# reclaimprotocol/gnark-symmetric-crypto

Measured on AMD Instinct MI355X. Metric: Groth16 proofs/sec (ChaCha20-V3 1-block), higher is better.
Workload: dtype u32 limbs (BN254 Fr/Fp, 254-bit modular integers); 1 GPU; ChaCha20-V3 single 64-byte block, reference pk.chacha20/r1cs.chacha20; 1xMI355X per rank: batch of 8192 independent proofs per GPU per step, fixed (r,s) (--dump-outputs); statements from xoshiro256** seeded 0x9E3779B97F4A7C15 + index; batch_per_gpu=8192, callers=2, parallelism=proofs sharded over 1 GPU(s), one process per GPU, gather to rank 0, tables=single algorithm per device

## Files before the change

gnark-symmetric-crypto_amd/__init__.py:

```python
import ctypes as C
import json
import os
import subprocess

_HERE = os.path.dirname(os.path.abspath(__file__))
LIB_PATH = os.path.join(_HERE, "libprove.so")
VERIFY_LIB_PATH = os.path.join(_HERE, "libverify.so")
CSRC = os.path.join(_HERE, "csrc")

CHACHA20, AES_128, AES_256 = 0, 1, 2
ALGORITHM_NAMES = {0: "chacha20", 1: "aes-128-ctr", 2: "aes-256-ctr"}

EXPORTS = ["enforce_binding", "InitAlgorithm", "Free", "Prove", "ProveBatch", "gsc_prove_raw", "gsc_setup",
           "gsc_set_deterministic_randomness", "gsc_debug_prove", "gsc_debug_vector", "gsc_describe", "gsc_last_stage_ms", "gsc_last_dominant_kernel", "gsc_last_kernel_clock", "gsc_debug_field_ops", "gsc_debug_limb_ops", "gsc_debug_curve_ops", "gsc_debug_decode_points", "gsc_debug_tower_ops", "gsc_debug_compute_h", "gsc_debug_compute_d", "gsc_debug_z_sum", "gsc_debug_quot_fold_dft", "gsc_debug_secret_residue", "gsc_debug_secret_scan", "gsc_debug_wipe", "gsc_debug_clock_trace", "gsc_debug_glv_split",
           "gsc_verify_init", "gsc_verify_raw", "VerifyBatch", "gsc_debug_pairing",
           "gsc_verify_raw_batched", "gsc_verify_all", "VerifyAll", "gsc_debug_verify_randomizers",
           "gsc_verify_json", "gsc_verify_last_path", "gsc_debug_verify_path", "gsc_debug_pairing_few",
           "gsc_verify_claims", "VerifyClaims",
           "gsc_prove_check_init", "gsc_prove_check_stats", "gsc_debug_prove_corrupt",
           "gsc_release_algorithm", "gsc_replace_algorithm", "gsc_memory_info", "gsc_key_generation",
           "gsc_setup_contribute", "gsc_setup_verify_contribution", "gsc_debug_scale_points",
           "gsc_srs_verify", "gsc_debug_srs_generate", "gsc_debug_group_idft", "gsc_debug_column_sums", "gsc_setup_from_srs", "gsc_debug_msm", "gsc_debug_solve", "gsc_debug_assemble",
           "gsc_srs_initial", "gsc_srs_contribute", "gsc_srs_verify_contribution", "gsc_debug_scale_powers"]


class GoSlice(C.Structure):
    _fields_ = [("data", C.c_void_p), ("len", C.c_longlong), ("cap", C.c_longlong)]


class DebugMsmArgs(C.Structure):
    _fields_ = [("group", C.c_int32), ("nbases", C.c_uint32),
                ("points", C.c_char_p), ("kind", C.c_char_p), ("rowlen", C.c_void_p), ("rows", C.c_void_p),
                ("n_rows", C.c_uint32), ("zero_row", C.c_uint32),
                ("c", C.c_int32), ("cv", C.c_int32), ("mont", C.c_int32),
                ("batch", C.c_uint32), ("nproofs", C.c_uint32), ("per_flat", C.c_uint32), ("per_win", C.c_uint32), ("digit_bases", C.c_uint32),
                ("digit_rows", C.c_void_p), ("scalars_be", C.c_char_p),
                ("plane", C.c_char_p), ("plane_rows", C.c_uint32), ("plane_stride", C.c_uint32),
                ("out", C.c_void_p), ("out_inf", C.c_void_p),
                ("flat_digits", C.c_void_p), ("flat_digits_cap", C.c_size_t), ("win_digits", C.c_void_p), ("win_digits_cap", C.c_size_t),
                ("gok", C.c_void_p), ("gok_cap", C.c_size_t), ("group_ok", C.c_void_p), ("group_ok_cap", C.c_size_t),
                ("info", C.c_void_p)]


class DebugSolveArgs(C.Structure):
    _fields_ = [("n_public", C.c_uint32), ("n_secret", C.c_uint32), ("n_internal", C.c_uint32), ("n_constraints", C.c_uint32),
                ("calldata", C.c_void_p), ("n_calldata", C.c_uint32),
                ("blueprint", C.c_void_p), ("constraint_off", C.c_void_p), ("wire_off", C.c_void_p), ("n_instr", C.c_uint32),
# ... 660 lines not shown
    if n <= 0:
        raise RuntimeError("algorithm not initialised")
    assert len(ab_be) == 2 * m * 64 * 32
    out = C.create_string_buffer(n * 64 * 32)
    if L.gsc_debug_compute_d(algorithm_id, ab_be, m, out, len(out)) != n:
        raise RuntimeError("gsc_debug_compute_d failed")
    return out.raw


def debug_z_sum(algorithm_id: int, abc_be: bytes, m: int):
    L = lib()
    L.gsc_debug_z_sum.restype = C.c_int
    L.gsc_debug_z_sum.argtypes = [C.c_ubyte, C.c_char_p, C.c_size_t, C.c_void_p, C.c_void_p]
    assert len(abc_be) == 3 * m * 64 * 32
    out, flags = C.create_string_buffer(64 * 64), C.create_string_buffer(64)
    if L.gsc_debug_z_sum(algorithm_id, abc_be, m, out, flags) != 0:
        raise RuntimeError("gsc_debug_z_sum failed")
    return out.raw, flags.raw


def debug_quot_fold_dft(L: int, m: int, perm, u_be: bytes, u_inf: bytes, v_be: bytes, v_inf: bytes):
    lb = lib()
    n = 1 << L
    lb.gsc_debug_quot_fold_dft.restype = C.c_int
    lb.gsc_debug_quot_fold_dft.argtypes = [C.c_int, C.c_uint32, C.c_void_p] + [C.c_char_p] * 4 + [C.c_void_p] * 4
    assert len(u_be) == 64 * m and len(u_inf) == m and len(v_be) == 64 * n and len(v_inf) == n and (perm is None or len(perm) == n)
    pm = (C.c_uint32 * n)(*perm) if perm is not None else None
    u2, f2, v2, g2 = C.create_string_buffer(64 * m), C.create_string_buffer(m), C.create_string_buffer(64 * max(m - 1, 1)), C.create_string_buffer(max(m - 1, 1))
    if lb.gsc_debug_quot_fold_dft(L, m, pm, u_be, u_inf, v_be, v_inf, u2, f2, v2, g2) != 0:
        raise RuntimeError("gsc_debug_quot_fold_dft failed")
    return u2.raw, f2.raw, v2.raw[:64 * (m - 1)], g2.raw[:m - 1]


def verify_init(algorithm_id: int, verifying_key: bytes) -> bool:
    s, keep = _slice(verifying_key)
    return bool(lib().gsc_verify_init(algorithm_id, s))


def verify_raw(algorithm_id: int, proofs: bytes, lens, signals: bytes, n: int = None):
    n = len(lens) if n is None else n
    assert len(proofs) >= 196 * n and len(signals) >= 144 * n
    lens_arr = (C.c_uint32 * max(n, 1))(*lens[:n])
    out = C.create_string_buffer(max(n, 1))
    rc = lib().gsc_verify_raw(algorithm_id, bytes(proofs), lens_arr, bytes(signals), n, out)
    if rc < 0:
        raise RuntimeError("gsc_verify_raw failed (%d): %s" % (rc, "no key loaded" if rc == -1 else "device error"))
    return list(out.raw[:n])


def verify_batch(items) -> list:
    enc = [{k: (list(v) if isinstance(v, (bytes, bytearray)) else v) for k, v in it.items()} if isinstance(it, dict) else it for it in items]
    s, keep = _slice(json.dumps(enc).encode())
    return json.loads(_take(lib().VerifyBatch(s)))


def verify_batch_bytes(params_json: bytes) -> bytes:
    s, keep = _slice(params_json)
    return _take(lib().VerifyBatch(s))


def verify_raw_batched(algorithm_id: int, proofs: bytes, lens, signals: bytes, n: int = None):
    n = len(lens) if n is None else n
    assert len(proofs) >= 196 * n and len(signals) >= 144 * n
    lens_arr = (C.c_uint32 * max(n, 1))(*lens[:n])
    out = C.create_string_buffer(max(n, 1))
    rc = lib().gsc_verify_raw_batched(algorithm_id, bytes(proofs), lens_arr, bytes(signals), n, out)
# ... 125 lines not shown
```

gnark-symmetric-crypto_amd/csrc/capi.cpp:

```cpp
#include "../../include/libprove.h"
#include "engine.hpp"
#include "dispatch.hpp"
#include "formats.hpp"
#include "registry.hpp"
#include "glv.hpp"
#include "host_ciphers.hpp"
#include "json.hpp"
#include "setup.hpp"
#include "phase2_gpu.hpp"
#include "srs_gpu.hpp"
#include "srs_contrib.hpp"
#include "srs_contrib_gpu.hpp"
#include "msm_debug.hpp"
#include "solver_debug.hpp"
#include "assemble_debug.hpp"
#include <sys/random.h>
#include <cerrno>
#include <condition_variable>
#include <deque>
#include <thread>
#include <cstdio>
#include <cstdlib>
#include <chrono>
#include <cstring>
// ... 634 lines not shown
        std::string report;
        const long long total = (long long)a->debug_secret_scan(report);
        if (out && cap) { const size_t n = report.size() < cap - 1 ? report.size() : cap - 1; memcpy(out, report.data(), n); out[n] = 0; }
        return total;
    } catch (const std::exception& e) { fprintf(stderr, "gsc_debug_secret_scan: %s\n", e.what()); return -1; }
}
int gsc_debug_wipe(uint64_t bytes, int fill, const uint64_t* desc, size_t ndesc, const uint8_t* cls, size_t ncls, uint8_t* buf_out, const uint64_t* win, size_t nwin, uint64_t* counts, float* ms) {
    if (hooks_refused("gsc_debug_wipe") || (ndesc && !desc) || (nwin && (!win || !counts)) || (ncls && !cls) || ndesc > 4096 || nwin > 4096) return -1;
    try { const float t = debug_wipe(config_from_env().device, bytes, fill, desc, ndesc, cls, ncls, buf_out, win, nwin, counts); if (ms) *ms = t; return 0; }
    catch (const std::exception& e) { fprintf(stderr, "gsc_debug_wipe: %s\n", e.what()); return -1; }
}
long long gsc_debug_compute_d(GoUint8 algorithmID, const uint8_t* ab_be, size_t m, uint8_t* d_out, size_t cap) {
    if (hooks_refused("gsc_debug_compute_d") || algorithmID > 2) return -1;
    const Snapshot snap = snapshot(algorithmID); Algorithm* a = algo_of(snap); if (!a) return -1;
    if (!d_out) return (long long)a->domain_size();
    if (cap < a->domain_size() * 64 * 32) return -1;
    try { a->debug_compute_d(ab_be, m, d_out); return (long long)a->domain_size(); }
    catch (const std::exception& e) { printf("%s\n", e.what()); return -1; }
}
int gsc_debug_z_sum(GoUint8 algorithmID, const uint8_t* abc_be, size_t m, uint8_t* out, uint8_t* flags) {
    if (hooks_refused("gsc_debug_z_sum") || algorithmID > 2 || !abc_be || !out || !flags) return -1;
    const Snapshot snap = snapshot(algorithmID); Algorithm* a = algo_of(snap); if (!a) return -1;
    try { a->debug_z_sum(abc_be, m, out, flags); return 0; }
    catch (const std::exception& e) { printf("%s\n", e.what()); return -1; }
}

int gsc_debug_quot_fold_dft(int L, uint32_t m, const uint32_t* perm, const uint8_t* u_be, const uint8_t* u_inf, const uint8_t* v_be, const uint8_t* v_inf,
                            uint8_t* u2_be, uint8_t* u2_inf, uint8_t* v2_be, uint8_t* v2_inf) {
    if (hooks_refused("gsc_debug_quot_fold_dft") || L < 2 || L > 17 || m < 2 || m > (1u << L) || !u_be || !u_inf || !v_be || !v_inf || !u2_be || !u2_inf || !v2_be || !v2_inf) return -1;
    try { debug_quot_fold_dft(config_from_env().device, L, m, perm, u_be, u_inf, v_be, v_inf, u2_be, u2_inf, v2_be, v2_inf); return 0; }
    catch (const std::exception& e) { printf("%s\n", e.what()); return -1; }
}

size_t gsc_describe(GoUint8 algorithmID, char* out, size_t cap) {
    if (algorithmID > 2 || !cap) return 0;
    const Snapshot snap = snapshot(algorithmID); Algorithm* a = algo_of(snap);
    std::string s = a ? a->describe() + " key=" + snap->key_id + " gen=" + std::to_string(snap.generation()) : std::string("not initialised");
    size_t n = s.size() < cap - 1 ? s.size() : cap - 1; memcpy(out, s.data(), n); out[n] = 0; return n;
}
int gsc_last_dominant_kernel(GoUint8 algorithmID, char* name, size_t cap, float* ms, size_t* statements, size_t* columns, size_t* nbases) {
    if (algorithmID > 2) return -1;
    const Snapshot snap = snapshot(algorithmID); Algorithm* a = algo_of(snap); if (!a) return -1;
    const KernelStat st = a->last_kernel_stat();
    if (name && cap) { const size_t n = strlen(st.name) < cap - 1 ? strlen(st.name) : cap - 1; memcpy(name, st.name, n); name[n] = 0; }
    if (ms) *ms = st.ms;
    if (statements) *statements = st.statements;
    if (columns) *columns = st.columns;
    if (nbases) *nbases = st.nbases;
    return 0;
}
int gsc_last_kernel_clock(GoUint8 algorithmID, float* clock_mhz, int* windows) {
    if (algorithmID > 2) return -1;
    const Snapshot snap = snapshot(algorithmID); Algorithm* a = algo_of(snap); if (!a) return -1;
    const KernelStat st = a->last_kernel_stat();
    if (clock_mhz) *clock_mhz = st.clock_mhz;
    if (windows) *windows = st.nwin;
    return 0;
}
int gsc_last_stage_ms(GoUint8 algorithmID, float out[4]) {
    if (algorithmID > 2) return -1;
    const Snapshot snap = snapshot(algorithmID); Algorithm* a = algo_of(snap); if (!a) return -1;
    const KernelStat st = a->last_kernel_stat();
    for (int i = 0; i < 4; i++) out[i] = st.stage_ms[i];
    return 0;
}

// ... 2 lines not shown
```

gnark-symmetric-crypto_amd/csrc/chunk_route.hpp:

```cpp
#pragma once
#include "engine.hpp"

namespace gsc {

struct RouteFacts {
    bool small_ok = false;
    bool has_commitment = false;
    bool quotient_eval = false, fuse_z_digits = false;
    bool zfew_flat = false;
    bool a_flat = false, b1_flat = false, b2_flat = false;
};
struct RouteCall {
    bool dbg = false;
    bool allow_few_solver = true;
    bool allow_small = true;
    bool skip_resident = false;
};

struct ChunkRoute {
    bool latency = false;
    bool resident_wanted = false;
    bool small = false;
    bool resident = false;
    bool early_ab = false, early_b2 = false;
    bool use_zfew = false;
    bool eval = false;
    bool z_digits_ready = false;
    bool overlap_q = false;
    const char* kernel_name = "";
};

constexpr size_t OVERLAP_QUOTIENT_BELOW = 4096;

inline ChunkRoute chunk_route(size_t n, const EngineConfig& cfg, const RouteFacts& f, const RouteCall& call) {
    const size_t B = (n + 63) / 64 * 64;
    ChunkRoute r;
    r.latency = cfg.few_path && n <= (size_t)cfg.few_max;
    r.resident_wanted = n <= (size_t)cfg.few_max && B == 64 && cfg.few_solver;
    r.small = f.small_ok && call.allow_small && !cfg.solver_trace && (!r.latency || cfg.small_witness_few);
    r.resident = r.resident_wanted && call.allow_few_solver && !r.small && !call.skip_resident;
    r.early_ab = r.latency && f.a_flat && f.b1_flat;
    r.early_b2 = r.early_ab && f.b2_flat;
    r.use_zfew = r.latency && f.zfew_flat;
    r.eval = f.quotient_eval && !r.use_zfew;
    r.z_digits_ready = r.eval && f.fuse_z_digits && !r.latency;
    r.overlap_q = r.z_digits_ready && !call.dbg && (cfg.overlap_quotient == 2 || (cfg.overlap_quotient && B < OVERLAP_QUOTIENT_BELOW));
    r.kernel_name = !r.latency ? "k_msm_win<Fp29f>"
                  : r.small ? "k_wit_chain + k_wit_rows"
                  : !r.resident ? "k_solver (one launch per level)"
                  : f.has_commitment ? "k_solver_few + commitment MSM" : "k_solver_few";
    return r;
}

}
```

gnark-symmetric-crypto_amd/csrc/engine.hip:

```cpp
#include "engine_impl.hpp"
#include "dispatch.hpp"
#include <cstdio>
#include <cstdlib>
#include <cstring>
#include <thread>

namespace gsc {

namespace {
int env_int(const char* name, int dflt) { const char* v = getenv(name); return v && *v ? atoi(v) : dflt; }
}

bool test_hooks_enabled() {
    static const bool on = [] { const char* e = getenv("GSC_ENABLE_TEST_HOOKS"); return e && e[0] == '1' && e[1] == 0; }();
    return on;
}
namespace { const bool g_hooks_read_at_load = test_hooks_enabled(); }

EngineConfig config_from_env() {
    EngineConfig c;
    c.device = env_int("GSC_DEVICE", 0);
    if (const char* dv = getenv("GSC_DEVICES")) {
        for (const char* q = dv; *q;) { while (*q == ',' || *q == ' ') q++; if (!*q) break; char* end = nullptr; const long v = strtol(q, &end, 10); if (end == q) throw std::runtime_error("GSC_DEVICES: expected a comma-separated list of device ordinals"); c.devices.push_back((int)v); q = end; }
    }
    c.max_batch = (size_t)env_int("GSC_MAX_BATCH", 1024);
    c.lanes = env_int("GSC_LANES", 0);
    c.small_lanes = env_int("GSC_SMALL_LANES", -1);
    if (c.small_lanes > 8) throw std::runtime_error("GSC_SMALL_LANES must be at most 8");
    c.small_lane_cap = env_int("GSC_SMALL_LANE_CAP", 0);
    if (c.small_lane_cap < 0 || c.small_lane_cap % 64) throw std::runtime_error("GSC_SMALL_LANE_CAP must be a multiple of 64");
    const bool hooks = test_hooks_enabled();
    c.min_split = (size_t)(hooks ? env_int("GSC_MIN_SPLIT", 0) : 0);
    c.bit_groups = env_int("GSC_BIT_GROUPS", 1);
    c.window_z = env_int("GSC_WINDOW_Z", 0);
    c.window_w = env_int("GSC_WINDOW_W", 0);
    c.z_table_gb = env_int("GSC_Z_TABLE_GB", 48);
    c.w_table_gb = env_int("GSC_W_TABLE_GB", 16);
    c.row_margin_bits = hooks ? env_int("GSC_ROW_MARGIN_BITS", 1) : 1;
    c.few_path = env_int("GSC_FEW_PATH", 1);
    c.few_solver = env_int("GSC_FEW_SOLVER", 1);
    c.few_max = env_int("GSC_FEW_MAX", 0);
    if (c.few_max < 0 || c.few_max > (int)MSM_FEW_PROOFS) throw std::runtime_error("GSC_FEW_MAX must be in [0, 32]");
    c.few_workgroups = hooks ? env_int("GSC_FEW_WGS", 0) : 0;
    c.few_z_gb = env_int("GSC_FEW_Z_GB", 12);
    c.few_wide = env_int("GSC_FEW_WIDE", 1);
    c.quotient_eval = env_int("GSC_QUOTIENT_EVAL", 1);
    c.fuse_z_digits = env_int("GSC_FUSE_Z_DIGITS", 1);
    c.quotient_fold = env_int("GSC_QUOTIENT_FOLD", 1);
    if (c.quotient_fold < 0 || c.quotient_fold > 2) throw std::runtime_error("GSC_QUOTIENT_FOLD must be 0, 1 or 2");
    c.quotient_live_tiles = env_int("GSC_QUOTIENT_LIVE_TILES", 1) ? 1 : 0;
    c.small_witness = env_int("GSC_SMALL_WITNESS", 1);
    c.small_witness_few = env_int("GSC_SMALL_WITNESS_FEW", 1);
    c.ntt_plain = env_int("GSC_NTT_PLAIN", 1) ? 1 : 0;
    c.overlap_quotient = env_int("GSC_OVERLAP_QUOTIENT", 1);
    if (c.overlap_quotient < 0 || c.overlap_quotient > 2) throw std::runtime_error("GSC_OVERLAP_QUOTIENT must be 0, 1 or 2");
    c.stream_priorities = env_int("GSC_STREAM_PRIORITIES", 1);
    if (c.stream_priorities != 0 && c.stream_priorities != 1 && !(hooks && c.stream_priorities >= 111 && c.stream_priorities <= 333)) throw std::runtime_error("GSC_STREAM_PRIORITIES must be 0 or 1");
    if (test_hooks_enabled()) { c.win_slice = env_int("GSC_WIN_SLICE", 256); if (c.win_slice < 64 || c.win_slice > 4096 || c.win_slice % 8) throw std::runtime_error("GSC_WIN_SLICE must be a multiple of 8 in [64, 4096]"); }
    if (c.small_witness < 0 || c.small_witness > 2 || (c.small_witness == 2 && !test_hooks_enabled())) throw std::runtime_error("GSC_SMALL_WITNESS must be 0 or 1");
    if (c.few_workgroups < 0 || c.few_workgroups > 256) throw std::runtime_error("GSC_FEW_WGS must be in [0, 256]");
    c.trace_host = getenv("GSC_TRACE_HOST") != nullptr;
    c.prove_check = env_int("GSC_PROVE_CHECK", 0) != 0;
    if (const char* d = getenv("GSC_VK_DIR")) c.vk_dir = d;
    if (test_hooks_enabled()) { c.solver_trace = getenv("GSC_SOLVER_TRACE") != nullptr; c.few_test_abort = getenv("GSC_FEW_TEST_ABORT") != nullptr; c.keep_secrets = getenv("GSC_KEEP_SECRETS") != nullptr; c.wipe_full = env_int("GSC_WIPE", 1) != 0; c.fail_after_stage = env_int("GSC_FAIL_AFTER_STAGE", 0); c.wipe_grid = env_int("GSC_WIPE_GRID", 0); if (c.wipe_grid < 0 || c.wipe_grid > 65536) throw std::runtime_error("GSC_WIPE_GRID must be in [0, 65536]"); c.z_exp_entry_bits = env_int("GSC_Z_EXP_ENTRY_BITS", 0); }
    if (c.max_batch < 64) c.max_batch = 64;
    c.max_batch = (c.max_batch + 63) / 64 * 64;
    if ((c.window_z && (c.window_z < 4 || c.window_z > MSM_MAX_WINDOW)) || (c.window_w && (c.window_w < 4 || c.window_w > 16))) throw std::runtime_error("GSC_WINDOW_Z must be in [4,17], GSC_WINDOW_W in [4,16]");
    return c;
}

void debug_field_ops(int device, int field, int op, const uint8_t* a, const uint8_t* b, uint8_t* out, size_t n, int chain) {
    use_device(device);
    DevBuf<fe> da(n), db(n), dout(n);
    HIP_CHECK(hipMemcpy(da.p, a, 32 * n, hipMemcpyHostToDevice)); HIP_CHECK(hipMemcpy(db.p, b, 32 * n, hipMemcpyHostToDevice));
    if (!launch_field_ops(field, op, da.p, db.p, dout.p, n, chain, nullptr)) throw std::runtime_error("gsc_debug_field_ops: field " + std::to_string(field) + " has no op " + std::to_string(op));
    HIP_CHECK(hipGetLastError());
    HIP_CHECK(hipDeviceSynchronize());
    HIP_CHECK(hipMemcpy(out, dout.p, 32 * n, hipMemcpyDeviceToHost));
}

void debug_limb_ops(int device, int field, int op, const int32_t* a, const int32_t* b, const int32_t* c, const int32_t* d, int32_t* out, size_t n) {
    const int operands = op == 0 ? 2 : op == 2 ? 4 : 1;
    const int32_t* src[4] = {a, b, c, d};
// ... 68 lines not shown
    HIP_CHECK(hipMemset(dflags.p, 0, n));
    if (!launch_tower_ops(path, op, din.p, dout.p, dflags.p, n, nullptr)) return false;
    HIP_CHECK(hipGetLastError());
    HIP_CHECK(hipDeviceSynchronize());
    if (ow) HIP_CHECK(hipMemcpy(out, dout.p, 4 * (size_t)ow * n, hipMemcpyDeviceToHost));
    HIP_CHECK(hipMemcpy(flags, dflags.p, n, hipMemcpyDeviceToHost));
    return true;
}

void debug_quot_fold_dft(int device, int L, uint32_t m, const uint32_t* perm, const uint8_t* u_be, const uint8_t* u_inf, const uint8_t* v_be, const uint8_t* v_inf,
                         uint8_t* u2_be, uint8_t* u2_inf, uint8_t* v2_be, uint8_t* v2_inf) {
    const size_t n = (size_t)1 << L;
    std::vector<uint32_t> pm(n);
    {
        std::vector<uint8_t> seen(n, 0);
        for (size_t i = 0; i < n; i++) { pm[i] = perm ? perm[i] : (uint32_t)i; if (pm[i] >= n || seen[pm[i]]++) throw std::runtime_error("gsc_debug_quot_fold_dft: perm is not a permutation of 0 .. n - 1"); }
    }
    use_device(device);
    DevBuf<uint32_t> d_perm(n);
    DevBuf<uint8_t> d_be((m + n) * 64), d_inf(m + n), d_stU(m), d_stV(n), d_stU2(m), d_stV2(m - 1), d_out((2 * (size_t)m - 1) * 64), d_flags(2 * (size_t)m - 1), scratch(quot_fold_dft_scratch_bytes(L, m));
    DevBuf<G1Aff> d_U(m), d_V(n), d_U2(m), d_V2(m - 1);
    HIP_CHECK(hipMemcpy(d_perm.p, pm.data(), 4 * n, hipMemcpyHostToDevice));
    HIP_CHECK(hipMemcpy(d_be.p, u_be, 64 * (size_t)m, hipMemcpyHostToDevice)); HIP_CHECK(hipMemcpy(d_be.p + 64 * (size_t)m, v_be, 64 * n, hipMemcpyHostToDevice));
    HIP_CHECK(hipMemcpy(d_inf.p, u_inf, m, hipMemcpyHostToDevice)); HIP_CHECK(hipMemcpy(d_inf.p + m, v_inf, n, hipMemcpyHostToDevice));
    launch_g1_aff_from_be(d_be.p, d_inf.p, m, d_U.p, d_stU.p, nullptr);
    launch_g1_aff_from_be(d_be.p + 64 * (size_t)m, d_inf.p + m, n, d_V.p, d_stV.p, nullptr);
    launch_quot_fold_dft(L, m, d_perm.p, d_U.p, d_stU.p, d_V.p, d_stV.p, d_U2.p, d_stU2.p, d_V2.p, d_stV2.p, scratch.p, nullptr);
    launch_g1_aff_to_be(d_U2.p, d_stU2.p, m, d_out.p, d_flags.p, nullptr);
    launch_g1_aff_to_be(d_V2.p, d_stV2.p, m - 1, d_out.p + 64 * (size_t)m, d_flags.p + m, nullptr);
    HIP_CHECK(hipGetLastError());
    HIP_CHECK(hipDeviceSynchronize());
    HIP_CHECK(hipMemcpy(u2_be, d_out.p, 64 * (size_t)m, hipMemcpyDeviceToHost)); HIP_CHECK(hipMemcpy(u2_inf, d_flags.p, m, hipMemcpyDeviceToHost));
    if (m > 1) { HIP_CHECK(hipMemcpy(v2_be, d_out.p + 64 * (size_t)m, 64 * (size_t)(m - 1), hipMemcpyDeviceToHost)); HIP_CHECK(hipMemcpy(v2_inf, d_flags.p + m, m - 1, hipMemcpyDeviceToHost)); }
}

float debug_wipe(int device, uint64_t bytes, int fill, const uint64_t* desc, size_t ndesc, const uint8_t* cls, size_t ncls, uint8_t* out, const uint64_t* win, size_t nwin, uint64_t* counts) {
    use_device(device);
    if (!bytes || bytes > ((uint64_t)1 << 36)) throw std::runtime_error("gsc_debug_wipe: buffer size out of range");
    auto checked = [&](const uint64_t* d, uint8_t* base, const uint8_t* d_cls) {
        const uint64_t off = d[0], rows = d[1], pitch = d[2], width = d[3];
        if (off > bytes || rows > bytes || pitch > bytes || width > bytes) throw std::runtime_error("gsc_debug_wipe: descriptor outside the buffer");
        if (rows && width) {
            if (rows > 1 && pitch < width) throw std::runtime_error("gsc_debug_wipe: rows overlap");
            const unsigned __int128 end = (unsigned __int128)off + (unsigned __int128)(rows - 1) * pitch + width;
            if (end > bytes) throw std::runtime_error("gsc_debug_wipe: descriptor outside the buffer");
        }
        if (d[4] && (!d_cls || !ncls)) throw std::runtime_error("gsc_debug_wipe: plane image without row classes");
        return WipeDesc{base + off, rows, pitch, width, d[4] ? d_cls : nullptr, d[4] ? (uint64_t)ncls : 0};
    };
    DevBuf<uint8_t> buf(bytes), d_cls(ncls ? ncls : 1); DevBuf<unsigned long long> d_cnt(nwin ? nwin : 1);
    if (ncls) HIP_CHECK(hipMemcpy(d_cls.p, cls, ncls, hipMemcpyHostToDevice));
    std::vector<WipeDesc> ds, ws;
    for (size_t i = 0; i < ndesc; i++) ds.push_back(checked(desc + 5 * i, buf.p, d_cls.p));
    for (size_t i = 0; i < nwin; i++) ws.push_back(checked(win + 5 * i, buf.p, d_cls.p));
    HIP_CHECK(hipMemset(buf.p, fill, bytes));
    HIP_CHECK(hipMemset(d_cnt.p, 0, d_cnt.bytes()));
    HIP_CHECK(hipDeviceSynchronize());
    hipEvent_t e0, e1; HIP_CHECK(hipEventCreate(&e0)); HIP_CHECK(hipEventCreate(&e1));
    struct Ev { hipEvent_t a, b; ~Ev() { (void)hipEventDestroy(a); (void)hipEventDestroy(b); } } ev{e0, e1};
    HIP_CHECK(hipEventRecord(e0, nullptr));
    launch_wipe(ds.data(), ds.size(), 0, nullptr);
    HIP_CHECK(hipEventRecord(e1, nullptr));
    for (size_t i = 0; i < nwin; i++) launch_scan_idle(ws[i], d_cnt.p + i, nullptr);
    HIP_CHECK(hipGetLastError());
    HIP_CHECK(hipDeviceSynchronize());
    float ms = 0; HIP_CHECK(hipEventElapsedTime(&ms, e0, e1));
// ... 41 lines not shown
    for (size_t k = 0; k < impls_.size(); k++) { std::lock_guard<std::mutex> l(impls_[k]->check_mu); impls_[k]->check = ctx[k]; }
    return true;
}
void Algorithm::prove_check_off() { for (auto& i : impls_) { std::lock_guard<std::mutex> l(i->check_mu); i->check.reset(); } }
void Algorithm::prove_check_stats(uint64_t out[4]) const {
    for (int k = 0; k < 4; k++) out[k] = 0;
    for (auto& i : impls_) if (auto c = i->check_now()) prove_check_add_stats(*c, out);
}
bool Algorithm::debug_prove_corrupt(uint32_t index, int which, int mode) {
    if (which < 0 || which > 4 || mode < 0 || mode > 1 || (which > 2 && !impls_[0]->has_commitment)) return false;
    corrupt_.store((uint64_t)1 << 63 | (uint64_t)mode << 40 | (uint64_t)which << 32 | index);
    return true;
}
Algorithm::~Algorithm() = default;
Cipher Algorithm::cipher() const { return impls_[0]->cipher; }
size_t Algorithm::max_batch() const { size_t c = 0; for (auto& i : impls_) c += i->cap; return c; }
size_t Algorithm::devices() const { return impls_.size(); }
size_t Algorithm::lanes() const { return impls_[0]->lanes.size(); }
namespace { thread_local KernelStat t_call_stat; thread_local const Algorithm* t_call_owner = nullptr; }
KernelStat Algorithm::last_kernel_stat() const {
    if (t_call_owner == this) return t_call_stat;
    AlgorithmImpl* a = impls_[last_replica_.load() < impls_.size() ? last_replica_.load() : 0].get();
    std::lock_guard<std::mutex> lk(a->stat_mu);
    return a->last_stat;
}
std::string Algorithm::describe() const {
    const AlgorithmImpl* impl_ = impls_[0].get();
    char buf[640];
    snprintf(buf, sizeof buf, "wires=%zu constraints=%zu domain=2^%d max_batch=%zu lanes=%zu small=%zux%zu devices=%zu window_z=%d window_w=%d tables=%.2f GiB bases A=%zu B=%zu K=%zu Z=%zu grouped A=%zu B=%zu K=%zu wide(windowed+expanded) A=%zu+%zu B=%zu+%zu K=%zu+%zu",
             impl_->n_wires, impl_->n_constraints, impl_->L, max_batch(), impl_->full_lanes, impl_->lanes.size() - impl_->full_lanes, impl_->lanes.size() > impl_->full_lanes ? impl_->lanes.back()->cap : (size_t)0, impls_.size(), impl_->cfg.window_z, impl_->cfg.window_w, impl_->table_bytes / 1073741824.0,
             impl_->mA.nbases, impl_->mB1.nbases, impl_->mK.nbases, impl_->mZ.digit_bases ? impl_->mZ.digit_bases : impl_->mZ.nbases, impl_->mA.nbit, impl_->mB1.nbit, impl_->mK.nbit,
             impl_->mA.nwide, impl_->mA.nexpanded, impl_->mB1.nwide, impl_->mB1.nexpanded, impl_->mK.nwide, impl_->mK.nexpanded);
    std::string out = buf;
    if (impl_->quotient_eval) out += std::string(" quotient=evaluation-form") + (impl_->fuse_z_digits ? "+digits" : "") + (!impl_->fuse_z_digits || !impl_->cfg.overlap_quotient ? "" : impl_->cfg.overlap_quotient == 2 ? "+beside-wire-sets" : "+beside-wire-sets(<4096)") + "(c: " + std::to_string(impl_->mC.nbit) + " grouped + " + std::to_string(impl_->mC.nflat - impl_->mC.nbit) + " flat + " + std::to_string(impl_->mC.nwide) + " windowed)";
    else out += " quotient=coefficient-form";
    if (impl_->quotient_eval) out += impl_->mZ.digit_bases ? " Zlive=" + std::to_string(impl_->mZ.nwide) + " Zfold=dft" :" Zfold=off(" + impl_->fold_why + ")";
    if (impl_->quotient_eval) out += " Qtiles=" + std::to_string(quot_live_tiles(impl_->L, impl_->quot_live)) + "/" + std::to_string(1u << (impl_->L - (impl_->L + 1) / 2));
    out += impl_->small.ok ? " witness=small-integer(" + std::to_string(impl_->small.n_levels) + " chained levels, fallbacks " + std::to_string(impl_->small_fallbacks.load()) + ")" : " witness=generic" + (impl_->small.why.empty() ? std::string() : "(" + impl_->small.why + ")");
    out += impl_->cfg.keep_secrets ? " wipe=off" : impl_->cfg.wipe_full ? " wipe=full" : " wipe=inputs";
    {
        size_t bytes = 0; bool on = false;
        for (auto& i : impls_) if (auto c = i->check_now()) { on = true; bytes += prove_check_device_bytes(*c); }
        out += on ? " check=on(" + std::to_string(bytes) + ")" : " check=off";
    }
    out += " served(calls/statements)=";
    const auto sv = picker_->served();
    for (size_t i = 0; i < sv.size(); i++) out += (i ? "," : "") + std::to_string(sv[i].calls) + "/" + std::to_string(sv[i].statements);
    return out;
}
size_t Algorithm::domain_size() const { return impls_[0]->domain_n; }
template <class Quot>
static void debug_quotient(AlgorithmImpl& a, const char* who, const uint8_t* mats_be, size_t mats, size_t m, uint8_t* out, Quot quot) {
    if (m > a.n_constraints) throw std::runtime_error(std::string(who) + ": more rows than constraints");
    HIP_CHECK(hipSetDevice(a.cfg.device));
    struct Hold { AlgorithmImpl& a; size_t i; ~Hold() { a.release_lane(i); } } hold{a, a.acquire_lane(0)};
    AlgorithmImpl::Lane& ln = *a.lanes[0];
    const size_t B = 64, cnt = m * B;
    DevBuf<uint8_t> d_be(mats * cnt * 32 + 32, true);
    d_be.upload(mats_be, mats * cnt * 32, ln.stream);
    fe* const dst[3] = {ln.d_A.p, ln.d_B.p, ln.d_C.p};
    for (size_t k = 0; k < mats; k++) launch_fr_from_be(d_be.p + k * cnt * 32, dst[k], cnt, ln.stream);
    NttPlan plan{a.L, a.tw_fwd.p, a.tw_inv.p, a.scale_mid.p, a.scale_out.p, a.dom.p + 5, a.qr.p};
    HIP_CHECK(quot(plan, ln, B));
    if (out) HIP_CHECK(hipMemcpyAsync(out, ln.d_A.p, a.domain_n * B * 32, hipMemcpyDeviceToHost, ln.stream));
    if (!a.cfg.keep_secrets && a.cfg.wipe_full) a.wipe_whole(ln, ln.stream);
    HIP_CHECK(hipStreamSynchronize(ln.stream));
}
// ... 119 lines not shown
```

gnark-symmetric-crypto_amd/csrc/engine.hpp:

```cpp
#pragma once
#include <cstdint>
#include <cstring>
#include <atomic>
#include <cstddef>
#include <memory>
#include <string>
#include <utility>
#include <vector>

namespace gsc {

enum Cipher : int { CHACHA20 = 0, AES_128 = 1, AES_256 = 2 };

struct ProofRequest {
    uint8_t key[32]; uint32_t keylen;
    uint8_t nonce[12]; uint32_t counter;
    uint8_t plaintext[64];
    uint8_t ciphertext[64];
    uint8_t r[32], s[32], mask[32];
    ~ProofRequest() { explicit_bzero(this, sizeof *this); }
};
struct ProofResult {
    int status = 0;
    uint8_t proof[196]; size_t proof_len = 0;
};

struct EngineConfig {
    int device = 0;
    std::vector<int> devices;
    size_t max_batch = 1024;
    int lanes = 0;
    int small_lanes = -1;
    int small_lane_cap = 0;
    size_t min_split = 0;
    int window_z = 0;
    int window_w = 0;
    int z_table_gb = 48, w_table_gb = 16;
    int bit_groups = 1;
    int row_margin_bits = 1;
    int few_path = 1;
    int few_max = 0;
    int few_solver = 1;
    int few_workgroups = 0;
    int few_z_gb = 12;
    int few_wide = 1;
    int quotient_eval = 1;
    int fuse_z_digits = 1;
    int quotient_fold = 1;
    int quotient_live_tiles = 1;
    int small_witness = 1;
    int ntt_plain = 1;
    int overlap_quotient = 1;
    int stream_priorities = 1;
    int small_witness_few = 1;
    int win_slice = 256;
    bool prove_check = false;
    std::string vk_dir;
    bool trace_host = false;
    bool solver_trace = false;
    int z_exp_entry_bits = 0;
    bool keep_secrets = false;
    bool wipe_full = true;
    int wipe_grid = 0;
    int fail_after_stage = 0;
    bool few_test_abort = false;
    std::vector<size_t> outgoing_bytes; size_t reclaim_bytes = 0;
};
EngineConfig config_from_env();
bool test_hooks_enabled();

struct KernelStat { const char* name = ""; float ms = 0; size_t statements = 0, columns = 0, nbases = 0; float stage_ms[4] = {0, 0, 0, 0}; float clock_mhz = 0; int nwin = 0; };

struct DebugVectors { std::vector<uint8_t> W, A, B, C, H; size_t n_wires = 0, n_constraints = 0, n = 0; };

class AlgorithmImpl;
class Algorithm {
  public:
    Algorithm(Cipher cipher, const uint8_t* pk, size_t pk_len, const uint8_t* r1cs, size_t r1cs_len, const EngineConfig& cfg);
    ~Algorithm();
    Cipher cipher() const;
    void prove_batch(const ProofRequest* reqs, size_t n, ProofResult* results, DebugVectors* debug_first = nullptr, bool whole = false);
    void forget_thread_stat() const;
    size_t max_batch() const;
    size_t devices() const;
    size_t lanes() const;
    std::string describe() const;
    KernelStat last_kernel_stat() const;
    void debug_compute_h(const uint8_t* abc_be, size_t m, uint8_t* h_out);
    void debug_compute_d(const uint8_t* ab_be, size_t m, uint8_t* d_out);
    size_t domain_size() const;
    void debug_z_sum(const uint8_t* abc_be, size_t m, uint8_t* out, uint8_t* flags);
    size_t debug_secret_residue();
    size_t debug_secret_scan(std::string& report);
    size_t scrub_before_free();
    std::vector<std::pair<int, size_t>> replica_bytes() const;
    bool prove_check_init(const uint8_t* vk, size_t len);
    void prove_check_off();
    void prove_check_stats(uint64_t out[4]) const;
    bool debug_prove_corrupt(uint32_t index, int which, int mode);
  private:
    std::atomic<uint64_t> corrupt_{0};
    std::vector<std::unique_ptr<AlgorithmImpl>> impls_;
    std::unique_ptr<class ReplicaPicker> picker_;
    mutable std::atomic<size_t> last_replica_{0};
};

bool device_memory_info(int device, uint64_t out[4]);
size_t verifier_device_bytes(int device);

void debug_quot_fold_dft(int device, int L, uint32_t m, const uint32_t* perm, const uint8_t* u_be, const uint8_t* u_inf, const uint8_t* v_be, const uint8_t* v_inf,
                         uint8_t* u2_be, uint8_t* u2_inf, uint8_t* v2_be, uint8_t* v2_inf);
float debug_wipe(int device, uint64_t bytes, int fill, const uint64_t* desc, size_t ndesc, const uint8_t* cls, size_t ncls, uint8_t* out, const uint64_t* win, size_t nwin, uint64_t* counts);
void debug_clock_trace(int device, uint32_t n, uint32_t interval_us, unsigned long long* out);
void debug_field_ops(int device, int field, int op, const uint8_t* a, const uint8_t* b, uint8_t* out, size_t n, int chain);
void debug_limb_ops(int device, int field, int op, const int32_t* a, const int32_t* b, const int32_t* c, const int32_t* d, int32_t* out, size_t n);
void debug_curve_ops(int device, int group, int op, const uint8_t* pts, const uint8_t* inf, const uint8_t* lam, size_t n, size_t k, uint8_t* out, uint8_t* flags);
void debug_decode_points(int device, int group, const uint8_t* bytes, size_t len, size_t n, uint8_t* out_xy, uint8_t* status);
bool debug_tower_ops(int device, int path, int op, const int32_t* in, size_t n, int32_t* out, uint8_t* flags);

}
```

gnark-symmetric-crypto_amd/csrc/engine_impl.hpp:

```cpp
#pragma once
#include "engine.hpp"
#include "chunk_route.hpp"
#include "formats.hpp"
#include "kernels.hpp"
#include "wit_small.hpp"
#include "solver_tables.hpp"
#include "msm_set.hpp"
#include "wipe_plan.hpp"
#include "prove_check.hpp"
#include <atomic>
#include <chrono>
#include <cstring>
#include <condition_variable>
#include <memory>
#include <mutex>
#include <stdexcept>
#include <string>
#include <vector>

namespace gsc {

template <class T>
struct PinnedBuf {
    T* p = nullptr; size_t n = 0;
    PinnedBuf() = default;
    PinnedBuf(const PinnedBuf&) = delete; PinnedBuf& operator=(const PinnedBuf&) = delete;
    ~PinnedBuf() { if (p) (void)hipHostFree(p); }
    void alloc(size_t count) { if (p) { (void)hipHostFree(p); p = nullptr; } n = count; if (count) { HIP_CHECK(hipHostMalloc((void**)&p, count * sizeof(T), hipHostMallocDefault)); memset(p, 0, count * sizeof(T)); } }
    size_t bytes() const { return n * sizeof(T); }
};

struct KeyPoints {
    std::vector<uint8_t> x, y;
    KeyPoints() = default;
    KeyPoints(const std::vector<uint8_t>& x_, const std::vector<uint8_t>& y_ = {}) : x(x_), y(y_) {}
};
std::vector<uint8_t> decode_g1_points(const KeyPoints& pts, G1Aff* out, hipStream_t stream);
std::vector<uint8_t> decode_g2_points(const KeyPoints& pts, G2Aff* out, hipStream_t stream);


constexpr int STREAM_PLAIN = 1 << 30, STREAM_ROLE_INIT = -1;
hipStream_t stream_take(int device, int kind, int role);
void stream_give(int device, int kind, int role, hipStream_t s);

std::atomic<size_t>& prover_bytes_on(int device);

class AlgorithmImpl : public SolverTables {
  public:
    Cipher cipher; EngineConfig cfg;
    size_t domain_n = 0; int L = 0;
    std::mutex pool_mu; std::condition_variable pool_cv; std::vector<uint8_t> lane_busy;
    size_t acquire_lane(int want = -1, size_t n = 0) {
        std::unique_lock<std::mutex> l(pool_mu);
        size_t got = 0;
        pool_cv.wait(l, [&] {
            bool found = false;
            for (size_t i = 0; i < lane_busy.size(); i++) {
                if (lane_busy[i] || (want >= 0 && (size_t)want != i) || lanes[i]->cap < n) continue;
                if (!found || lanes[i]->cap < lanes[got]->cap) { got = i; found = true; }
            }
            return found;
        });
        lane_busy[got] = 1;
        return got;
    }
    std::atomic<int> calls_in_flight{0};
    int cu_count = 256;
    std::atomic<uint32_t> few_skip{0}; std::atomic<uint32_t> few_penalty{16};
    std::mutex stat_mu; KernelStat last_stat;
    std::mutex check_mu; std::shared_ptr<ProveCheckCtx> check;
    std::shared_ptr<ProveCheckCtx> check_now() { std::lock_guard<std::mutex> l(check_mu); return check; }
    std::atomic<uint64_t>* corrupt = nullptr;
    void release_lane(size_t i) { { std::lock_guard<std::mutex> l(pool_mu); lane_busy[i] = 0; } pool_cv.notify_all(); }
    hipStream_t stream = nullptr;
    size_t table_bytes = 0;
    std::vector<uint8_t> row_class;

    std::vector<uint8_t> row_class_a, row_class_b;
    void init_small(const SolverProgram& sp);
    std::atomic<uint64_t> small_fallbacks{0};
    DevBuf<int32_t> tw_fwd, tw_inv, tw_inv_plain, qr; DevBuf<fe> scale_mid, scale_mid_plain, scale_out, dom;
    MsmSet<G1Aff> mA, mB1, mK, mZ, mZfew, mPed, mPedSigma; MsmSet<G2Aff> mB2;
    bool quotient_eval = false; MsmSet<G1Aff> mC; std::vector<uint8_t> row_class_c;
    bool fuse_z_digits = false;
    std::string fold_why = "GSC_QUOTIENT_FOLD=0";
    size_t quot_live = 0;
    bool fold_quotient_bases(const DevBuf<G1Aff>& d_U, const std::vector<uint8_t>& stU, const DevBuf<G1Aff>& d_V, const std::vector<uint8_t>& stV, const std::vector<uint32_t>& rowsZ,
                             DevBuf<G1Aff>& d_U2, std::vector<uint8_t>& stU2, DevBuf<G1Aff>& d_V2, std::vector<uint8_t>& stV2);
    struct Lane {
        hipStream_t stream = nullptr, side = nullptr, side2 = nullptr;
        hipEvent_t ev_ab = nullptr, ev_fs = nullptr, ev_b2 = nullptr, ev_s2 = nullptr;
        hipEvent_t ev_ws = nullptr;
        hipEvent_t ev_wa = nullptr, ev_wa_done = nullptr;
        hipEvent_t ev_few = nullptr;
        hipEvent_t ev[7] = {};
        float stage_ms[4] = {0, 0, 0, 0}; float msm_z_kernel_ms = 0; size_t last_batch = 0;
        PinnedBuf<uint8_t> h_in, h_rs, h_mask, h_out, h_flags, h_cpts; PinnedBuf<uint32_t> h_status; PinnedBuf<GlvSplit> h_glv; PinnedBuf<unsigned long long> h_words;
        uint32_t* h_fsync() const { return reinterpret_cast<uint32_t*>(h_words.p); }
        uint32_t& h_wsflag() const { return *reinterpret_cast<uint32_t*>(h_words.p + 1); }
        unsigned long long* h_clk() const { return h_words.p + 2; }
        KernelStat stat;
        DevBuf<unsigned long long> d_clk;
        size_t n_real = 0;
        size_t cap = 0;
        DevBuf<uint8_t> d_inputs, d_rs, d_out, d_flags, d_mask_in, d_cpts; DevBuf<uint32_t> d_status, d_fsync; DevBuf<GlvSplit> d_glv;
        DevBuf<fe> d_mask, d_commit; DevBuf<G1Xyzz> d_sumD, d_sumPok;
        DevBuf<fe> d_W, d_A, d_B, d_C;
        bool small_active = false;
        DevBuf<int8_t> d_W8, d_A8, d_B8, d_C8; DevBuf<uint32_t> d_wsflag;
        DevBuf<G1Xyzz> d_part1a, d_part1b, d_sumA, d_sumB1, d_sumK, d_sumZ, d_sumC, d_tmp; DevBuf<G2Xyzz> d_part2a, d_part2b, d_sumB2;
        DevBuf<uint4> d_digits_s2; DevBuf<uint8_t> d_gok_s2;
        DevBuf<uint4> d_digits_s; DevBuf<uint8_t> d_gok_s; DevBuf<G1Xyzz> d_part1c, d_part1d;
        DevBuf<uint4> d_digits;
        DevBuf<uint4> d_digits_w;
        static constexpr int NSETS = 8;
        DevBuf<G1Xyzz> d_sj1[NSETS], d_flat1[NSETS]; DevBuf<G2Xyzz> d_sj2, d_flat2;
        MsmHornerJobs pending1{}, pending2{};
        DevBuf<uint8_t> d_gok;
        struct Region { int region; uint8_t* p; size_t bytes; };
        std::vector<Region> regions; size_t allocated = 0;
        template <class T> void reg(int region, DevBuf<T>& b) { if (b.p) regions.push_back(Region{region, reinterpret_cast<uint8_t*>(b.p), b.bytes()}); }
        struct ScratchNeed { size_t part1a = 0, part1b = 0, part2a = 0, part2b = 0, digits = 0, digits_w = 0, gok = 0, sj1[8] = {0, 0, 0, 0, 0, 0, 0, 0}, sj2 = 0; };
        std::vector<ScratchNeed> need_at;
        bool wipe_a_pending = false;
        ~Lane() { if (ev_few) { for (int d = 0; d < 64; d++) { FewSolverChain& c = few_solver_chain(d); std::lock_guard<std::mutex> lk(c.m); if (c.last == ev_few) c.last = nullptr; } (void)hipEventDestroy(ev_few); }
                  for (auto& e : ev) if (e) (void)hipEventDestroy(e); if (ev_ws) (void)hipEventDestroy(ev_ws); if (ev_wa) (void)hipEventDestroy(ev_wa); if (ev_wa_done) (void)hipEventDestroy(ev_wa_done); if (ev_ab) (void)hipEventDestroy(ev_ab); if (ev_fs) (void)hipEventDestroy(ev_fs); if (ev_b2) (void)hipEventDestroy(ev_b2); if (ev_s2) (void)hipEventDestroy(ev_s2); if (side2) stream_give(device, kind[2], 3 * index + 2, side2); if (side) stream_give(device, kind[1], 3 * index + 1, side); if (stream) stream_give(device, kind[0], 3 * index, stream); }
        int device = 0, index = 0, kind[3] = {STREAM_PLAIN, STREAM_PLAIN, STREAM_PLAIN};
    };
    std::vector<std::unique_ptr<Lane>> lanes;
    size_t cap = 0;
    size_t full_lanes = 0;
    static constexpr size_t SMALL_LANE_CAP = 1024;

    AlgorithmImpl(Cipher c, const uint8_t* pk, size_t pk_len, const uint8_t* r1cs, size_t r1cs_len, const EngineConfig& cf);
    ~AlgorithmImpl() { prover_bytes_on(cfg.device) -= accounted; lanes.clear(); if (stream) stream_give(cfg.device, STREAM_PLAIN, STREAM_ROLE_INIT, stream); }
    size_t held_bytes() const { size_t b = table_bytes; for (auto& ln : lanes) b += ln->allocated; return b; }
    size_t accounted = 0;

    std::unique_ptr<SolverProgram> init_program(const R1csFile& cs);

    static void pack_inputs(const ProofRequest* reqs, size_t n, size_t B, uint8_t* h_in, uint8_t* h_rs);

    void calibrate();

    std::vector<uint8_t> decompress_g1(const KeyPoints& pts, G1Aff* out) { return decode_g1_points(pts, out, stream); }
    std::vector<uint8_t> decompress_g2(const KeyPoints& pts, G2Aff* out) { return decode_g2_points(pts, out, stream); }

    static constexpr size_t EXPAND_MAX = 64;
    static constexpr int EXPAND_C = 15, NARROW_MAX_BITS = 14;

    template <class AffT, class XyzzT, class Decomp>
    void build_set(MsmSet<AffT>& set, const KeyPoints& raw, size_t point_bytes, const std::vector<uint32_t>& rows, int c, const char* what, Decomp decomp, bool uniform, int expand_cv = 0,
                   const std::vector<uint8_t>* classes = nullptr, uint32_t zero_row = 0xFFFFFFFFu, bool latency_layout = true);
    void init_key(const R1csFile& cs, const PkFile& key);

    void alloc_lane(Lane& ln, size_t B);

    RouteFacts route_facts() const { return RouteFacts{small.ok, has_commitment, quotient_eval, fuse_z_digits, mZfew.nflat != 0, mA.latency_flat(), mB1.latency_flat(), mB2.latency_flat()}; }
    struct Chunk {
        const ProofRequest* reqs; size_t n, B; DebugVectors* dbg; ChunkRoute rt;
        std::chrono::steady_clock::time_point t_start, t_enqueued, t_done;
        std::shared_ptr<ProveCheckCtx> check = nullptr;
        uint64_t corrupt = 0;
        std::vector<uint8_t> verdict = {};
        bool check_fell_back = false;
    };
    MsmLaunchOpts msm_opts;
    MsmCtx with_plane(MsmCtx c, const Lane& ln, const fe* scalars) const {
        if (!ln.small_active) return c;
        if (scalars == ln.d_W.p) { c.plane = ln.d_W8.p; c.plane_rows = n_wires; c.plane_stride = small.rows_per_group; }
        else if (scalars == ln.d_C.p) { c.plane = ln.d_C8.p; c.plane_rows = n_constraints; c.plane_stride = n_constraints; }
        return c;
    }
    int set_index(const MsmSet<G1Aff>& set) const { const MsmSet<G1Aff>* all[Lane::NSETS] = {&mA, &mB1, &mK, &mZ, &mPed, &mPedSigma, &mZfew, &mC}; for (int k = 0; k < Lane::NSETS; k++) if (all[k] == &set) return k; return 0; }
    void run_msm_g1(Lane& ln, const Chunk& ck, const MsmSet<G1Aff>& set, const fe* scalars, int mont, G1Xyzz* sum, bool timed = false, bool side = false, bool digits_ready = false);
    void run_msm_g2(Lane& ln, const Chunk& ck, const MsmSet<G2Aff>& set, const fe* scalars, int mont, G2Xyzz* sum, bool side = false);
    template <class AffT> void flush_horner(MsmHornerJobs& pending, size_t B, hipStream_t s) { launch_msm_horner<AffT>(pending, B, s); pending.n = 0; }

    void fetch_column(Lane& ln, const fe* mat, size_t rows, size_t B, size_t col, std::vector<uint8_t>& out);
    void wipe_secrets(Lane& ln, size_t B, bool small_call);
    WipePlan plan_wipe(const Lane& ln, const Chunk& ck) const;
    void run_wipe(Lane& ln, const std::vector<WipeItem>& items, hipStream_t s, unsigned max_blocks);
    void wipe_phase_a(Lane& ln, const Chunk& ck);
    void wipe_phase_b(Lane& ln, const Chunk& ck);
    void wipe_whole(Lane& ln, hipStream_t s);
    void fail_after(int stage) const { if (cfg.fail_after_stage == stage) throw std::runtime_error("GSC_FAIL_AFTER_STAGE=" + std::to_string(stage) + ": test failure injected"); }
    size_t secret_residue();
    size_t secret_scan(size_t lane_base, std::string& report, size_t& registered, size_t& allocated);

    void prove_chunk(Lane& ln, const ProofRequest* reqs, size_t n, ProofResult* results, DebugVectors* dbg, bool allow_few_solver = true, bool allow_small = true);
    std::unique_ptr<ProveCheckPass> check_enqueue(Lane& ln, const Chunk& ck);
    void stage_upload(Lane& ln, const Chunk& ck);
    void stage_witness(Lane& ln, const Chunk& ck);
    void stage_early_sums(Lane& ln, const Chunk& ck);
    void stage_quotient(Lane& ln, const Chunk& ck);
    void stage_msms(Lane& ln, const Chunk& ck);
    void stage_assembly(Lane& ln, Chunk& ck);
    void stage_stat(Lane& ln, const Chunk& ck);
    void run_levels(Lane& ln, const Chunk& ck, SolverArgs& sa, uint32_t from, uint32_t to);
    void solve_small(Lane& ln, const Chunk& ck);
    void dump_solver_trace(Lane& ln, const unsigned long long* d_trace);
    void trace_chunk(Lane& ln, const Chunk& ck);

    void serialize(const uint8_t* o, uint8_t flags, uint32_t status, const uint8_t* commitment_xy, const uint8_t* pok_xy, ProofResult& res, bool released = true) const;
};

}
// ... 1 lines not shown
```

gnark-symmetric-crypto_amd/csrc/engine_prove.hip:

```cpp
#include "engine_impl.hpp"
#include "glv.hpp"
#include "prove_check_kernels.hpp"
#include <chrono>
#include <cstdio>
#include <cstring>

namespace gsc {

FewSolverChain& few_solver_chain(int device) { static FewSolverChain* chains = new FewSolverChain[64]; return chains[device & 63]; }

namespace {
const uint8_t kHalfP[32] = {0x18, 0x32, 0x27, 0x39, 0x70, 0x98, 0xd0, 0x14, 0xdc, 0x28, 0x22, 0xdb, 0x40, 0xc0, 0xac, 0x2e,
                            0xcb, 0xc0, 0xb5, 0x48, 0xb4, 0x38, 0xe5, 0x46, 0x9e, 0x10, 0x46, 0x0b, 0x6c, 0x3e, 0x7e, 0xa3};

void le_limbs_to_be(const uint8_t* le, uint8_t* be) { for (int i = 0; i < 32; i++) be[i] = le[31 - i]; }
bool be_greater(const uint8_t* a, const uint8_t* b) { int c = memcmp(a, b, 32); return c > 0; }
bool be_is_zero(const uint8_t* a) { for (int i = 0; i < 32; i++) if (a[i]) return false; return true; }
}

void AlgorithmImpl::run_msm_g1(Lane& ln, const Chunk& ck, const MsmSet<G1Aff>& set, const fe* scalars, int mont, G1Xyzz* sum, bool timed, bool side, bool digits_ready) {
    const int k = set_index(set);
    MsmRun<G1Xyzz> r{MsmCtx{ln.stream, ln.d_digits_w.p && &set != &mZ ? ln.d_digits_w.p : ln.d_digits.p, ln.d_gok.p}, scalars, mont != 0, ck.B, ck.n, ck.rt.latency,
                     ln.d_part1a.p, ln.d_part1b.p, ln.d_sj1[k].p, ln.d_flat1[k].p, sum};
    if (side) {
// ... 252 lines not shown
        if (dbg) {
            DevBuf<fe> ta(domain_n * B, true), tb(domain_n * B, true), tc(domain_n * B, true);
            HIP_CHECK(hipMemcpyAsync(ta.p, ln.d_A.p, n_constraints * B * sizeof(fe), hipMemcpyDeviceToDevice, ln.stream));
            HIP_CHECK(hipMemcpyAsync(tb.p, ln.d_B.p, n_constraints * B * sizeof(fe), hipMemcpyDeviceToDevice, ln.stream));
            HIP_CHECK(hipMemcpyAsync(tc.p, ln.d_C.p, n_constraints * B * sizeof(fe), hipMemcpyDeviceToDevice, ln.stream));
            HIP_CHECK(launch_compute_h(plan, ta.p, tb.p, tc.p, n_constraints, B, ln.stream, 0));
            fetch_column(ln, ta.p, domain_n, B, 0, dbg->H);
        }
        if (rt.overlap_q) HIP_CHECK(hipStreamWaitEvent(qs, ln.ev[1], 0));
        if (rt.z_digits_ready) HIP_CHECK(launch_compute_d_digits(plan, ln.d_A.p, ln.d_B.p, n_constraints, B, QuotDigits{ln.d_digits.p, mZ.c, mZ.nwin}, qs, narrow, quot_live));
        else HIP_CHECK(launch_compute_d(plan, ln.d_A.p, ln.d_B.p, n_constraints, B, ln.stream, few_cols, narrow, quot_live));
    } else HIP_CHECK(launch_compute_h(plan, ln.d_A.p, ln.d_B.p, ln.d_C.p, n_constraints, B, ln.stream, few_cols, narrow));
    HIP_CHECK(hipEventRecord(ln.ev[2], qs));
    if (dbg && !rt.eval) fetch_column(ln, ln.d_A.p, domain_n, B, 0, dbg->H);
}

void AlgorithmImpl::stage_msms(Lane& ln, const Chunk& ck) {
    const size_t B = ck.B; const ChunkRoute& rt = ck.rt;
    if (!rt.early_ab) {
        run_msm_g1(ln, ck, mA, ln.d_W.p, 1, ln.d_sumA.p);
        run_msm_g1(ln, ck, mB1, ln.d_W.p, 1, ln.d_sumB1.p);
        flush_horner<G1Aff>(ln.pending1, B, ln.stream);
        HIP_CHECK(hipEventRecord(ln.ev_ab, ln.stream));
        HIP_CHECK(hipStreamWaitEvent(ln.side, ln.ev_ab, 0));
        launch_fin_scalarmul(ln.d_sumA.p, ln.d_sumB1.p, ln.d_rs.p, B, ln.d_out.p, ln.d_flags.p, ln.d_tmp.p, ln.side);
    }
    if (!rt.early_b2) run_msm_g2(ln, ck, mB2, ln.d_W.p, 1, ln.d_sumB2.p);
    if (ln.pending2.n) {
        HIP_CHECK(hipEventRecord(ln.ev_b2, ln.stream));
        HIP_CHECK(hipStreamWaitEvent(ln.side, ln.ev_b2, 0));
        flush_horner<G2Aff>(ln.pending2, B, ln.side);
    }
    HIP_CHECK(hipEventRecord(ln.ev_fs, ln.side));
    run_msm_g1(ln, ck, mK, ln.d_W.p, 1, ln.d_sumK.p);
    if (rt.eval) {
        HIP_CHECK(hipMemsetAsync(ln.d_C.p + domain_n * B, 0, B * sizeof(fe), ln.stream));
        run_msm_g1(ln, ck, mC, ln.d_C.p, 1, ln.d_sumC.p);
    }
    if (rt.overlap_q) { HIP_CHECK(hipEventRecord(ln.ev_ws, ln.stream)); HIP_CHECK(hipStreamWaitEvent(ln.stream, ln.ev[2], 0)); }
    wipe_phase_a(ln, ck);
    run_msm_g1(ln, ck, rt.use_zfew ? mZfew : mZ, ln.d_A.p, 0, ln.d_sumZ.p, !rt.latency, false, rt.z_digits_ready);
    if (has_commitment) run_msm_g1(ln, ck, mPedSigma, ln.d_W.p, 1, ln.d_sumPok.p);
    flush_horner<G1Aff>(ln.pending1, B, ln.stream);
    if (has_commitment) launch_points_to_affine_be(ln.d_sumPok.p, B, ln.d_cpts.p + 64 * B, ln.d_flags.p, 16, ln.stream);
    HIP_CHECK(hipGetLastError());
    HIP_CHECK(hipEventRecord(ln.ev[3], ln.stream));
}

void AlgorithmImpl::stage_assembly(Lane& ln, Chunk& ck) {
    const size_t B = ck.B; const ChunkRoute& rt = ck.rt;
    HIP_CHECK(hipStreamWaitEvent(ln.stream, ln.ev_fs, 0));
    if (rt.early_b2) HIP_CHECK(hipStreamWaitEvent(ln.stream, ln.ev_s2, 0));
    launch_fin_combine(ln.d_sumB2.p, ln.d_sumK.p, ln.d_sumZ.p, rt.eval ? ln.d_sumC.p : nullptr, ln.d_tmp.p, B, ln.d_out.p, ln.d_flags.p, ln.stream);
    HIP_CHECK(hipGetLastError());
    HIP_CHECK(hipEventRecord(ln.ev[4], ln.stream));
    if (ck.corrupt) {
        launch_prove_corrupt(ln.d_out.p, ln.d_cpts.p, B, ck.n, (uint32_t)ck.corrupt, (int)((ck.corrupt >> 32) & 0xFF), (int)((ck.corrupt >> 40) & 0xFF), ln.stream);
        HIP_CHECK(hipGetLastError());
    }
    const std::unique_ptr<ProveCheckPass> pass = ck.check ? check_enqueue(ln, ck) : nullptr;
    HIP_CHECK(hipMemcpyAsync(ln.h_out.p, ln.d_out.p, 256 * B, hipMemcpyDeviceToHost, ln.stream));
    HIP_CHECK(hipMemcpyAsync(ln.h_flags.p, ln.d_flags.p, (B + 3) / 4 * 4, hipMemcpyDeviceToHost, ln.stream));
    HIP_CHECK(hipMemcpyAsync(ln.h_status.p, ln.d_status.p, B * 4, hipMemcpyDeviceToHost, ln.stream));
    if (has_commitment) HIP_CHECK(hipMemcpyAsync(ln.h_cpts.p, ln.d_cpts.p, 128 * B, hipMemcpyDeviceToHost, ln.stream));
    memset(ln.h_words.p, 0, ln.h_words.bytes());
    if (rt.resident) HIP_CHECK(hipMemcpyAsync(ln.h_fsync(), ln.d_fsync.p, 8, hipMemcpyDeviceToHost, ln.stream));
    if (rt.small) HIP_CHECK(hipMemcpyAsync(&ln.h_wsflag(), ln.d_wsflag.p, 4, hipMemcpyDeviceToHost, ln.stream));
    wipe_phase_b(ln, ck);
    if (!rt.latency) { HIP_CHECK(hipMemcpyAsync(ln.h_clk(), ln.d_clk.p, (cfg.trace_host ? 44 : 32) * 8, hipMemcpyDeviceToHost, ln.stream)); HIP_CHECK(hipMemsetAsync(ln.d_clk.p, 0, 32 * 8, ln.stream)); }
    ck.t_enqueued = std::chrono::steady_clock::now();
    HIP_CHECK(hipStreamSynchronize(ln.stream));
    if (pass) {
        ck.verdict = pass->finish(ln.h_status.p, ln.h_flags.p); ck.check_fell_back = pass->fell_back();
        if (!ln.h_fsync()[1] && !ln.h_wsflag()) {
            size_t checked = 0, refused = 0;
            for (size_t i = 0; i < ck.n; i++) if (ln.h_status.p[i] == 0xFFFFFFFFu && !ln.h_flags.p[i]) { checked++; refused += !ck.verdict[i]; }
            pass->count(checked, refused);
        }
    }
    ck.t_done = std::chrono::steady_clock::now();
}

std::unique_ptr<ProveCheckPass> AlgorithmImpl::check_enqueue(Lane& ln, const Chunk& ck) {
    std::vector<uint8_t> sig(144 * ck.n);
    for (size_t i = 0; i < ck.n; i++) {
        const ProofRequest& q = ck.reqs[i]; uint8_t* o = sig.data() + 144 * i;
// ... 121 lines not shown
```

gnark-symmetric-crypto_amd/csrc/engine_tables.hip:

```cpp
#include "engine_impl.hpp"
#include "host_ciphers.hpp"
#include <algorithm>
#include <chrono>
#include <cstdio>
#include <cstring>
#include <map>
#include <tuple>

namespace gsc {

AlgorithmImpl::AlgorithmImpl(Cipher c, const uint8_t* pk, size_t pk_len, const uint8_t* r1cs, size_t r1cs_len, const EngineConfig& cf) : cipher(c), cfg(cf) {
    if (!cfg.few_max) cfg.few_max = cipher == CHACHA20 ? 32 : 20;
    if (cfg.few_max < 0 || cfg.few_max > (int)MSM_FEW_PROOFS) throw std::runtime_error("EngineConfig::few_max must be in [0, " + std::to_string(MSM_FEW_PROOFS) + "]");
    msm_opts.win_slice = (size_t)cfg.win_slice;
    int ndev = 0;
    if (hipGetDeviceCount(&ndev) != hipSuccess || ndev == 0) throw std::runtime_error("no HIP device available: the GPU prover has no CPU fallback");
    HIP_CHECK(hipSetDevice(cfg.device));
    stream = stream_take(cfg.device, STREAM_PLAIN, STREAM_ROLE_INIT);
    struct StreamGuard { hipStream_t& s; int device; bool armed = true; ~StreamGuard() { if (armed && s) { stream_give(device, STREAM_PLAIN, STREAM_ROLE_INIT, s); s = nullptr; } } } stream_guard{stream, cfg.device};
    { int cus = 0; if (hipDeviceGetAttribute(&cus, hipDeviceAttributeMultiprocessorCount, cfg.device) == hipSuccess && cus > 0) cu_count = cus; }
    const bool trace = cfg.trace_host;
    auto now = [] { return std::chrono::steady_clock::now(); };
    auto ms = [](std::chrono::steady_clock::time_point a, std::chrono::steady_clock::time_point b) { return std::chrono::duration<double, std::milli>(b - a).count(); };
    const auto t0 = now();
// ... 129 lines not shown
    HIP_CHECK(hipStreamSynchronize(stream));
}

namespace {
template <class AffT, size_t STRIDE, class Compressed, class Raw, class After>
std::vector<uint8_t> decode_points(const KeyPoints& pts, AffT* out, hipStream_t stream, Compressed compressed, Raw raw, After after) {
    const size_t n = pts.x.size() / STRIDE; std::vector<uint8_t> st(n);
    if (!n) return st;
    if (!pts.y.empty() && pts.y.size() != pts.x.size()) throw std::runtime_error("key points: the y bytes do not match the x bytes");
    DevBuf<uint8_t> d_x(pts.x.size()), d_y(pts.y.size()), d_st(n);
    d_x.upload(pts.x.data(), pts.x.size(), stream);
    compressed(d_x.p, out, d_st.p, n, stream);
    if (!pts.y.empty()) {
        d_y.upload(pts.y.data(), pts.y.size(), stream);
        raw(d_x.p, d_y.p, out, d_st.p, n, stream);
    }
    after(out, d_st.p, n, stream);
    HIP_CHECK(hipGetLastError());
    HIP_CHECK(hipMemcpyAsync(st.data(), d_st.p, n, hipMemcpyDeviceToHost, stream));
    HIP_CHECK(hipStreamSynchronize(stream));
    return st;
}
}

std::vector<uint8_t> decode_g1_points(const KeyPoints& pts, G1Aff* out, hipStream_t stream) {
    return decode_points<G1Aff, 32>(pts, out, stream, launch_decompress_g1, launch_decode_raw_g1, [](G1Aff*, uint8_t*, size_t, hipStream_t) {});
}
std::vector<uint8_t> decode_g2_points(const KeyPoints& pts, G2Aff* out, hipStream_t stream) {
    return decode_points<G2Aff, 64>(pts, out, stream, launch_decompress_g2, launch_decode_raw_g2, launch_g2_subgroup);
}

template <class AffT, class XyzzT, class Decomp>
void AlgorithmImpl::build_set(MsmSet<AffT>& set, const KeyPoints& raw, size_t point_bytes, const std::vector<uint32_t>& rows, int c, const char* what, Decomp decomp, bool uniform, int expand_cv,
                              const std::vector<uint8_t>* classes, uint32_t zero_row, bool latency_layout) {
    const std::vector<uint8_t>& cls = classes ? *classes : row_class;
    const size_t n = raw.x.size() / point_bytes;
    if (rows.size() != n) throw std::runtime_error(std::string("pk: row map size mismatch for ") + what);
    set.nbases = n;
    DevBuf<AffT> bases(n ? n : 1);
    const std::vector<uint8_t> st = decomp(raw, bases.p);
    for (size_t i = 0; i < n; i++) if (st[i] == 1) throw std::runtime_error(std::string("pk: invalid point in ") + what);
    const uint32_t ROW_ZERO = zero_row != 0xFFFFFFFFu ? zero_row : (uint32_t)(n_wires + 3);
    const MsmFlatPlan plan = msm_plan_flat(msm_sort_bases(st, rows, cls, uniform, cfg.bit_groups, cfg.row_margin_bits, NARROW_MAX_BITS), rows, ROW_ZERO, uniform, expand_cv, EXPAND_MAX, EXPAND_C, msm_windows);
    msm_build_tables<AffT, XyzzT>(set, bases.p, plan, rows, c, stream, &table_bytes);
    if (set.nwide && !uniform && cfg.few_path && cfg.few_wide && latency_layout) {
        const std::vector<uint32_t>& wide = plan.wide;
        KeyPoints raw_w; raw_w.x.resize(set.nwide * point_bytes); if (!raw.y.empty()) raw_w.y.resize(set.nwide * point_bytes);
        std::vector<uint32_t> rows_w(set.nwide);
        for (size_t i = 0; i < set.nwide; i++) {
            memcpy(raw_w.x.data() + i * point_bytes, raw.x.data() + (size_t)wide[i] * point_bytes, point_bytes); rows_w[i] = rows[wide[i]];
            if (!raw.y.empty()) memcpy(raw_w.y.data() + i * point_bytes, raw.y.data() + (size_t)wide[i] * point_bytes, point_bytes);
        }
        set.few_wide.reset(new MsmSet<AffT>());
        build_set<AffT, XyzzT>(*set.few_wide, raw_w, point_bytes, rows_w, c, what, decomp, true, 8, classes, zero_row);
    }
}

bool AlgorithmImpl::fold_quotient_bases(const DevBuf<G1Aff>& d_U, const std::vector<uint8_t>& stU, const DevBuf<G1Aff>& d_V, const std::vector<uint8_t>& stV, const std::vector<uint32_t>& rowsZ,
                                        DevBuf<G1Aff>& d_U2, std::vector<uint8_t>& stU2, DevBuf<G1Aff>& d_V2, std::vector<uint8_t>& stV2) {
    const size_t m = n_constraints;
    DevBuf<uint32_t> d_perm(domain_n); d_perm.upload(rowsZ.data(), domain_n, stream);
    DevBuf<uint8_t> d_stU(m), d_stV(domain_n), d_stU2(m), d_stV2(m - 1), scratch(quot_fold_dft_scratch_bytes(L, (uint32_t)m));
    d_stU.upload(stU.data(), m, stream); d_stV.upload(stV.data(), domain_n, stream);
    d_U2.alloc(m); d_V2.alloc(m - 1); stU2.resize(m); stV2.resize(m - 1);
    hipEvent_t ev[3]; for (auto& e : ev) HIP_CHECK(hipEventCreate(&e));
    struct Free { hipEvent_t* e; ~Free() { for (int i = 0; i < 3; i++) (void)hipEventDestroy(e[i]); } } free_ev{ev};
    HIP_CHECK(hipEventRecord(ev[0], stream));
    launch_quot_fold_dft(L, (uint32_t)m, d_perm.p, d_U.p, d_stU.p, d_V.p, d_stV.p, d_U2.p, d_stU2.p, d_V2.p, d_stV2.p, scratch.p, stream, ev[1]);
    HIP_CHECK(hipGetLastError());
    HIP_CHECK(hipEventRecord(ev[2], stream));
    HIP_CHECK(hipMemcpyAsync(stU2.data(), d_stU2.p, m, hipMemcpyDeviceToHost, stream));
    HIP_CHECK(hipMemcpyAsync(stV2.data(), d_stV2.p, m - 1, hipMemcpyDeviceToHost, stream));
    HIP_CHECK(hipStreamSynchronize(stream));
    if (cfg.trace_host) {
        float w = 0, t = 0; HIP_CHECK(hipEventElapsedTime(&w, ev[0], ev[1])); HIP_CHECK(hipEventElapsedTime(&t, ev[1], ev[2]));
        fprintf(stderr, "  tables G1.Z fold (dft): weights %.0f ms, transforms %.0f ms\n", w, t);
    }
    if (std::count(stV2.begin(), stV2.end(), (uint8_t)0) != (ptrdiff_t)(m - 1)) { fold_why = "a folded V base is the point at infinity"; return false; }
    fold_why.clear();
    return true;
}

void AlgorithmImpl::init_key(const R1csFile& cs, const PkFile& key) {
    if (key.n_wires != n_wires) throw std::runtime_error("pk: wire count does not match the r1cs");
    domain_n = key.domain_n; L = 0; while (((size_t)1 << L) < domain_n) L++;
    if (domain_n < n_constraints || domain_n != (size_t)1 << L) throw std::runtime_error("pk: domain too small for the constraint system");
    if (L < NTT_MIN_LOG2 || L > NTT_MAX_LOG2) throw std::runtime_error("pk: unsupported domain size 2^" + std::to_string(L) + " (the quotient kernels cover 2^15 .. 2^17: ChaCha20-V3 and AES-V2)");
    if (cs.has_commitment != key.has_commitment_key) throw std::runtime_error("pk: commitment keys do not match the r1cs");
    {
        uint8_t be[5 * 32];
        memcpy(be, key.omega, 32); memcpy(be + 32, key.omega_inv, 32); memcpy(be + 64, key.coset_g, 32); memcpy(be + 96, key.coset_g_inv, 32); memcpy(be + 128, key.n_inv, 32);
        DevBuf<uint8_t> d_be(sizeof be); d_be.upload(be, sizeof be, stream);
        dom.alloc(6);
        launch_fr_from_be(d_be.p, dom.p, 5, stream);
        tw_fwd.alloc(domain_n / 2 * 12); tw_inv.alloc(domain_n / 2 * 12); scale_mid.alloc(domain_n); scale_mid_plain.alloc(domain_n); tw_inv_plain.alloc(domain_n / 2 * 12); scale_out.alloc(domain_n); qr.alloc((2 * NTT_QMAX + 1) * 12);
        DevBuf<uint32_t> d_flag(1); uint32_t flag = 0;
        HIP_CHECK(hipMemsetAsync(d_flag.p, 0, 4, stream));
        launch_ntt_constants(dom.p, dom.p + 1, dom.p + 4, L, tw_fwd.p, tw_inv.p, scale_mid.p, scale_out.p, dom.p + 5, qr.p, d_flag.p, tw_inv_plain.p, scale_mid_plain.p, stream);
        HIP_CHECK(hipGetLastError());
        HIP_CHECK(hipMemcpyAsync(&flag, d_flag.p, 4, hipMemcpyDeviceToHost, stream));
        HIP_CHECK(hipStreamSynchronize(stream));
        if (flag) throw std::runtime_error("pk: the domain generator is not gnark-crypto's root of unity for this size");
    }
    auto cat = [](KeyPoints a, std::initializer_list<KeyPoints> more) {
        bool any_y = !a.y.empty();
        for (auto& m : more) any_y = any_y || !m.y.empty();
        if (any_y) a.y.resize(a.x.size(), 0);
        for (auto& m : more) {
            a.x.insert(a.x.end(), m.x.begin(), m.x.end());
            if (any_y) { a.y.insert(a.y.end(), m.y.begin(), m.y.end()); a.y.resize(a.x.size(), 0); }
        }
        return a;
    };
    const uint32_t ROW_ONE = 0, ROW_R = (uint32_t)n_wires, ROW_S = ROW_R + 1, ROW_NRS = ROW_R + 2;
    std::vector<uint32_t> rowsA, rowsB, rowsK;
    for (size_t i = 0; i < n_wires; i++) { if (!key.inf_A[i]) rowsA.push_back((uint32_t)i); if (!key.inf_B[i]) rowsB.push_back((uint32_t)i); }
    {
        std::vector<uint8_t> skip(n_wires, 0);
        if (cs.has_commitment) { for (uint32_t w : cs.commit_private) skip[w] = 1; skip[cs.commit_wire] = 1; }
        for (size_t i = cs.n_public; i < n_wires; i++) if (!skip[i]) rowsK.push_back((uint32_t)i);
        if (rowsK.size() * 32 != key.g1_K.size()) throw std::runtime_error("pk: G1.K size does not match the private wires");
    }
    rowsA.push_back(ROW_ONE); rowsA.push_back(ROW_R);
    std::vector<uint32_t> rowsB2 = rowsB;
    rowsB.push_back(ROW_ONE); rowsB.push_back(ROW_S); rowsB2.push_back(ROW_ONE); rowsB2.push_back(ROW_S);
    rowsK.push_back(ROW_NRS);
    quotient_eval = cfg.quotient_eval != 0;
    std::vector<uint32_t> rowsZ(quotient_eval ? domain_n : domain_n - 1); for (size_t i = 0; i < rowsZ.size(); i++) rowsZ[i] = quotient_eval ? quot_digit_index(L, (uint32_t)i) : (uint32_t)i;
    std::vector<uint32_t> rowsZkey(domain_n - 1); for (size_t i = 0; i < rowsZkey.size(); i++) rowsZkey[i] = (uint32_t)i;
    std::vector<uint32_t> rowsC; if (quotient_eval) { rowsC.resize(n_constraints); for (size_t i = 0; i < n_constraints; i++) rowsC[i] = (uint32_t)i; }
    if (!cfg.window_z) {
        double budget = cfg.z_table_gb * 1e9;
        size_t free_b = 0, total_b = 0;
        if (hipMemGetInfo(&free_b, &total_b) == hipSuccess) {
            const double nlanes = cfg.lanes > 0 ? cfg.lanes : (cs.has_commitment ? 2 : 1);
            const double lane = nlanes * (double)cfg.max_batch * ((double)n_wires * 32 + 3.0 * (double)domain_n * 32 + (double)domain_n * 2 * 20 + 1e5) * 1.15;
            const double others = (cfg.w_table_gb + (cfg.few_path ? cfg.few_z_gb + (cs.has_commitment ? 8 : 0) : 0)) * 1e9 + 8.0 * 1073741824.0;
            const double room = (double)free_b + (double)cfg.reclaim_bytes - lane - others;
            if (room < budget) budget = room > 0 ? room : 0;
        }
        cfg.window_z = 4;
        for (int c = MSM_MAX_WINDOW; c >= 4; c--) if ((double)rowsZ.size() * (double)((size_t)1 << (c - 1)) * 64.0 <= budget) { cfg.window_z = c; break; }
    }
    if (!cfg.window_w) {
        auto wide_in = [&](const std::vector<uint32_t>& rows, const std::vector<uint8_t>& cls) {
            size_t k = 0;
            for (uint32_t r : rows) { const int cl = r < cls.size() ? cls[r] : 255; if (cfg.bit_groups <= 0 || cl == 255 || cl + cfg.row_margin_bits > NARROW_MAX_BITS) k++; }
            return k > EXPAND_MAX ? (double)k : 0.0;
        };
        auto wide_of = [&](const std::vector<uint32_t>& rows) { return wide_in(rows, row_class); };
        const double g1 = wide_of(rowsA) + wide_of(rowsB) + wide_of(rowsK) + 2 * wide_of(cs.commit_private) + wide_in(rowsC, row_class_c), g2 = wide_of(rowsB2);
        cfg.window_w = 4;
        for (int c = 16; c >= 4; c--) if ((g1 * 64.0 + g2 * 128.0) * (double)((size_t)1 << (c - 1)) <= cfg.w_table_gb * 1e9) { cfg.window_w = c; break; }
    }
    auto dec1 = [this](const KeyPoints& raw, G1Aff* out) { return decompress_g1(raw, out); };
    auto dec2 = [this](const KeyPoints& raw, G2Aff* out) { return decompress_g2(raw, out); };
    const bool trace = cfg.trace_host;
    auto timed = [&](const char* what, auto&& fn) {
        const auto a0 = std::chrono::steady_clock::now(); const size_t b0 = table_bytes; fn();
        if (trace) fprintf(stderr, "  tables %-8s %7.0f ms %8.2f GiB\n", what, std::chrono::duration<double, std::milli>(std::chrono::steady_clock::now() - a0).count(), (table_bytes - b0) / 1073741824.0);
    };
    timed("G1.A", [&] { build_set<G1Aff, G1Xyzz>(mA, cat({key.g1_A, key.g1_A_y}, {{key.g1_alpha, key.g1_alpha_y}, {key.g1_delta, key.g1_delta_y}}), 32, rowsA, cfg.window_w, "G1.A", dec1, false); });
    timed("G1.B", [&] { build_set<G1Aff, G1Xyzz>(mB1, cat({key.g1_B, key.g1_B_y}, {{key.g1_beta, key.g1_beta_y}, {key.g1_delta, key.g1_delta_y}}), 32, rowsB, cfg.window_w, "G1.B", dec1, false); });
    timed("G1.K", [&] { build_set<G1Aff, G1Xyzz>(mK, cat({key.g1_K, key.g1_K_y}, {{key.g1_delta, key.g1_delta_y}}), 32, rowsK, cfg.window_w, "G1.K", dec1, false); });
    if (!quotient_eval) timed("G1.Z", [&] { build_set<G1Aff, G1Xyzz>(mZ, KeyPoints(key.g1_Z, key.g1_Z_y), 32, rowsZ, cfg.window_z, "G1.Z", dec1, true); });
    else {
        const size_t nz = key.g1_Z.size() / 32;
        if (nz + 1 != domain_n) throw std::runtime_error("pk: G1.Z does not hold n - 1 points");
        DevBuf<G1Aff> d_U(domain_n), d_V(domain_n); std::vector<uint8_t> stU(domain_n), stV(domain_n);
        timed("G1.Z -> U, V", [&] {
            DevBuf<G1Aff> zb(nz); const std::vector<uint8_t> st = decompress_g1(KeyPoints(key.g1_Z, key.g1_Z_y), zb.p);
            for (size_t i = 0; i < nz; i++) if (st[i] == 1) throw std::runtime_error("pk: invalid point in G1.Z");
            DevBuf<uint8_t> d_st(nz), d_stU(domain_n), d_stV(domain_n); d_st.upload(st.data(), nz, stream);
            DevBuf<fe> tw(domain_n / 2); DevBuf<G1Xyzz> scratch(domain_n); DevBuf<uint32_t> d_perm(domain_n);
            d_perm.upload(rowsZ.data(), domain_n, stream);
            launch_quot_bases(zb.p, d_st.p, L, 0, dom.p + 1, dom.p + 4, tw.p, scratch.p, nullptr, d_U.p, d_stU.p, stream);
            launch_quot_bases(zb.p, d_st.p, L, 1, dom.p + 1, dom.p + 4, tw.p, scratch.p, d_perm.p, d_V.p, d_stV.p, stream);
            HIP_CHECK(hipGetLastError());
            HIP_CHECK(hipMemcpyAsync(stU.data(), d_stU.p, domain_n, hipMemcpyDeviceToHost, stream));
            HIP_CHECK(hipMemcpyAsync(stV.data(), d_stV.p, domain_n, hipMemcpyDeviceToHost, stream));
            HIP_CHECK(hipStreamSynchronize(stream));
        });
        auto from_dev = [this](const DevBuf<G1Aff>& src, const std::vector<uint8_t>& st) {
            return [this, &src, &st](const KeyPoints& raw, G1Aff* out) {
                const size_t n = raw.x.size() / 32;
                HIP_CHECK(hipMemcpyAsync(out, src.p, n * sizeof(G1Aff), hipMemcpyDeviceToDevice, stream));
                HIP_CHECK(hipStreamSynchronize(stream));
                return std::vector<uint8_t>(st.begin(), st.begin() + n);
            };
        };
        DevBuf<G1Aff> d_U2, d_V2; std::vector<uint8_t> stU2, stV2;
        size_t live = domain_n;
        if (cfg.quotient_fold) {
            if (n_constraints < 2 || domain_n - n_constraints + 1 < domain_n / 64) fold_why = "nothing to drop";
            else if (std::count(stV.begin(), stV.end(), (uint8_t)0) != (ptrdiff_t)domain_n) fold_why = "a V base is the point at infinity";
            else timed("G1.Z fold", [&] { if (fold_quotient_bases(d_U, stU, d_V, stV, rowsZ, d_U2, stU2, d_V2, stV2)) live = n_constraints - 1; });
        }
        const bool folded = live != domain_n;
        const std::vector<uint8_t> rawV(live * 32, 0), rawU(n_constraints * 32, 0);
        const std::vector<uint32_t> rowsV(rowsZ.begin(), rowsZ.begin() + live);
        timed("G1.Z (V)", [&] { build_set<G1Aff, G1Xyzz>(mZ, rawV, 32, rowsV, cfg.window_z, "G1.Z (evaluation form)", folded ? from_dev(d_V2, stV2) : from_dev(d_V, stV), true); });
        fuse_z_digits = mZ.nwide == live && cfg.fuse_z_digits != 0;
        if (folded) mZ.digit_bases = domain_n;
        quot_live = folded && cfg.quotient_live_tiles ? live : 0;
        timed("G1.Z (U)", [&] { build_set<G1Aff, G1Xyzz>(mC, rawU, 32, rowsC, cfg.window_w, "G1.Z (evaluation form, c)", folded ? from_dev(d_U2, stU2) : from_dev(d_U, stU), false, 0, &row_class_c, (uint32_t)domain_n, false); });
    }
    if (cfg.few_path && cfg.few_z_gb > 0) {
        const size_t nz = key.g1_Z.size() / 32;
        int cv = 0;
        for (int t : {8, 6, 4}) if ((double)nz * msm_windows(t) * (double)((size_t)1 << (t - 1)) * sizeof(G1Aff) <= (double)cfg.few_z_gb * 1e9) { cv = t; break; }
        if (cv) timed("G1.Z (latency layout)", [&] { build_set<G1Aff, G1Xyzz>(mZfew, KeyPoints(key.g1_Z, key.g1_Z_y), 32, rowsZkey, cfg.window_z, "G1.Z", dec1, true, cv); });
    }
    timed("G2.B", [&] { build_set<G2Aff, G2Xyzz>(mB2, cat({key.g2_B, key.g2_B_y}, {{key.g2_beta, key.g2_beta_y}, {key.g2_delta, key.g2_delta_y}}), 64, rowsB2, cfg.window_w, "G2.B", dec2, false); });
    if (cs.has_commitment) {
        if (cs.n_public_committed) throw std::runtime_error("r1cs: public committed wires are not supported");
        if (key.ped_basis.size() != cs.commit_private.size() * 32) throw std::runtime_error("pk: commitment basis size does not match the r1cs");
        build_set<G1Aff, G1Xyzz>(mPed, KeyPoints(key.ped_basis, key.ped_basis_y), 32, cs.commit_private, cfg.window_w, "commitment basis", dec1, false);
        build_set<G1Aff, G1Xyzz>(mPedSigma, KeyPoints(key.ped_basis_sigma, key.ped_basis_sigma_y), 32, cs.commit_private, cfg.window_w, "commitment basis (sigma)", dec1, false);
    }
}

void AlgorithmImpl::alloc_lane(Lane& ln, size_t B) {
    ln.cap = B;
    struct Tally { Tally(size_t* t) { devbuf_tally = t; } ~Tally() { devbuf_tally = nullptr; } } tally{&ln.allocated};
    int least = 0, greatest = 0;
    HIP_CHECK(hipDeviceGetStreamPriorityRange(&least, &greatest));
    if (cfg.stream_priorities && least != greatest) {
        const int code = cfg.stream_priorities == 1 ? 213 : cfg.stream_priorities;
        auto level = [&](int d) { return d == 1 ? greatest : d == 3 ? least : (least + greatest) / 2; };
        ln.kind[0] = level(code / 100); ln.kind[1] = level(code / 10 % 10); ln.kind[2] = level(code % 10);
    }
    ln.device = cfg.device; ln.index = (int)lanes.size() - 1;
    ln.stream = stream_take(ln.device, ln.kind[0], 3 * ln.index); ln.side = stream_take(ln.device, ln.kind[1], 3 * ln.index + 1); ln.side2 = stream_take(ln.device, ln.kind[2], 3 * ln.index + 2);
    for (auto& e : ln.ev) HIP_CHECK(hipEventCreate(&e));
    HIP_CHECK(hipEventCreate(&ln.ev_ws));
    HIP_CHECK(hipEventCreateWithFlags(&ln.ev_wa, hipEventDisableTiming)); HIP_CHECK(hipEventCreateWithFlags(&ln.ev_wa_done, hipEventDisableTiming));
    HIP_CHECK(hipEventCreateWithFlags(&ln.ev_few, hipEventDisableTiming));
    HIP_CHECK(hipEventCreateWithFlags(&ln.ev_ab, hipEventDisableTiming)); HIP_CHECK(hipEventCreateWithFlags(&ln.ev_fs, hipEventDisableTiming)); HIP_CHECK(hipEventCreateWithFlags(&ln.ev_b2, hipEventDisableTiming)); HIP_CHECK(hipEventCreateWithFlags(&ln.ev_s2, hipEventDisableTiming));
    ln.h_in.alloc(176 * B); ln.h_rs.alloc(64 * B); ln.h_glv.alloc(2 * MSM_FEW_PROOFS); ln.h_out.alloc(256 * B); ln.h_flags.alloc((B + 3) / 4 * 4); ln.h_status.alloc(B); ln.h_words.alloc(56);
    ln.d_clk.alloc(48); HIP_CHECK(hipMemsetAsync(ln.d_clk.p, 0, 48 * 8, ln.stream));
    ln.d_inputs.alloc(176 * B); ln.d_rs.alloc(64 * B); ln.d_out.alloc(256 * B); ln.d_flags.alloc((B + 3) / 4 * 4); ln.d_status.alloc(B); ln.d_fsync.alloc(2); ln.d_glv.alloc(2 * MSM_FEW_PROOFS);
    HIP_CHECK(hipMemsetAsync(ln.d_out.p, 0, ln.d_out.bytes(), ln.stream)); HIP_CHECK(hipMemsetAsync(ln.d_flags.p, 0, ln.d_flags.bytes(), ln.stream));
    HIP_CHECK(hipMemsetAsync(ln.d_status.p, 0, ln.d_status.bytes(), ln.stream)); HIP_CHECK(hipMemsetAsync(ln.d_fsync.p, 0, ln.d_fsync.bytes(), ln.stream));
    ln.d_W.alloc((n_wires + 4) * B); ln.d_A.alloc(domain_n * B); ln.d_B.alloc(domain_n * B); ln.d_C.alloc((domain_n + 1) * B);
    if (small.ok) {
        ln.d_W8.alloc((size_t)small.rows_per_group * B); ln.d_A8.alloc(n_constraints * B); ln.d_B8.alloc(n_constraints * B); ln.d_C8.alloc(n_constraints * B); ln.d_wsflag.alloc(1);
        HIP_CHECK(hipMemsetAsync(ln.d_wsflag.p, 0, 4, ln.stream));
        launch_wit_mark_wide(ln.d_A8.p, n_constraints, n_constraints, ws_cls_a.p, B, ln.stream); launch_wit_mark_wide(ln.d_B8.p, n_constraints, n_constraints, ws_cls_b.p, B, ln.stream);
        launch_wit_mark_wide(ln.d_C8.p, n_constraints, n_constraints, ws_cls_c.p, B, ln.stream);
        HIP_CHECK(hipGetLastError());
    }
    size_t p1 = 0, p1b = 0, p2 = 0, p2b = 0, dg = 0, dgz = 0, sj2 = 0, gk = 0; size_t sj1[Lane::NSETS] = {0, 0, 0, 0, 0, 0, 0, 0};
    auto need = [&](auto& m, size_t b, size_t& pa, size_t& pb, size_t& sj) {
        for (int latency = 0; latency <= (b == 64 ? 1 : 0); latency++) {
            const MsmGeometry g = msm_geometry(m.shape(), b, latency != 0, msm_opts);
            pa = std::max(pa, g.pa); pb = std::max(pb, g.pb); sj = std::max(sj, g.sj); dg = std::max(dg, g.digit_words); gk = std::max(gk, g.gok_bytes);
        }
    };
    MsmSet<G1Aff>* g1sets[Lane::NSETS] = {&mA, &mB1, &mK, &mZ, &mPed, &mPedSigma, &mZfew, &mC};
    ln.need_at.clear();
    for (size_t b = 64; b <= B; b += 64) {
        for (int k = 0; k < Lane::NSETS; k++) if (g1sets[k] != &mZfew || b == 64) {
            if (fuse_z_digits && g1sets[k] == &mZ) { const size_t keep = dg; dg = 0; need(mZ, b, p1, p1b, sj1[k]); if (dg > dgz) dgz = dg; dg = keep; }
            else need(*g1sets[k], b, p1, p1b, sj1[k]);
        }
        need(mB2, b, p2, p2b, sj2);
        Lane::ScratchNeed nd;
        nd.part1a = p1 * sizeof(G1Xyzz); nd.part1b = p1b * sizeof(G1Xyzz); nd.part2a = p2 * sizeof(G2Xyzz); nd.part2b = p2b * sizeof(G2Xyzz);
        nd.digits = (fuse_z_digits ? dgz : dg) * sizeof(uint4); nd.digits_w = fuse_z_digits ? (dg ? dg : 1) * sizeof(uint4) : 0; nd.gok = gk ? gk : 1; nd.sj2 = (sj2 ? sj2 : 1) * sizeof(G2Xyzz);
        for (int k = 0; k < Lane::NSETS; k++) nd.sj1[k] = (sj1[k] ? sj1[k] : 1) * sizeof(G1Xyzz);
        ln.need_at.push_back(nd);
    }
    if (fuse_z_digits) { ln.d_digits_w.alloc(dg ? dg : 1); dg = dgz; }
    ln.d_part1a.alloc(p1); ln.d_part1b.alloc(p1b); ln.d_part2a.alloc(p2); ln.d_part2b.alloc(p2b);
    ln.d_digits.alloc(dg); ln.d_gok.alloc(gk ? gk : 1);
    {
        size_t dgs = 1, gks = 1, ps = 1;
        for (const MsmSet<G1Aff>* m : {&mA, &mB1}) {
            const size_t noct = (m->nflat + 7) / 8, nsl = (noct + 63) / 64, noctw = m->few_wide ? (m->few_wide->nflat + 7) / 8 : 0, nslw = (noctw + 63) / 64;
            if (noct * 64 > dgs) dgs = noct * 64;
            if (noctw * 64 > dgs) dgs = noctw * 64;
            if (m->nbit / 8 * MSM_FEW_PROOFS > gks) gks = m->nbit / 8 * MSM_FEW_PROOFS;
            if ((nsl + nslw) * 64 > ps) ps = (nsl + nslw) * 64;
        }
        { const size_t o1 = (mB2.nflat + 7) / 8, o2 = mB2.few_wide ? (mB2.few_wide->nflat + 7) / 8 : 0; ln.d_digits_s2.alloc((o1 > o2 ? o1 : o2) * 64 + 1); }
        ln.d_gok_s2.alloc(mB2.nbit / 8 * MSM_FEW_PROOFS + 1);
        ln.d_digits_s.alloc(dgs); ln.d_gok_s.alloc(gks); ln.d_part1c.alloc(ps); ln.d_part1d.alloc((ps / 64 + MSM_REDUCE_FANIN - 1) / MSM_REDUCE_FANIN * 64 + 64);
    }
    for (int k = 0; k < Lane::NSETS; k++) { ln.d_sj1[k].alloc(sj1[k] ? sj1[k] : 1); ln.d_flat1[k].alloc(g1sets[k]->nflat && g1sets[k]->nwide ? B : 1); }
    ln.d_sj2.alloc(sj2 ? sj2 : 1); ln.d_flat2.alloc(B);
    ln.d_sumA.alloc(B); ln.d_sumB1.alloc(B); ln.d_sumK.alloc(B); ln.d_sumZ.alloc(B); ln.d_sumC.alloc(B); ln.d_sumB2.alloc(B); ln.d_tmp.alloc(2 * B);
    if (has_commitment) {
        ln.d_mask_in.alloc(32 * B); ln.d_mask.alloc(B); ln.d_commit.alloc(B); ln.d_cpts.alloc(128 * B); ln.d_sumD.alloc(B); ln.d_sumPok.alloc(B);
        ln.h_mask.alloc(32 * B); ln.h_cpts.alloc(128 * B);
        HIP_CHECK(hipMemsetAsync(ln.d_cpts.p, 0, ln.d_cpts.bytes(), ln.stream));
    }
    ln.regions.clear();
    ln.reg(WR_INPUTS, ln.d_inputs); ln.reg(WR_RS, ln.d_rs); ln.reg(WR_GLV, ln.d_glv); ln.reg(WR_MASK_IN, ln.d_mask_in); ln.reg(WR_MASK, ln.d_mask); ln.reg(WR_COMMIT, ln.d_commit);
    ln.reg(WR_SUM_D, ln.d_sumD); ln.reg(WR_SUM_POK, ln.d_sumPok);
    ln.reg(WR_W, ln.d_W); ln.reg(WR_A, ln.d_A); ln.reg(WR_B, ln.d_B); ln.reg(WR_C, ln.d_C); ln.reg(WR_W8, ln.d_W8); ln.reg(WR_A8, ln.d_A8); ln.reg(WR_B8, ln.d_B8); ln.reg(WR_C8, ln.d_C8);
    ln.reg(WR_PART1A, ln.d_part1a); ln.reg(WR_PART1B, ln.d_part1b); ln.reg(WR_PART2A, ln.d_part2a); ln.reg(WR_PART2B, ln.d_part2b); ln.reg(WR_PART1C, ln.d_part1c); ln.reg(WR_PART1D, ln.d_part1d);
    ln.reg(WR_DIGITS, ln.d_digits); ln.reg(WR_DIGITS_W, ln.d_digits_w); ln.reg(WR_DIGITS_S, ln.d_digits_s); ln.reg(WR_DIGITS_S2, ln.d_digits_s2);
    ln.reg(WR_GOK, ln.d_gok); ln.reg(WR_GOK_S, ln.d_gok_s); ln.reg(WR_GOK_S2, ln.d_gok_s2);
    for (int k = 0; k < Lane::NSETS; k++) { ln.reg(WR_SJ1 + k, ln.d_sj1[k]); ln.reg(WR_FLAT1 + k, ln.d_flat1[k]); }
    ln.reg(WR_SJ2, ln.d_sj2); ln.reg(WR_FLAT2, ln.d_flat2);
    ln.reg(WR_SUM_A, ln.d_sumA); ln.reg(WR_SUM_B1, ln.d_sumB1); ln.reg(WR_SUM_K, ln.d_sumK); ln.reg(WR_SUM_Z, ln.d_sumZ); ln.reg(WR_SUM_C, ln.d_sumC); ln.reg(WR_SUM_B2, ln.d_sumB2); ln.reg(WR_TMP, ln.d_tmp);
    ln.reg(WR_OUT, ln.d_out); ln.reg(WR_FLAGS, ln.d_flags); ln.reg(WR_STATUS, ln.d_status); ln.reg(WR_CPTS, ln.d_cpts); ln.reg(WR_CLK, ln.d_clk); ln.reg(WR_FSYNC, ln.d_fsync); ln.reg(WR_WSFLAG, ln.d_wsflag);
    wipe_whole(ln, ln.stream);
    HIP_CHECK(hipStreamSynchronize(ln.stream));
}
}
```

gnark-symmetric-crypto_amd/csrc/k_quot_bases.hip:

```cpp
#include "kernels.hpp"
#include "bn254_fp29.hpp"
#include "verify_dev.hpp"
#include "group_idft.hpp"

namespace gsc {
using namespace bn254;

namespace {

__device__ __forceinline__ fe9 qb_to_fp29(const fe& old_mont) { return Fp29::to_mont(Fp29::unpack(Fp::from_mont(old_mont))); }
__device__ __forceinline__ fe qb_from_fp29(const fe9& m) { return Fp::to_mont(Fp29::pack(Fp29::from_mont(m))); }

__device__ __forceinline__ fe qb_fr_pow(const fe& a, uint32_t e) {
    fe acc = Fr::one(); bool started = false;
    for (int i = 31; i >= 0; i--) {
        if (started) acc = Fr::sqr(acc);
        if ((e >> i) & 1) { acc = started ? Fr::mul(acc, a) : a; started = true; }
    }
    return acc;
}

__device__ __forceinline__ fe qb_zeta(int L) {
    fe c; const uint32_t w[8] = {0x725b19f0u, 0x9bd61b6eu, 0x41112ed4u, 0x402d111eu, 0x8ef62abcu, 0x00e0a7ebu, 0xa58a7e85u, 0x2a3c09f0u};
    for (int i = 0; i < 8; i++) c.l[i] = w[i];
    fe z = Fr::to_mont(c);
    for (int t = 0; t < 27 - L; t++) z = Fr::sqr(z);
    return z;
}

template <class F>
__device__ __noinline__ Xyzz9<F> qb_scalar_mul(const Xyzz9<F>& P, const fe& k) {
    using C = Curve9<F>;
    Xyzz9<F> acc = C::infinity();
    int top = 255;
    while (top >= 0 && !((k.l[top >> 5] >> (top & 31)) & 1u)) top--;
    for (int i = top; i >= 0; i--) {
// ... 127 lines not shown
    G1x::store_xyzz(dst, qb_scalar_mul(G1x::from_aff(P), Fr::from_mont(lam[pos - (m - 1)])));
}

__global__ __launch_bounds__(64) void k_qfd_pointwise(const fe* What, uint32_t n, int L, int mode, fe* Y) {
    const uint32_t k = blockIdx.x * blockDim.x + threadIdx.x;
    if (k >= n) return;
    fe s; uint32_t src = k;
    if (mode == 0) { s = qb_fr_pow(qb_zeta(L), n - 1 - k); src = (k + 1) & (n - 1); }
    else {
        const fe half = Fr::inv(Fr::from_u32(2));
        s = k ? Fr::sub(Fr::mul(Fr::from_u32(n + 1), half), Fr::from_u32(k)) : Fr::neg(Fr::mul(Fr::from_u32(n - 1), half));
    }
    const Xyzz9<Fp29f> p = G1x::load_xyzz(What + 4 * (size_t)src);
    G1x::store_xyzz(Y + 4 * (size_t)(__brev(k) >> (32 - L)), qb_scalar_mul(p, Fr::from_mont(s)));
}

__global__ __launch_bounds__(64) void k_qfd_finish(const fe* Ax, const fe* Gy, const uint32_t* perm, uint32_t n, uint32_t m, const fe* node, const fe* weight,
                                                   const Aff<Fp>* U, const uint8_t* stU, const Aff<Fp>* V, const uint8_t* stV, Aff<Fp>* U2, uint8_t* stU2, Aff<Fp>* V2, uint8_t* stV2) {
    const uint32_t p = blockIdx.x * blockDim.x + threadIdx.x;
    if (p >= 2 * m - 1) return;
    const bool on_coset = p >= m;
    const uint32_t o = on_coset ? p - m : p, i = on_coset ? perm[o] : p, at = (n - i) & (n - 1);
    const fe s = on_coset ? Fr::mul(weight[p], Fr::inv(Fr::mul(Fr::from_u32(n), node[p]))) : Fr::neg(Fr::mul(weight[p], Fr::inv(Fr::from_u32(2))));
    Xyzz9<Fp29f> q = qb_scalar_mul(G1x::load_xyzz((on_coset ? Gy : Ax) + 4 * (size_t)at), Fr::from_mont(s));
    const Aff<Fp>& b = on_coset ? V[o] : U[o];
    if ((on_coset ? stV[o] : stU[o]) != 2) q = G1x::add(q, G1x::from_aff(Aff9<Fp29f>{qb_to_fp29(b.x), qb_to_fp29(b.y)}));
    Aff<Fp>* out = on_coset ? V2 + o : U2 + o; uint8_t* st = on_coset ? stV2 + o : stU2 + o;
    if (q.inf) { *st = 2; *out = Aff<Fp>{Fp::zero(), Fp::zero()}; return; }
    const Aff9<Fp29f> a = G1x::to_aff(q);
    *out = Aff<Fp>{qb_from_fp29(a.x), qb_from_fp29(a.y)};
    *st = 0;
}

__global__ __launch_bounds__(64) void k_qfd_from_be(const uint8_t* be, const uint8_t* flags, uint32_t n, Aff<Fp>* out, uint8_t* status) {
    const uint32_t i = blockIdx.x * blockDim.x + threadIdx.x;
    if (i >= n) return;
    fe xy[2] = {fe{}, fe{}};
    for (int c = 0; c < 2; c++) for (int k = 0; k < 32; k++) xy[c].l[7 - k / 4] |= (uint32_t)be[64 * (size_t)i + 32 * c + k] << (8 * (3 - k % 4));
    const bool inf = flags[i] != 0;
    out[i] = inf ? Aff<Fp>{Fp::zero(), Fp::zero()} : Aff<Fp>{Fp::to_mont(xy[0]), Fp::to_mont(xy[1])};
    status[i] = inf ? 2 : 0;
}
__global__ __launch_bounds__(64) void k_qfd_to_be(const Aff<Fp>* in, const uint8_t* status, uint32_t n, uint8_t* be, uint8_t* flags) {
    const uint32_t i = blockIdx.x * blockDim.x + threadIdx.x;
    if (i >= n) return;
    const bool inf = status[i] == 2;
    fe xy[2] = {fe{}, fe{}};
    if (!inf) { xy[0] = Fp::from_mont(in[i].x); xy[1] = Fp::from_mont(in[i].y); }
    flags[i] = inf ? 1 : 0;
    for (int c = 0; c < 2; c++) for (int k = 0; k < 32; k++) be[64 * (size_t)i + 32 * c + k] = (uint8_t)(xy[c].l[7 - k / 4] >> (8 * (3 - k % 4)));
}

}

size_t quot_fold_dft_scratch_bytes(int L, uint32_t m) {
    const size_t n = (size_t)1 << L, nj = n - m + 1;
    return (2 + n + n / 2 + 2 * (2 * (size_t)m - 1) + 2 * nj) * sizeof(fe) + 3 * n * sizeof(G1Xyzz);
}
static void launch_quot_fold_weights(const fe* omega, const uint32_t* perm, int L, uint32_t m, fe* pw, fe* node, fe* weight, fe* yj, fe* lam, hipStream_t s) {
    const uint32_t n = 1u << L;
    hipLaunchKernelGGL(k_qf_powers, dim3((n + 63) / 64), dim3(64), 0, s, omega, perm, n, L, m, pw, yj);
    hipLaunchKernelGGL(k_qf_weights, dim3((m + n + 63) / 64), dim3(64), 0, s, pw, perm, n, L, m, node, weight, yj, lam);
}
void launch_quot_fold_dft(int L, uint32_t m, const uint32_t* perm, const G1Aff* U, const uint8_t* stU, const G1Aff* V, const uint8_t* stV,
                          G1Aff* U2, uint8_t* stU2, G1Aff* V2, uint8_t* stV2, void* scratch, hipStream_t s, hipEvent_t weights_done) {
    const uint32_t n = 1u << L, hn = n / 2, nj = n - m + 1, ncols = 2 * m - 1, blocks = (n + 63) / 64;
    fe* cst = static_cast<fe*>(scratch); fe* pw = cst + 2; fe* tw = pw + n; fe* node = tw + hn; fe* weight = node + ncols; fe* yj = weight + ncols; fe* lam = yj + nj;
    fe* What = lam + nj; fe* Ax = What + 4 * (size_t)n; fe* Gy = Ax + 4 * (size_t)n;
    hipLaunchKernelGGL(k_qfd_consts, dim3(1), dim3(64), 0, s, L, cst);
    launch_quot_fold_weights(cst, perm, L, m, pw, node, weight, yj, lam, s);
    if (weights_done) (void)hipEventRecord(weights_done, s);
    hipLaunchKernelGGL(k_qb_twiddles, dim3((hn + 63) / 64), dim3(64), 0, s, cst + 1, hn, tw);
    auto transform = [&](fe* Y) { for (int st = 0; st < L; st++) hipLaunchKernelGGL(k_qb_stage<Fp29f>, dim3((hn + 63) / 64), dim3(64), 0, s, Y, hn, L, st, tw); };
    hipLaunchKernelGGL(k_qfd_load, dim3(blocks), dim3(64), 0, s, reinterpret_cast<const Aff<Fp>*>(V), stV, perm, n, L, m, lam, What);
    transform(What);
    hipLaunchKernelGGL(k_qfd_pointwise, dim3(blocks), dim3(64), 0, s, What, n, L, 0, Ax);
    hipLaunchKernelGGL(k_qfd_pointwise, dim3(blocks), dim3(64), 0, s, What, n, L, 1, Gy);
    transform(Ax);
    transform(Gy);
    hipLaunchKernelGGL(k_qfd_finish, dim3((ncols + 63) / 64), dim3(64), 0, s, Ax, Gy, perm, n, m, node, weight, reinterpret_cast<const Aff<Fp>*>(U), stU,
                       reinterpret_cast<const Aff<Fp>*>(V), stV, reinterpret_cast<Aff<Fp>*>(U2), stU2, reinterpret_cast<Aff<Fp>*>(V2), stV2);
}
void launch_g1_aff_from_be(const uint8_t* be, const uint8_t* flags, size_t n, G1Aff* out, uint8_t* status, hipStream_t s) {
    if (n) hipLaunchKernelGGL(k_qfd_from_be, dim3((unsigned)((n + 63) / 64)), dim3(64), 0, s, be, flags, (uint32_t)n, reinterpret_cast<Aff<Fp>*>(out), status);
}
void launch_g1_aff_to_be(const G1Aff* in, const uint8_t* status, size_t n, uint8_t* be, uint8_t* flags, hipStream_t s) {
    if (n) hipLaunchKernelGGL(k_qfd_to_be, dim3((unsigned)((n + 63) / 64)), dim3(64), 0, s, reinterpret_cast<const Aff<Fp>*>(in), status, (uint32_t)n, be, flags);
}

void launch_g1_sum_be(const G1Xyzz* a, const G1Xyzz* b, size_t n, uint8_t* out, uint8_t* flags, hipStream_t s) {
    if (n) hipLaunchKernelGGL(k_qf_sum_be, dim3((unsigned)((n + 63) / 64)), dim3(64), 0, s, reinterpret_cast<const fe*>(a), reinterpret_cast<const fe*>(b), (uint32_t)n, out, flags);
}

size_t group_idft_scratch_bytes(int L, bool g2) { const size_t n = (size_t)1 << L; return (2 + n / 2) * sizeof(fe) + n * (g2 ? sizeof(G2Xyzz) : sizeof(G1Xyzz)); }
template <class P, class F> static void group_idft(const P* in, int L, void* scratch, P* out, hipStream_t s) {
    const uint32_t n = 1u << L, hn = n / 2;
    fe* cst = static_cast<fe*>(scratch); fe* tw = cst + 2; fe* Y = tw + hn;
    hipLaunchKernelGGL(k_qfd_consts, dim3(1), dim3(64), 0, s, L, cst);
    hipLaunchKernelGGL(k_qb_twiddles, dim3((hn + 63) / 64), dim3(64), 0, s, cst + 1, hn, tw);
    hipLaunchKernelGGL((k_gt_load<P, F>), dim3((n + 63) / 64), dim3(64), 0, s, in, n, L, Y);
    for (int st = 0; st < L; st++) hipLaunchKernelGGL(k_qb_stage<F>, dim3((hn + 63) / 64), dim3(64), 0, s, Y, hn, L, st, tw);
    hipLaunchKernelGGL((k_gt_finish<P, F>), dim3((n + 63) / 64), dim3(64), 0, s, (const fe*)Y, n, out);
}
void launch_group_idft(const vfy::VP1* in, int L, void* scratch, vfy::VP1* out, hipStream_t s) { group_idft<vfy::VP1, Fp29f>(in, L, scratch, out, s); }
void launch_group_idft(const vfy::VP2* in, int L, void* scratch, vfy::VP2* out, hipStream_t s) { group_idft<vfy::VP2, Fp2x>(in, L, scratch, out, s); }

void launch_quot_bases(const G1Aff* zfile, const uint8_t* zstatus, int L, int mode, const fe* omega_inv, const fe* n_inv,
                       fe* tw, G1Xyzz* scratch, const uint32_t* perm, G1Aff* out, uint8_t* status, hipStream_t s) {
    const uint32_t n = 1u << L, hn = n / 2;
    fe* Y = reinterpret_cast<fe*>(scratch);
    hipLaunchKernelGGL(k_qb_twiddles, dim3((hn + 63) / 64), dim3(64), 0, s, omega_inv, hn, tw);
    hipLaunchKernelGGL(k_qb_load, dim3((n + 63) / 64), dim3(64), 0, s, reinterpret_cast<const Aff<Fp>*>(zfile), zstatus, n, L, mode, omega_inv, n_inv, Y);
    for (int st = 0; st < L; st++) hipLaunchKernelGGL(k_qb_stage<Fp29f>, dim3((hn + 63) / 64), dim3(64), 0, s, Y, hn, L, st, tw);
    hipLaunchKernelGGL(k_qb_finish, dim3((n + 63) / 64), dim3(64), 0, s, Y, n, perm, reinterpret_cast<Aff<Fp>*>(out), status);
}
// ... 3 lines not shown
```

gnark-symmetric-crypto_amd/csrc/kernels.hpp:

```cpp
#pragma once
#include "glv.hpp"
#include "msm_layout.hpp"
#include <hip/hip_runtime.h>
#include <cstdint>
#include <cstddef>
#include "bn254_dev.hpp"

namespace gsc {
using bn254::fe;
using bn254::fe2;

struct G1Aff { fe x, y; };
struct G2Aff { fe2 x, y; };
struct G1Xyzz { fe x, y, zz, zzz; };
struct G2Xyzz { fe2 x, y, zz, zzz; };

void launch_decompress_g1(const uint8_t* in, G1Aff* out, uint8_t* status, size_t n, hipStream_t s);
void launch_decompress_g2(const uint8_t* in, G2Aff* out, uint8_t* status, size_t n, hipStream_t s);
void launch_decode_raw_g1(const uint8_t* in_x, const uint8_t* in_y, G1Aff* out, uint8_t* status, size_t n, hipStream_t s);
void launch_decode_raw_g2(const uint8_t* in_x, const uint8_t* in_y, G2Aff* out, uint8_t* status, size_t n, hipStream_t s);
void launch_g2_subgroup(const G2Aff* pts, uint8_t* status, size_t n, hipStream_t s);
void launch_fp_from_mont(const fe* in, fe* out, size_t n, hipStream_t s);
void launch_fr_from_be(const uint8_t* in, fe* out, size_t n, hipStream_t s);
void launch_fr_inverse(const fe* in, fe* out, size_t n, hipStream_t s);
// ... 67 lines not shown

struct WipeDesc { uint8_t* base; uint64_t rows, pitch, width; const uint8_t* cls; uint64_t cls_period; };
constexpr uint32_t WIPE_MAX_DESCS = 64;
constexpr uint64_t WIPE_UNIT_BYTES = 4096;
constexpr unsigned WIPE_GRID_DEFAULT = 2048, WIPE_GRID_SCAN = 4096;
constexpr unsigned WIPE_GRID_BESIDE = 512;
struct WipeList { WipeDesc d[WIPE_MAX_DESCS]; uint64_t first[WIPE_MAX_DESCS + 1]; uint32_t n; };
void launch_wipe(const WipeDesc* descs, size_t n, unsigned max_blocks, hipStream_t s);
void launch_scan_idle(const WipeDesc& desc, unsigned long long* counter, hipStream_t s);
struct NttPlan { int L; const int32_t* tw_fwd; const int32_t* tw_inv; const fe* scale_mid; const fe* scale_out; const fe* half_c; const int32_t* qr;
                 unsigned long long* clk = nullptr;
                 const int32_t* tw_inv_plain = nullptr; const fe* scale_mid_plain = nullptr; };
constexpr int NTT_QMAX = 512;
constexpr int NTT_MIN_LOG2 = 15, NTT_MAX_LOG2 = 17;
hipError_t launch_compute_h(const NttPlan& p, fe* a, fe* b, fe* c, size_t m, size_t batch, hipStream_t s, size_t ncols = 0, const NttNarrow* narrow = nullptr);
hipError_t launch_compute_d(const NttPlan& p, fe* a, fe* b, size_t m, size_t batch, hipStream_t s, size_t ncols = 0, const NttNarrow* narrow = nullptr, size_t live = 0);
struct QuotDigits { uint4* digits; int c, nwin; };
hipError_t launch_compute_d_digits(const NttPlan& p, fe* a, fe* b, size_t m, size_t batch, const QuotDigits& qd, hipStream_t s, const NttNarrow* narrow = nullptr, size_t live = 0);
inline uint32_t quot_digit_index(int L, uint32_t t) {
    const int Lhi = (L + 1) / 2, Llo = L - Lhi; const uint32_t quarter = (1u << Lhi) / 4;
    const uint32_t kq = t & 3, m = t >> 2, u4 = m % quarter, g = m / quarter;
    return ((u4 + kq * quarter) << Llo) + g;
}
inline uint32_t quot_live_tiles(int L, size_t live) {
    const int Lhi = (L + 1) / 2, Llo = L - Lhi; const size_t G = (size_t)1 << Lhi, all = (size_t)1 << Llo;
    const size_t tiles = live ? (live + G - 1) / G : all;
    return (uint32_t)(tiles < 1 ? 1 : tiles > all ? all : tiles);
}
void launch_quot_bases(const G1Aff* zfile, const uint8_t* zstatus, int L, int mode, const fe* omega_inv, const fe* n_inv,
                       fe* tw, G1Xyzz* scratch, const uint32_t* perm, G1Aff* out, uint8_t* status, hipStream_t s);
size_t quot_fold_dft_scratch_bytes(int L, uint32_t m);
void launch_quot_fold_dft(int L, uint32_t m, const uint32_t* perm, const G1Aff* U, const uint8_t* stU, const G1Aff* V, const uint8_t* stV,
                          G1Aff* U2, uint8_t* stU2, G1Aff* V2, uint8_t* stV2, void* scratch, hipStream_t s, hipEvent_t weights_done = nullptr);
void launch_g1_aff_from_be(const uint8_t* be, const uint8_t* flags, size_t n, G1Aff* out, uint8_t* status, hipStream_t s);
void launch_g1_aff_to_be(const G1Aff* in, const uint8_t* status, size_t n, uint8_t* be, uint8_t* flags, hipStream_t s);
void launch_g1_sum_be(const G1Xyzz* a, const G1Xyzz* b, size_t n, uint8_t* out, uint8_t* flags, hipStream_t s);

void launch_build_rows(const G1Aff* bases, const MsmRowSeg* segs, size_t nsegs, uint32_t cap, G1Aff* table, G1Xyzz* scratch, hipStream_t s);
void launch_build_rows(const G2Aff* bases, const MsmRowSeg* segs, size_t nsegs, uint32_t cap, G2Aff* table, G2Xyzz* scratch, hipStream_t s);
void launch_shift_bases(const G1Aff* in, const uint32_t* src, const uint32_t* shift, size_t n, G1Aff* out, hipStream_t s);
void launch_shift_bases(const G2Aff* in, const uint32_t* src, const uint32_t* shift, size_t n, G2Aff* out, hipStream_t s);

constexpr int MSM_MAX_WINDOW = 17;
struct MsmRecodeArgs {
    const fe* scalars; const uint32_t* rows;
    int mont;
    size_t nbases, batch; int c, nwin;
    uint4* digits;
};
void launch_msm_recode(const MsmRecodeArgs& a, hipStream_t s);
inline int msm_windows(int c) {
    int nwin = (254 + c - 1) / c;
    const int top_bits = 254 - c * (nwin - 1);
    const unsigned long long lead = 0xc19139cb84c680a6ull;
    const unsigned long long top = lead >> (64 - top_bits);
    if (top + 1 > (1ull << (c - 1)) - 1) nwin++;
    return nwin;
}
struct MsmWinArgs {
    const void* table; int c, nwin; size_t nbases;
    const uint4* digits; size_t batch;
    size_t nslices, per;
    void* partial;
    unsigned long long* clk = nullptr;
    uint32_t exp_entry_mask = 0;
    size_t digit_bases = 0;
// ... 52 lines not shown
```

gnark-symmetric-crypto_amd/csrc/msm_set.hip:

```cpp
#include "msm_set.hpp"

namespace gsc {

namespace {

template <class AffT, class XyzzT>
void build_rows(const AffT* bases, const std::vector<uint64_t>& off, const std::vector<uint32_t>& len, AffT* table, hipStream_t stream) {
    const uint32_t cap = 256;
    const std::vector<MsmRowSeg> segs = msm_row_segments(off, len, cap);
    if (segs.empty()) return;
    size_t chunk = ((size_t)4 << 30) / (cap * sizeof(XyzzT)); if (chunk > segs.size()) chunk = segs.size();
    DevBuf<XyzzT> scratch(chunk * cap); DevBuf<MsmRowSeg> d_segs(segs.size());
    d_segs.upload(segs.data(), segs.size(), stream);
    for (size_t t0 = 0; t0 < segs.size(); t0 += chunk) launch_build_rows(bases, d_segs.p + t0, segs.size() - t0 < chunk ? segs.size() - t0 : chunk, cap, table, scratch.p, stream);
    HIP_CHECK(hipGetLastError());
    HIP_CHECK(hipStreamSynchronize(stream));
}

template <class AffT, class XyzzT>
void build_subset(const AffT* b, size_t ng, AffT* t, uint8_t* ok, hipStream_t stream) {
    size_t chunk = ((size_t)2 << 30) / (MSM_GROUP_ENTRIES * sizeof(XyzzT)); if (chunk > ng) chunk = ng;
    DevBuf<XyzzT> sc(chunk * MSM_GROUP_ENTRIES);
    for (size_t g0 = 0; g0 < ng; g0 += chunk) launch_build_subset(b + 8 * g0, ng - g0 < chunk ? ng - g0 : chunk, t + g0 * MSM_GROUP_ENTRIES, sc.p, ok + g0, stream);
    HIP_CHECK(hipStreamSynchronize(stream));
}

template <class XyzzT>
void reduce_slices(const MsmRun<XyzzT>& r, size_t nslices, size_t cols, XyzzT* out, std::vector<std::pair<size_t, bool>>* levels) {
    XyzzT* src = r.pa; XyzzT* alt = r.pb; size_t ns = nslices;
    for (;;) {
        const size_t groups = r.latency ? (ns + 63) / 64 : msm_reduce_groups(ns, cols);
        XyzzT* dst = groups == 1 ? out : alt;
        if (levels) levels->emplace_back(ns, !r.latency && msm_reduce_by_proof(ns, cols));
        if (r.latency) launch_msm_reduce_few(src, ns, cols, r.B, r.n_real, dst, r.ctx.stream);
        else launch_msm_reduce(src, ns, cols, dst, r.ctx.stream);
        if (groups == 1) break;
        XyzzT* t = src; src = dst; alt = t; ns = groups;
    }
}

}

template <class AffT, class XyzzT>
void msm_build_tables(MsmSet<AffT>& set, const AffT* bases, const MsmFlatPlan& plan, const std::vector<uint32_t>& rows, int c, hipStream_t stream, size_t* table_bytes) {
    const std::vector<uint32_t>&src = plan.src, &shift = plan.shift, &frows = plan.frows, &len = plan.len, &wide = plan.wide; const std::vector<int32_t>& octwin = plan.octwin;
    const size_t D = (size_t)1 << (c - 1);
    set.c = c; set.nwin = msm_windows(c);
    if (plan.nexpanded) { set.cv = plan.cv; set.nexpanded = plan.nexpanded; }
    set.nflat = src.size(); set.nbit = plan.nbit;
    if (set.nflat) {
        DevBuf<AffT> fb(set.nflat); DevBuf<uint32_t> d_src(set.nflat), d_shift(set.nflat);
        d_src.upload(src.data(), src.size(), stream); d_shift.upload(shift.data(), shift.size(), stream);
        launch_shift_bases(bases, d_src.p, d_shift.p, set.nflat, fb.p, stream);
        std::vector<uint64_t> off; const size_t entries = msm_row_offsets(len, off);
        set.ftable.alloc(entries); *table_bytes += set.ftable.bytes();
        set.rowoff.alloc(set.nflat); set.rowlen.alloc(set.nflat); set.frows.alloc(set.nflat); set.octwin.alloc(octwin.size());
        set.rowoff.upload(off.data(), set.nflat, stream); set.rowlen.upload(len.data(), set.nflat, stream);
        set.frows.upload(frows.data(), set.nflat, stream); set.octwin.upload(octwin.data(), octwin.size(), stream);
        build_rows<AffT, XyzzT>(fb.p, off, len, set.ftable.p, stream);
        if (set.nbit) {
            const size_t ng = set.nbit / 8;
            set.sub.alloc(ng * MSM_GROUP_ENTRIES); set.group_ok.alloc(ng);
            *table_bytes += set.sub.bytes();
            build_subset<AffT, XyzzT>(fb.p, ng, set.sub.p, set.group_ok.p, stream);
        }
        HIP_CHECK(hipGetLastError());
        HIP_CHECK(hipStreamSynchronize(stream));
    }
    set.nwide = wide.size();
    if (set.nwide) {
        DevBuf<AffT> wb(set.nwide); DevBuf<uint32_t> d_src(set.nwide), d_shift(set.nwide);
        std::vector<uint32_t> zero(set.nwide, 0u), wrows(set.nwide);
        for (size_t i = 0; i < set.nwide; i++) wrows[i] = rows[wide[i]];
        d_src.upload(wide.data(), set.nwide, stream); d_shift.upload(zero.data(), set.nwide, stream);
        launch_shift_bases(bases, d_src.p, d_shift.p, set.nwide, wb.p, stream);
        set.wrows.alloc(set.nwide); set.wrows.upload(wrows.data(), set.nwide, stream);
        set.wtable.alloc(set.nwide * D); *table_bytes += set.wtable.bytes();
        std::vector<uint64_t> off(set.nwide); std::vector<uint32_t> wlen(set.nwide, (uint32_t)D);
        for (size_t i = 0; i < set.nwide; i++) off[i] = i * D;
        build_rows<AffT, XyzzT>(wb.p, off, wlen, set.wtable.p, stream);
        HIP_CHECK(hipGetLastError());
        HIP_CHECK(hipStreamSynchronize(stream));
    }
}

template <class AffT, class XyzzT>
void msm_run(const MsmSet<AffT>& set, const MsmRun<XyzzT>& r, MsmHornerJobs& pending) {
    const MsmCtx& ctx = r.ctx;
    const size_t B = r.B;
    const MsmGeometry g = msm_geometry(set.shape(), B, r.latency, r.opts);
    std::vector<std::pair<size_t, bool>>* const flat_levels = r.levels ? &r.levels->flat : nullptr;
    auto flat_few = [&](const MsmSet<AffT>& m, size_t nslices, XyzzT* out, bool stamp) {
        if (!m.nflat) return;
        MsmFlatRecodeArgs ra{r.scalars, m.frows.p, m.octwin.p, m.nflat, B, m.cv, ctx.digits, m.nbit, m.group_ok.p, ctx.gok, r.wires ? 1 : 0, ctx.plane, ctx.plane_rows, ctx.plane_stride};
        launch_msm_recode_flat_few(ra, r.n_real, ctx.stream);
        MsmFlatArgs a{m.ftable.p, m.rowoff.p, m.rowlen.p, m.nflat, ctx.digits, B, nslices, g.flat_per, out, m.nbit, m.sub.p, ctx.gok, r.scalars, m.frows.p};
        if (stamp && r.ev_begin) HIP_CHECK(hipEventRecord(r.ev_begin, ctx.stream));
        launch_msm_flat_few<AffT>(a, r.n_real, ctx.stream);
        if (stamp && r.ev_end) HIP_CHECK(hipEventRecord(r.ev_end, ctx.stream));
    };
    if (r.latency && set.few_wide) {
        const size_t own = g.flat_slices - g.few_wide_slices;
        flat_few(set, own, r.pa, true);
        flat_few(*set.few_wide, g.few_wide_slices, r.pa + own * B, false);
        reduce_slices(r, g.flat_slices, B, r.sum, flat_levels);
        return;
    }
    if (set.nflat) {
        if (r.latency) flat_few(set, g.flat_slices, r.pa, true);
        else {
            MsmFlatRecodeArgs ra{r.scalars, set.frows.p, set.octwin.p, set.nflat, B, set.cv, ctx.digits, set.nbit, set.group_ok.p, ctx.gok, r.wires ? 1 : 0, ctx.plane, ctx.plane_rows, ctx.plane_stride};
            launch_msm_recode_flat(ra, ctx.stream);
            MsmFlatArgs a{set.ftable.p, set.rowoff.p, set.rowlen.p, set.nflat, ctx.digits, B, g.flat_slices, g.flat_per, r.pa, set.nbit, set.sub.p, ctx.gok, r.scalars, set.frows.p};
            launch_msm_flat<AffT>(a, ctx.stream);
        }
        reduce_slices(r, g.flat_slices, B, set.nwide ? r.flat : r.sum, flat_levels);
    }
    if (set.nwide) {
        uint4* const digits = r.win_digits ? r.win_digits : ctx.digits;
        MsmRecodeArgs ra{r.scalars, set.wrows.p, r.wires ? 1 : 0, set.nwide, B, set.c, set.nwin, digits};
        if (!r.digits_ready) launch_msm_recode(ra, ctx.stream);
        MsmWinArgs a{set.wtable.p, set.c, set.nwin, set.nwide, digits, B, g.win_slices, g.win_per, r.pa, r.clk, r.clk_mask,
                     r.digits_ready ? set.digit_bases : 0};
        if (r.ev_begin) HIP_CHECK(hipEventRecord(r.ev_begin, ctx.stream));
        if (r.latency) launch_msm_win_few<AffT>(a, r.n_real, ctx.stream);
        else launch_msm_win<AffT>(a, ctx.stream);
        if (r.ev_end) HIP_CHECK(hipEventRecord(r.ev_end, ctx.stream));
        reduce_slices(r, g.win_slices, g.sj, r.sj, r.levels ? &r.levels->win : nullptr);
        if (pending.n >= MSM_HORNER_JOBS) throw std::runtime_error("internal: too many pending Horner passes");
        pending.job[pending.n++] = MsmHornerJob{r.sj, set.nflat ? r.flat : (XyzzT*)nullptr, r.sum, set.nwin, set.c};
    }
    if (!set.nflat && !set.nwide) HIP_CHECK(hipMemsetAsync(r.sum, 0, B * sizeof(XyzzT), ctx.stream));
}

template void msm_build_tables<G1Aff, G1Xyzz>(MsmSet<G1Aff>&, const G1Aff*, const MsmFlatPlan&, const std::vector<uint32_t>&, int, hipStream_t, size_t*);
template void msm_build_tables<G2Aff, G2Xyzz>(MsmSet<G2Aff>&, const G2Aff*, const MsmFlatPlan&, const std::vector<uint32_t>&, int, hipStream_t, size_t*);
template void msm_run<G1Aff, G1Xyzz>(const MsmSet<G1Aff>&, const MsmRun<G1Xyzz>&, MsmHornerJobs&);
template void msm_run<G2Aff, G2Xyzz>(const MsmSet<G2Aff>&, const MsmRun<G2Xyzz>&, MsmHornerJobs&);

}
```

gnark-symmetric-crypto_amd/csrc/msm_set.hpp:

```cpp
#pragma once
#include "kernels.hpp"
#include "solver_tables.hpp"
#include <memory>
#include <utility>
#include <vector>

namespace gsc {

template <class AffT>
struct MsmSet {
    size_t nbases = 0;
    DevBuf<AffT> wtable; DevBuf<uint32_t> wrows; size_t nwide = 0; int c = 0, nwin = 0;
    size_t digit_bases = 0;
    DevBuf<AffT> ftable; DevBuf<uint64_t> rowoff; DevBuf<uint32_t> rowlen; DevBuf<uint32_t> frows; DevBuf<int32_t> octwin;
    size_t nflat = 0, nbit = 0, nexpanded = 0; int cv = 0; DevBuf<AffT> sub; DevBuf<uint8_t> group_ok;
    std::unique_ptr<MsmSet<AffT>> few_wide;
    bool latency_flat() const { return !nwide || few_wide; }
    MsmShape shape() const { return MsmShape{nflat, nbit, nwide, c, nwin, digit_bases, few_wide ? few_wide->nflat : 0}; }
};

template <class AffT, class XyzzT>
void msm_build_tables(MsmSet<AffT>& set, const AffT* bases, const MsmFlatPlan& plan, const std::vector<uint32_t>& rows, int c, hipStream_t stream, size_t* table_bytes);

struct MsmLevels { std::vector<std::pair<size_t, bool>> flat, win; };

struct MsmCtx { hipStream_t stream; uint4* digits; uint8_t* gok; const int8_t* plane = nullptr; size_t plane_rows = 0, plane_stride = 0; };

template <class XyzzT>
struct MsmRun {
    MsmCtx ctx;
    const fe* scalars; bool wires;
    size_t B, n_real; bool latency;
    XyzzT *pa, *pb, *sj, *flat, *sum;
    bool digits_ready = false;
    hipEvent_t ev_begin = nullptr, ev_end = nullptr;
    unsigned long long* clk = nullptr; uint32_t clk_mask = 0;
    MsmLaunchOpts opts;
    uint4* win_digits = nullptr;
    MsmLevels* levels = nullptr;
};
template <class AffT, class XyzzT>
void msm_run(const MsmSet<AffT>& set, const MsmRun<XyzzT>& run, MsmHornerJobs& pending);

}
```

gnark-symmetric-crypto_amd/csrc/wipe_plan.hpp:

```cpp
#pragma once
#include "chunk_route.hpp"
#include <cstdint>
#include <vector>

namespace gsc {

enum WipeRegion : int {
    WR_INPUTS, WR_RS, WR_GLV, WR_MASK_IN, WR_MASK, WR_COMMIT, WR_SUM_D, WR_SUM_POK,
    WR_W, WR_A, WR_B, WR_C, WR_W8, WR_A8, WR_B8, WR_C8,
    WR_PART1A, WR_PART1B, WR_PART2A, WR_PART2B, WR_PART1C, WR_PART1D,
    WR_DIGITS, WR_DIGITS_W, WR_DIGITS_S, WR_DIGITS_S2, WR_GOK, WR_GOK_S, WR_GOK_S2,
    WR_SJ1, WR_SJ1_LAST = WR_SJ1 + 7, WR_FLAT1, WR_FLAT1_LAST = WR_FLAT1 + 7, WR_SJ2, WR_FLAT2,
    WR_SUM_A, WR_SUM_B1, WR_SUM_K, WR_SUM_Z, WR_SUM_C, WR_SUM_B2, WR_TMP,
    WR_OUT, WR_FLAGS, WR_STATUS, WR_CPTS, WR_CLK, WR_FSYNC, WR_WSFLAG,
    WR_COUNT
};
constexpr int WR_FIRST_PUBLIC = WR_OUT;
inline bool wipe_region_public(int r) { return r >= WR_FIRST_PUBLIC; }
inline const char* wipe_region_name(int r) {
    static const char* const names[WR_COUNT] = {
        "inputs", "rs", "glv", "mask_in", "mask", "commit", "sumD", "sumPok",
        "W", "A", "B", "C", "W8", "A8", "B8", "C8",
        "part1a", "part1b", "part2a", "part2b", "part1c", "part1d",
        "digits", "digits_w", "digits_s", "digits_s2", "gok", "gok_s", "gok_s2",
        "sj1.A", "sj1.B1", "sj1.K", "sj1.Z", "sj1.Ped", "sj1.PedSigma", "sj1.Zfew", "sj1.C",
        "flat1.A", "flat1.B1", "flat1.K", "flat1.Z", "flat1.Ped", "flat1.PedSigma", "flat1.Zfew", "flat1.C", "sj2", "flat2",
        "sumA", "sumB1", "sumK", "sumZ", "sumC", "sumB2", "tmp",
        "out", "flags", "status", "cpts", "clk", "fsync", "wsflag"};
    return r >= 0 && r < WR_COUNT ? names[r] : "?";
}

enum WipeStage : int { WS_UPLOAD, WS_WITNESS, WS_QUOTIENT, WS_WIRE_SUMS, WS_Z_SUM, WS_POK_SUM, WS_HORNER, WS_ASSEMBLY };
constexpr int WIPE_PHASE_A_TRIGGER = WS_WIRE_SUMS;

inline int wipe_last_touch(int r, const ChunkRoute& rt, const RouteFacts& f) {
    switch (r) {
    case WR_INPUTS: return WS_WITNESS;
    case WR_MASK_IN: case WR_MASK: case WR_COMMIT: case WR_SUM_D: return f.has_commitment ? WS_WITNESS : WS_UPLOAD;
    case WR_W: case WR_W8: return f.has_commitment ? WS_POK_SUM : WS_WIRE_SUMS;
    case WR_A: return rt.z_digits_ready ? WS_QUOTIENT : WS_Z_SUM;
    case WR_B: case WR_A8: case WR_B8: return WS_QUOTIENT;
    case WR_C: case WR_C8: return rt.eval ? WS_WIRE_SUMS : WS_QUOTIENT;
    case WR_DIGITS_W: return f.has_commitment ? WS_POK_SUM : WS_WIRE_SUMS;
    case WR_DIGITS: case WR_PART1A: case WR_PART1B: case WR_GOK: return f.has_commitment ? WS_POK_SUM : WS_Z_SUM;
    case WR_PART2A: case WR_PART2B: case WR_SJ2: case WR_FLAT2: return WS_ASSEMBLY;
    case WR_SUM_POK: return f.has_commitment ? WS_HORNER : WS_UPLOAD;
    case WR_GLV: case WR_PART1C: case WR_PART1D: case WR_DIGITS_S: case WR_DIGITS_S2: case WR_GOK_S: case WR_GOK_S2: return WS_UPLOAD;
    default: break;
    }
    if (r >= WR_SJ1 && r <= WR_FLAT1_LAST) return WS_HORNER;
    return WS_ASSEMBLY;
}

struct WipeRegionInfo { int region; uint64_t bytes; };

struct WipeSizes {
    uint64_t B = 0, n = 0;
    uint64_t n_wires = 0, n_constraints = 0, domain_n = 0, rows_per_group = 0;
    uint64_t fe_bytes = 32, xyzz1_bytes = 0, xyzz2_bytes = 0;
    uint64_t part1a = 0, part1b = 0, part2a = 0, part2b = 0, digits = 0, digits_w = 0, gok = 0, sj1[8] = {0, 0, 0, 0, 0, 0, 0, 0}, sj2 = 0;
};

struct WipeItem { int region; uint64_t offset, rows, pitch, width; bool image; uint64_t image_period; };
struct WipePlan { std::vector<WipeItem> a, b; };

namespace wipe_detail {
inline uint64_t alloc_of(const std::vector<WipeRegionInfo>& table, int r) { for (const auto& t : table) if (t.region == r) return t.bytes; return 0; }
inline void prefix(std::vector<WipeItem>& out, const std::vector<WipeRegionInfo>& table, int r, uint64_t bytes) {
    const uint64_t have = alloc_of(table, r);
    if (bytes > have) bytes = have;
    if (bytes) out.push_back(WipeItem{r, 0, 1, bytes, bytes, false, 0});
}
inline void plane(std::vector<WipeItem>& out, const std::vector<WipeRegionInfo>& table, int r, uint64_t rows_per_group, uint64_t groups, bool image) {
    uint64_t rows = rows_per_group * groups; const uint64_t have = alloc_of(table, r) / 64;
    if (rows > have) rows = have;
    if (!rows) return;
    if (image) out.push_back(WipeItem{r, 0, rows, 64, 64, true, rows_per_group});
    else out.push_back(WipeItem{r, 0, 1, rows * 64, rows * 64, false, 0});
}
}

inline WipePlan wipe_plan(const ChunkRoute& rt, const RouteFacts& f, const WipeSizes& z, const std::vector<WipeRegionInfo>& table) {
    using namespace wipe_detail;
    WipePlan p;
    const uint64_t B = z.B, fe = z.fe_bytes, x1 = z.xyzz1_bytes, x2 = z.xyzz2_bytes;
    auto phase = [&](int r) -> std::vector<WipeItem>& { return !rt.latency && wipe_last_touch(r, rt, f) <= WIPE_PHASE_A_TRIGGER ? p.a : p.b; };
    prefix(phase(WR_W), table, WR_W, (z.n_wires + 4) * B * fe);
    const bool cols = rt.latency && rt.resident && z.n < B;
    auto matrix = [&](int r, uint64_t rows) {
        if (!alloc_of(table, r)) return;
        if (cols) phase(r).push_back(WipeItem{r, 0, rows, B * fe, z.n * fe, false, 0});
        else prefix(phase(r), table, r, rows * B * fe);
    };
    matrix(WR_A, z.domain_n); matrix(WR_B, z.domain_n); matrix(WR_C, z.domain_n + 1);
    if (rt.small) {
        plane(phase(WR_W8), table, WR_W8, z.rows_per_group, B / 64, false);
        for (int r : {WR_A8, WR_B8, WR_C8}) plane(phase(r), table, r, z.n_constraints, B / 64, true);
    }
    prefix(phase(WR_DIGITS_W), table, WR_DIGITS_W, z.digits_w);
    if (!(rt.latency && rt.use_zfew && alloc_of(table, WR_DIGITS_W))) prefix(p.b, table, WR_DIGITS, z.digits);
    prefix(p.b, table, WR_GOK, z.gok);
    prefix(p.b, table, WR_PART1A, z.part1a); prefix(p.b, table, WR_PART1B, z.part1b); prefix(p.b, table, WR_PART2A, z.part2a); prefix(p.b, table, WR_PART2B, z.part2b);
    for (int k = 0; k < 8; k++) { prefix(p.b, table, WR_SJ1 + k, z.sj1[k]); prefix(p.b, table, WR_FLAT1 + k, B * x1); }
    prefix(p.b, table, WR_SJ2, z.sj2); prefix(p.b, table, WR_FLAT2, B * x2);
    for (int r : {WR_SUM_A, WR_SUM_B1, WR_SUM_K, WR_SUM_Z, WR_SUM_C}) prefix(p.b, table, r, B * x1);
    prefix(p.b, table, WR_SUM_B2, B * x2); prefix(p.b, table, WR_TMP, 2 * B * x1);
    prefix(p.b, table, WR_INPUTS, 176 * B); prefix(p.b, table, WR_RS, 64 * B);
    if (f.has_commitment) {
        prefix(p.b, table, WR_MASK_IN, 32 * B); prefix(p.b, table, WR_MASK, B * fe); prefix(p.b, table, WR_COMMIT, B * fe);
        prefix(p.b, table, WR_SUM_D, B * x1); prefix(p.b, table, WR_SUM_POK, B * x1);
    }
    if (rt.latency)
        for (int r : {WR_GLV, WR_PART1C, WR_PART1D, WR_DIGITS_S, WR_DIGITS_S2, WR_GOK_S, WR_GOK_S2}) prefix(p.b, table, r, alloc_of(table, r));
    return p;
}

inline std::vector<WipeItem> wipe_plan_whole(const std::vector<WipeRegionInfo>& table, uint64_t n_constraints) {
    std::vector<WipeItem> out;
    for (const auto& t : table) {
        if (wipe_region_public(t.region) || !t.bytes) continue;
        if (t.region == WR_A8 || t.region == WR_B8 || t.region == WR_C8) out.push_back(WipeItem{t.region, 0, t.bytes / 64, 64, 64, true, n_constraints});
        else out.push_back(WipeItem{t.region, 0, 1, t.bytes, t.bytes, false, 0});
    }
    return out;
}

}
```

include/libprove.h:

```cpp
#ifndef GSC_LIBPROVE_H
#define GSC_LIBPROVE_H
#include <stddef.h>
#include <stdint.h>
#ifdef __cplusplus
extern "C" {
#endif

typedef unsigned char GoUint8;
typedef long long GoInt;
typedef struct { void *data; GoInt len; GoInt cap; } GoSlice;
struct Prove_return { void *r0;  GoInt r1;  };

extern void enforce_binding(void);

extern GoUint8 InitAlgorithm(GoUint8 algorithmID, GoSlice provingKey, GoSlice r1cs);

extern void Free(void *pointer);

extern struct Prove_return Prove(GoSlice params);


extern struct Prove_return ProveBatch(GoSlice params);

extern long long gsc_prove_raw(GoUint8 cipher, const uint8_t *inputs, size_t n, uint8_t *proofs, uint32_t *proof_lens, uint8_t *ciphertexts);

extern int gsc_setup(GoSlice r1cs, const uint8_t *seed32, void **pk, size_t *pk_len, void **vk, size_t *vk_len);


extern int gsc_set_deterministic_randomness(const uint8_t *r_be32, const uint8_t *s_be32, const uint8_t *mask_be32);

extern long long gsc_debug_prove(GoSlice params);
extern long long gsc_debug_vector(int which, uint8_t *out, size_t cap);

extern int gsc_debug_field_ops(int field, int op, const uint8_t *a, const uint8_t *b, uint8_t *out, size_t n, int chain);

extern int gsc_debug_limb_ops(int field, int op, const int32_t *a, const int32_t *b, const int32_t *c, const int32_t *d, int32_t *out, size_t n);

extern int gsc_debug_curve_ops(int group, int op, const uint8_t *pts, const uint8_t *inf, const uint8_t *lam, size_t n, size_t k, uint8_t *out, uint8_t *flags);

extern int gsc_debug_decode_points(int group, const uint8_t *bytes, size_t len, size_t n, uint8_t *out_xy, uint8_t *status);

extern int gsc_debug_tower_ops(int path, int op, const int32_t *in, size_t n, int32_t *out, uint8_t *flags);

extern long long gsc_debug_compute_h(GoUint8 algorithmID, const uint8_t *abc_be, size_t m, uint8_t *h_out, size_t cap);
extern long long gsc_debug_compute_d(GoUint8 algorithmID, const uint8_t *ab_be, size_t m, uint8_t *d_out, size_t cap);
extern int gsc_debug_clock_trace(uint32_t n, uint32_t interval_us, unsigned long long *out);
extern long long gsc_debug_secret_residue(GoUint8 algorithmID);
extern int gsc_debug_z_sum(GoUint8 algorithmID, const uint8_t *abc_be, size_t m, uint8_t *out, uint8_t *flags);
extern long long gsc_debug_secret_scan(GoUint8 algorithmID, char *out, size_t cap);
extern int gsc_debug_wipe(uint64_t bytes, int fill, const uint64_t *desc, size_t ndesc, const uint8_t *cls, size_t ncls, uint8_t *buf_out,
                          const uint64_t *win, size_t nwin, uint64_t *counts, float *ms);
extern int gsc_debug_quot_fold_dft(int L, uint32_t m, const uint32_t *perm, const uint8_t *u_be, const uint8_t *u_inf, const uint8_t *v_be, const uint8_t *v_inf,
                                   uint8_t *u2_be, uint8_t *u2_inf, uint8_t *v2_be, uint8_t *v2_inf);
extern int gsc_debug_glv_split(const uint8_t *k, uint8_t *out);

extern size_t gsc_describe(GoUint8 algorithmID, char *out, size_t cap);
extern int gsc_last_stage_ms(GoUint8 algorithmID, float out[4]);
extern int gsc_last_dominant_kernel(GoUint8 algorithmID, char *name, size_t cap, float *ms, size_t *statements, size_t *columns, size_t *nbases);
extern int gsc_last_kernel_clock(GoUint8 algorithmID, float *clock_mhz, int *windows);

extern int gsc_verify_init(GoUint8 algorithmID, GoSlice verifyingKey);
extern long long gsc_verify_raw(GoUint8 algorithmID, const uint8_t *proofs, const uint32_t *proof_lens, const uint8_t *signals, size_t n,
                                uint8_t *verdicts);
extern struct Prove_return VerifyBatch(GoSlice params);
extern long long gsc_debug_pairing(const uint8_t *g1_uncompressed, const uint8_t *g2_uncompressed, size_t n, uint8_t *out);
extern long long gsc_verify_raw_batched(GoUint8 algorithmID, const uint8_t *proofs, const uint32_t *proof_lens, const uint8_t *signals,
                                        size_t n, uint8_t *verdicts);
extern int gsc_verify_all(GoUint8 algorithmID, const uint8_t *proofs, const uint32_t *proof_lens, const uint8_t *signals, size_t n);
extern GoUint8 VerifyAll(GoSlice params);
extern long long gsc_verify_claims(GoUint8 algorithmID, const uint8_t *proofs, const uint32_t *proof_lens, const uint8_t *signals, size_t n,
                                   const uint64_t *claim_ends, size_t m, uint8_t *verdicts);
extern struct Prove_return VerifyClaims(GoSlice params);
extern int gsc_debug_verify_randomizers(const uint8_t *seed32, int all_ones);
extern GoUint8 gsc_verify_json(GoSlice params);
extern int gsc_verify_last_path(GoUint8 algorithmID);
extern int gsc_debug_verify_path(int mode);
extern long long gsc_debug_pairing_few(const uint8_t *g1_uncompressed, const uint8_t *g2_uncompressed, size_t n, uint8_t *out);

extern int gsc_prove_check_init(GoUint8 algorithmID, GoSlice verifyingKey);
extern int gsc_prove_check_stats(GoUint8 algorithmID, uint64_t out[4]);
extern int gsc_debug_prove_corrupt(GoUint8 algorithmID, uint32_t index, int which, int mode);

extern GoUint8 gsc_release_algorithm(GoUint8 algorithmID);
extern int gsc_replace_algorithm(GoUint8 algorithmID, GoSlice provingKey, GoSlice r1cs, GoSlice verifyingKey);
extern int gsc_memory_info(int device, uint64_t out[4]);
extern uint64_t gsc_key_generation(GoUint8 algorithmID);
// ... 78 lines not shown
```

Baseline: 29270 proofs/s.

## Fold the C-matrix quotient MSM bases into the K bases at setup

Adds a setup-time fold that combines the evaluation-form C-column bases with the matching K (private wire) bases, so the per-proof C MSM disappears and its contribution rides in the K MSM. Wires not covered by K become residual slots and a delta-row slot is added. The C wire-sum buffers are dropped from the wipe plan when folding is active. This removes one batched MSM per proof, at the cost of a larger folded K set and a more complex setup path that is on by default through GSC_C_FOLD.

```diff
diff --git a/gnark-symmetric-crypto_amd/__init__.py b/gnark-symmetric-crypto_amd/__init__.py
--- a/gnark-symmetric-crypto_amd/__init__.py
+++ b/gnark-symmetric-crypto_amd/__init__.py
@@ -12,7 +12,7 @@
 ALGORITHM_NAMES = {0: "chacha20", 1: "aes-128-ctr", 2: "aes-256-ctr"}
 
 EXPORTS = ["enforce_binding", "InitAlgorithm", "Free", "Prove", "ProveBatch", "gsc_prove_raw", "gsc_setup",
-           "gsc_set_deterministic_randomness", "gsc_debug_prove", "gsc_debug_vector", "gsc_describe", "gsc_last_stage_ms", "gsc_last_dominant_kernel", "gsc_last_kernel_clock", "gsc_debug_field_ops", "gsc_debug_limb_ops", "gsc_debug_curve_ops", "gsc_debug_decode_points", "gsc_debug_tower_ops", "gsc_debug_compute_h", "gsc_debug_compute_d", "gsc_debug_z_sum", "gsc_debug_quot_fold_dft", "gsc_debug_secret_residue", "gsc_debug_secret_scan", "gsc_debug_wipe", "gsc_debug_clock_trace", "gsc_debug_glv_split",
+           "gsc_set_deterministic_randomness", "gsc_debug_prove", "gsc_debug_vector", "gsc_describe", "gsc_last_stage_ms", "gsc_last_dominant_kernel", "gsc_last_kernel_clock", "gsc_debug_field_ops", "gsc_debug_limb_ops", "gsc_debug_curve_ops", "gsc_debug_decode_points", "gsc_debug_tower_ops", "gsc_debug_compute_h", "gsc_debug_compute_d", "gsc_debug_z_sum", "gsc_debug_quot_fold_dft", "gsc_debug_c_fold", "gsc_debug_secret_residue", "gsc_debug_secret_scan", "gsc_debug_wipe", "gsc_debug_clock_trace", "gsc_debug_glv_split",
            "gsc_verify_init", "gsc_verify_raw", "VerifyBatch", "gsc_debug_pairing",
            "gsc_verify_raw_batched", "gsc_verify_all", "VerifyAll", "gsc_debug_verify_randomizers",
            "gsc_verify_json", "gsc_verify_last_path", "gsc_debug_verify_path", "gsc_debug_pairing_few",
@@ -739,6 +739,20 @@
     return u2.raw, f2.raw, v2.raw[:64 * (m - 1)], g2.raw[:m - 1]
 
 
+def debug_c_fold(u_be: bytes, u_inf: bytes, col_start, term_row, term_coeff, coeff_be: bytes, k_be: bytes, k_inf: bytes, k_wire):
+    lb = lib()
+    m, nw, nk, nt, nc = len(u_inf), len(col_start) - 1, len(k_inf), len(term_row), len(coeff_be) // 32
+    lb.gsc_debug_c_fold.restype = C.c_int
+    lb.gsc_debug_c_fold.argtypes = [C.c_uint32, C.c_char_p, C.c_char_p, C.c_uint32, C.c_void_p, C.c_void_p, C.c_void_p, C.c_uint32, C.c_char_p,
+                                    C.c_uint32, C.c_char_p, C.c_char_p, C.c_void_p] + [C.c_void_p] * 4
+    assert len(u_be) == 64 * m and len(k_be) == 64 * nk and len(k_wire) == nk and len(term_coeff) == nt and len(coeff_be) == 32 * nc and nw >= 1
+    u32 = lambda v: (C.c_uint32 * max(len(v), 1))(*v)
+    uh, uf, k2, kf = C.create_string_buffer(64 * nw), C.create_string_buffer(nw), C.create_string_buffer(64 * max(nk, 1)), C.create_string_buffer(max(nk, 1))
+    if lb.gsc_debug_c_fold(m, u_be, u_inf, nw, u32(col_start), u32(term_row), u32(term_coeff), nc, coeff_be, nk, k_be, k_inf, u32(k_wire), uh, uf, k2, kf) != 0:
+        raise RuntimeError("gsc_debug_c_fold failed")
+    return uh.raw, uf.raw, k2.raw[:64 * nk], kf.raw[:nk]
+
+
 def verify_init(algorithm_id: int, verifying_key: bytes) -> bool:
     s, keep = _slice(verifying_key)
     return bool(lib().gsc_verify_init(algorithm_id, s))
diff --git a/gnark-symmetric-crypto_amd/csrc/c_fold.hpp b/gnark-symmetric-crypto_amd/csrc/c_fold.hpp
--- /dev/null
+++ b/gnark-symmetric-crypto_amd/csrc/c_fold.hpp
@@ -0,0 +1,49 @@
+#pragma once
+#include "srs_columns.hpp"
+#include "host_field.hpp"
+
+namespace gsc {
+namespace cfold {
+
+constexpr uint32_t NONE = 0xFFFFFFFFu;
+
+inline srs::Matrix o_columns(const R1csFile& cs) {
+    srs::Matrix M[3];
+    srs::build_matrices(cs, M);
+    return std::move(M[2]);
+}
+
+inline srs::CoeffTable coeff_table(const R1csFile& cs) {
+    const size_t nc = cs.n_coeff();
+    std::vector<uint8_t> be(32 * (nc ? nc : 1), 0);
+    for (size_t i = 0; i < nc; i++) { hostf::Fr c; memcpy(c.v.w, cs.coeff_limbs.data() + 8 * i, 32); c.to_be(&be[32 * i]); }
+    srs::CoeffTable t;
+    if (!srs::prepare_coeffs(be.data(), nc, t)) throw std::runtime_error("r1cs: a coefficient that is not below r");
+    return t;
+}
+
+struct Slots {
+    std::vector<uint32_t> slot_wire, slot_k, row;
+    size_t n_k = 0;
+    std::vector<uint32_t> residual;
+    size_t size() const { return row.size(); }
+};
+inline Slots plan_slots(const std::vector<uint32_t>& col_start, const std::vector<uint32_t>& k_wire, uint32_t delta_row) {
+    if (col_start.empty()) throw std::runtime_error("c fold: no column offsets");
+    const size_t nw = col_start.size() - 1;
+    std::vector<uint8_t> in_k(nw, 0);
+    Slots s; s.n_k = k_wire.size();
+    for (size_t j = 0; j < k_wire.size(); j++) {
+        if (k_wire[j] >= nw || in_k[k_wire[j]]++) throw std::runtime_error("c fold: a K point's wire is out of range or named twice");
+        s.slot_wire.push_back(k_wire[j]); s.slot_k.push_back((uint32_t)j); s.row.push_back(k_wire[j]);
+    }
+    s.slot_wire.push_back(NONE); s.slot_k.push_back((uint32_t)k_wire.size()); s.row.push_back(delta_row);
+    for (size_t w = 0; w < nw; w++) if (!in_k[w] && col_start[w + 1] > col_start[w]) {
+        s.residual.push_back((uint32_t)w);
+        s.slot_wire.push_back((uint32_t)w); s.slot_k.push_back(NONE); s.row.push_back((uint32_t)w);
+    }
+    return s;
+}
+
+}
+}
diff --git a/gnark-symmetric-crypto_amd/csrc/capi.cpp b/gnark-symmetric-crypto_amd/csrc/capi.cpp
--- a/gnark-symmetric-crypto_amd/csrc/capi.cpp
+++ b/gnark-symmetric-crypto_amd/csrc/capi.cpp
@@ -690,6 +690,15 @@
     catch (const std::exception& e) { printf("%s\n", e.what()); return -1; }
 }
 
+int gsc_debug_c_fold(uint32_t m, const uint8_t* u_be, const uint8_t* u_inf, uint32_t n_wires, const uint32_t* col_start, const uint32_t* term_row, const uint32_t* term_coeff,
+                     uint32_t n_coeff, const uint8_t* coeff_be, uint32_t n_k, const uint8_t* k_be, const uint8_t* k_inf, const uint32_t* k_wire,
+                     uint8_t* uhat_be, uint8_t* uhat_inf, uint8_t* k2_be, uint8_t* k2_inf) {
+    if (hooks_refused("gsc_debug_c_fold") || !n_wires || m > (1u << 20) || n_wires > (1u << 20) || n_k > (1u << 20) || n_coeff > (1u << 20) || !u_be || !u_inf || !col_start || !term_row || !term_coeff
+        || !coeff_be || !k_be || !k_inf || !k_wire || !uhat_be || !uhat_inf || !k2_be || !k2_inf) return -1;
+    try { debug_c_fold(config_from_env().device, m, u_be, u_inf, n_wires, col_start, term_row, term_coeff, n_coeff, coeff_be, n_k, k_be, k_inf, k_wire, uhat_be, uhat_inf, k2_be, k2_inf); return 0; }
+    catch (const std::exception& e) { printf("%s\n", e.what()); return -1; }
+}
+
 size_t gsc_describe(GoUint8 algorithmID, char* out, size_t cap) {
     if (algorithmID > 2 || !cap) return 0;
     const Snapshot snap = snapshot(algorithmID); Algorithm* a = algo_of(snap);
diff --git a/gnark-symmetric-crypto_amd/csrc/chunk_route.hpp b/gnark-symmetric-crypto_amd/csrc/chunk_route.hpp
--- a/gnark-symmetric-crypto_amd/csrc/chunk_route.hpp
+++ b/gnark-symmetric-crypto_amd/csrc/chunk_route.hpp
@@ -9,6 +9,7 @@
     bool quotient_eval = false, fuse_z_digits = false;
     bool zfew_flat = false;
     bool a_flat = false, b1_flat = false, b2_flat = false;
+    bool c_fold = false;
 };
 struct RouteCall {
     bool dbg = false;
@@ -27,6 +28,7 @@
     bool eval = false;
     bool z_digits_ready = false;
     bool overlap_q = false;
+    bool c_fold = false;
     const char* kernel_name = "";
 };
 
@@ -44,6 +46,7 @@
     r.use_zfew = r.latency && f.zfew_flat;
     r.eval = f.quotient_eval && !r.use_zfew;
     r.z_digits_ready = r.eval && f.fuse_z_digits && !r.latency;
+    r.c_fold = r.eval && f.c_fold && !r.latency;
     r.overlap_q = r.z_digits_ready && !call.dbg && (cfg.overlap_quotient == 2 || (cfg.overlap_quotient && B < OVERLAP_QUOTIENT_BELOW));
     r.kernel_name = !r.latency ? "k_msm_win<Fp29f>"
                   : r.small ? "k_wit_chain + k_wit_rows"
diff --git a/gnark-symmetric-crypto_amd/csrc/engine.hip b/gnark-symmetric-crypto_amd/csrc/engine.hip
--- a/gnark-symmetric-crypto_amd/csrc/engine.hip
+++ b/gnark-symmetric-crypto_amd/csrc/engine.hip
@@ -49,6 +49,7 @@
     c.quotient_fold = env_int("GSC_QUOTIENT_FOLD", 1);
     if (c.quotient_fold < 0 || c.quotient_fold > 2) throw std::runtime_error("GSC_QUOTIENT_FOLD must be 0, 1 or 2");
     c.quotient_live_tiles = env_int("GSC_QUOTIENT_LIVE_TILES", 1) ? 1 : 0;
+    c.c_fold = env_int("GSC_C_FOLD", 1) ? 1 : 0;
     c.small_witness = env_int("GSC_SMALL_WITNESS", 1);
     c.small_witness_few = env_int("GSC_SMALL_WITNESS_FEW", 1);
     c.ntt_plain = env_int("GSC_NTT_PLAIN", 1) ? 1 : 0;
@@ -183,6 +184,40 @@
     HIP_CHECK(hipDeviceSynchronize());
     HIP_CHECK(hipMemcpy(u2_be, d_out.p, 64 * (size_t)m, hipMemcpyDeviceToHost)); HIP_CHECK(hipMemcpy(u2_inf, d_flags.p, m, hipMemcpyDeviceToHost));
     if (m > 1) { HIP_CHECK(hipMemcpy(v2_be, d_out.p + 64 * (size_t)m, 64 * (size_t)(m - 1), hipMemcpyDeviceToHost)); HIP_CHECK(hipMemcpy(v2_inf, d_flags.p + m, m - 1, hipMemcpyDeviceToHost)); }
+}
+
+void debug_c_fold(int device, uint32_t m, const uint8_t* u_be, const uint8_t* u_inf, uint32_t n_wires, const uint32_t* col_start, const uint32_t* term_row, const uint32_t* term_coeff,
+                  uint32_t n_coeff, const uint8_t* coeff_be, uint32_t n_k, const uint8_t* k_be, const uint8_t* k_inf, const uint32_t* k_wire,
+                  uint8_t* uhat_be, uint8_t* uhat_inf, uint8_t* k2_be, uint8_t* k2_inf) {
+    if (col_start[0] != 0) throw std::runtime_error("gsc_debug_c_fold: column offsets must start at 0");
+    for (uint32_t w = 0; w < n_wires; w++) if (col_start[w + 1] < col_start[w] || col_start[w + 1] > (1u << 24)) throw std::runtime_error("gsc_debug_c_fold: column offsets decrease or are too large");
+    const size_t n_terms = col_start[n_wires];
+    srs::Matrix O; O.col_start.assign(col_start, col_start + n_wires + 1); O.row.assign(term_row, term_row + n_terms); O.coeff.assign(term_coeff, term_coeff + n_terms);
+    srs::CoeffTable ct;
+    if (!srs::prepare_coeffs(coeff_be, n_coeff, ct)) throw std::runtime_error("gsc_debug_c_fold: a coefficient that is not below r");
+    std::vector<uint32_t> slot_wire(n_wires + (size_t)n_k), slot_k(n_wires + (size_t)n_k);
+    for (uint32_t w = 0; w < n_wires; w++) { slot_wire[w] = w; slot_k[w] = cfold::NONE; }
+    for (uint32_t j = 0; j < n_k; j++) { slot_wire[n_wires + j] = k_wire[j]; slot_k[n_wires + j] = j; }
+    const size_t n_slots = slot_wire.size();
+    use_device(device);
+    DevBuf<uint8_t> d_be(((size_t)m + n_k) * 64 + 1), d_inf((size_t)m + n_k + 1), d_stU(m ? m : 1), d_stK(n_k ? n_k : 1), d_st(n_slots), d_out(n_slots * 64), d_flags(n_slots);
+    DevBuf<G1Aff> d_U(m ? m : 1), d_K(n_k ? n_k : 1), d_res(n_slots);
+    if (m) { HIP_CHECK(hipMemcpy(d_be.p, u_be, 64 * (size_t)m, hipMemcpyHostToDevice)); HIP_CHECK(hipMemcpy(d_inf.p, u_inf, m, hipMemcpyHostToDevice)); }
+    if (n_k) { HIP_CHECK(hipMemcpy(d_be.p + 64 * (size_t)m, k_be, 64 * (size_t)n_k, hipMemcpyHostToDevice)); HIP_CHECK(hipMemcpy(d_inf.p + m, k_inf, n_k, hipMemcpyHostToDevice)); }
+    launch_g1_aff_from_be(d_be.p, d_inf.p, m, d_U.p, d_stU.p, nullptr);
+    launch_g1_aff_from_be(d_be.p + 64 * (size_t)m, d_inf.p + m, n_k, d_K.p, d_stK.p, nullptr);
+    HIP_CHECK(hipGetLastError());
+    HIP_CHECK(hipDeviceSynchronize());
+    std::vector<uint8_t> stU(m), stK(n_k);
+    for (uint32_t i = 0; i < m; i++) stU[i] = u_inf[i] ? 2 : 0;
+    for (uint32_t j = 0; j < n_k; j++) stK[j] = k_inf[j] ? 2 : 0;
+    const std::vector<uint8_t> st = c_fold_bases(d_U.p, stU, d_K.p, stK, O, ct, slot_wire, slot_k, d_res.p, nullptr);
+    HIP_CHECK(hipMemcpy(d_st.p, st.data(), n_slots, hipMemcpyHostToDevice));
+    launch_g1_aff_to_be(d_res.p, d_st.p, n_slots, d_out.p, d_flags.p, nullptr);
+    HIP_CHECK(hipGetLastError());
+    HIP_CHECK(hipDeviceSynchronize());
+    HIP_CHECK(hipMemcpy(uhat_be, d_out.p, 64 * (size_t)n_wires, hipMemcpyDeviceToHost)); HIP_CHECK(hipMemcpy(uhat_inf, d_flags.p, n_wires, hipMemcpyDeviceToHost));
+    if (n_k) { HIP_CHECK(hipMemcpy(k2_be, d_out.p + 64 * (size_t)n_wires, 64 * (size_t)n_k, hipMemcpyDeviceToHost)); HIP_CHECK(hipMemcpy(k2_inf, d_flags.p + n_wires, n_k, hipMemcpyDeviceToHost)); }
 }
 
 float debug_wipe(int device, uint64_t bytes, int fill, const uint64_t* desc, size_t ndesc, const uint8_t* cls, size_t ncls, uint8_t* out, const uint64_t* win, size_t nwin, uint64_t* counts) {
@@ -290,7 +325,8 @@
              impl_->mA.nbases, impl_->mB1.nbases, impl_->mK.nbases, impl_->mZ.digit_bases ? impl_->mZ.digit_bases : impl_->mZ.nbases, impl_->mA.nbit, impl_->mB1.nbit, impl_->mK.nbit,
              impl_->mA.nwide, impl_->mA.nexpanded, impl_->mB1.nwide, impl_->mB1.nexpanded, impl_->mK.nwide, impl_->mK.nexpanded);
     std::string out = buf;
-    if (impl_->quotient_eval) out += std::string(" quotient=evaluation-form") + (impl_->fuse_z_digits ? "+digits" : "") + (!impl_->fuse_z_digits || !impl_->cfg.overlap_quotient ? "" : impl_->cfg.overlap_quotient == 2 ? "+beside-wire-sets" : "+beside-wire-sets(<4096)") + "(c: " + std::to_string(impl_->mC.nbit) + " grouped + " + std::to_string(impl_->mC.nflat - impl_->mC.nbit) + " flat + " + std::to_string(impl_->mC.nwide) + " windowed)";
+    if (impl_->quotient_eval) out += std::string(" quotient=evaluation-form") + (impl_->fuse_z_digits ? "+digits" : "") + (!impl_->fuse_z_digits || !impl_->cfg.overlap_quotient ? "" : impl_->cfg.overlap_quotient == 2 ? "+beside-wire-sets" : "+beside-wire-sets(<4096)") + (impl_->c_fold ? "(c: folded into K (+" + std::to_string(impl_->cfold_residual) + " wires))"
+                                                                              : "(c: " + std::to_string(impl_->mC.nbit) + " grouped + " + std::to_string(impl_->mC.nflat - impl_->mC.nbit) + " flat + " + std::to_string(impl_->mC.nwide) + " windowed Cfold=off(" + impl_->cfold_why + "))");
     else out += " quotient=coefficient-form";
     if (impl_->quotient_eval) out += impl_->mZ.digit_bases ? " Zlive=" + std::to_string(impl_->mZ.nwide) + " Zfold=dft" :" Zfold=off(" + impl_->fold_why + ")";
     if (impl_->quotient_eval) out += " Qtiles=" + std::to_string(quot_live_tiles(impl_->L, impl_->quot_live)) + "/" + std::to_string(1u << (impl_->L - (impl_->L + 1) / 2));
diff --git a/gnark-symmetric-crypto_amd/csrc/engine.hpp b/gnark-symmetric-crypto_amd/csrc/engine.hpp
--- a/gnark-symmetric-crypto_amd/csrc/engine.hpp
+++ b/gnark-symmetric-crypto_amd/csrc/engine.hpp
@@ -48,6 +48,7 @@
     int fuse_z_digits = 1;
     int quotient_fold = 1;
     int quotient_live_tiles = 1;
+    int c_fold = 1;
     int small_witness = 1;
     int ntt_plain = 1;
     int overlap_quotient = 1;
@@ -110,6 +111,9 @@
 
 void debug_quot_fold_dft(int device, int L, uint32_t m, const uint32_t* perm, const uint8_t* u_be, const uint8_t* u_inf, const uint8_t* v_be, const uint8_t* v_inf,
                          uint8_t* u2_be, uint8_t* u2_inf, uint8_t* v2_be, uint8_t* v2_inf);
+void debug_c_fold(int device, uint32_t m, const uint8_t* u_be, const uint8_t* u_inf, uint32_t n_wires, const uint32_t* col_start, const uint32_t* term_row, const uint32_t* term_coeff,
+                  uint32_t n_coeff, const uint8_t* coeff_be, uint32_t n_k, const uint8_t* k_be, const uint8_t* k_inf, const uint32_t* k_wire,
+                  uint8_t* uhat_be, uint8_t* uhat_inf, uint8_t* k2_be, uint8_t* k2_inf);
 float debug_wipe(int device, uint64_t bytes, int fill, const uint64_t* desc, size_t ndesc, const uint8_t* cls, size_t ncls, uint8_t* out, const uint64_t* win, size_t nwin, uint64_t* counts);
 void debug_clock_trace(int device, uint32_t n, uint32_t interval_us, unsigned long long* out);
 void debug_field_ops(int device, int field, int op, const uint8_t* a, const uint8_t* b, uint8_t* out, size_t n, int chain);
diff --git a/gnark-symmetric-crypto_amd/csrc/engine_impl.hpp b/gnark-symmetric-crypto_amd/csrc/engine_impl.hpp
--- a/gnark-symmetric-crypto_amd/csrc/engine_impl.hpp
+++ b/gnark-symmetric-crypto_amd/csrc/engine_impl.hpp
@@ -8,6 +8,7 @@
 #include "msm_set.hpp"
 #include "wipe_plan.hpp"
 #include "prove_check.hpp"
+#include "c_fold.hpp"
 #include <atomic>
 #include <chrono>
 #include <cstring>
@@ -44,6 +45,9 @@
 void stream_give(int device, int kind, int role, hipStream_t s);
 
 std::atomic<size_t>& prover_bytes_on(int device);
+
+std::vector<uint8_t> c_fold_bases(const G1Aff* U, const std::vector<uint8_t>& stU, const G1Aff* K, const std::vector<uint8_t>& stK, const srs::Matrix& O, const srs::CoeffTable& ct,
+                                  const std::vector<uint32_t>& slot_wire, const std::vector<uint32_t>& slot_k, G1Aff* out, hipStream_t s);
 
 class AlgorithmImpl : public SolverTables {
   public:
@@ -87,6 +91,7 @@
     size_t quot_live = 0;
     bool fold_quotient_bases(const DevBuf<G1Aff>& d_U, const std::vector<uint8_t>& stU, const DevBuf<G1Aff>& d_V, const std::vector<uint8_t>& stV, const std::vector<uint32_t>& rowsZ,
                              DevBuf<G1Aff>& d_U2, std::vector<uint8_t>& stU2, DevBuf<G1Aff>& d_V2, std::vector<uint8_t>& stV2);
+    bool c_fold = false; MsmSet<G1Aff> mKc; size_t cfold_residual = 0; std::string cfold_why = "GSC_C_FOLD=0";
     struct Lane {
         hipStream_t stream = nullptr, side = nullptr, side2 = nullptr;
         hipEvent_t ev_ab = nullptr, ev_fs = nullptr, ev_b2 = nullptr, ev_s2 = nullptr;
@@ -151,12 +156,12 @@
 
     template <class AffT, class XyzzT, class Decomp>
     void build_set(MsmSet<AffT>& set, const KeyPoints& raw, size_t point_bytes, const std::vector<uint32_t>& rows, int c, const char* what, Decomp decomp, bool uniform, int expand_cv = 0,
-                   const std::vector<uint8_t>* classes = nullptr, uint32_t zero_row = 0xFFFFFFFFu, bool latency_layout = true);
+                   const std::vector<uint8_t>* classes = nullptr, uint32_t zero_row = 0xFFFFFFFFu, bool latency_layout = true, bool batch_rows = true);
     void init_key(const R1csFile& cs, const PkFile& key);
 
     void alloc_lane(Lane& ln, size_t B);
 
-    RouteFacts route_facts() const { return RouteFacts{small.ok, has_commitment, quotient_eval, fuse_z_digits, mZfew.nflat != 0, mA.latency_flat(), mB1.latency_flat(), mB2.latency_flat()}; }
+    RouteFacts route_facts() const { return RouteFacts{small.ok, has_commitment, quotient_eval, fuse_z_digits, mZfew.nflat != 0, mA.latency_flat(), mB1.latency_flat(), mB2.latency_flat(), c_fold}; }
     struct Chunk {
         const ProofRequest* reqs; size_t n, B; DebugVectors* dbg; ChunkRoute rt;
         std::chrono::steady_clock::time_point t_start, t_enqueued, t_done;
@@ -172,7 +177,7 @@
         else if (scalars == ln.d_C.p) { c.plane = ln.d_C8.p; c.plane_rows = n_constraints; c.plane_stride = n_constraints; }
         return c;
     }
-    int set_index(const MsmSet<G1Aff>& set) const { const MsmSet<G1Aff>* all[Lane::NSETS] = {&mA, &mB1, &mK, &mZ, &mPed, &mPedSigma, &mZfew, &mC}; for (int k = 0; k < Lane::NSETS; k++) if (all[k] == &set) return k; return 0; }
+    int set_index(const MsmSet<G1Aff>& set) const { const MsmSet<G1Aff>* all[Lane::NSETS] = {&mA, &mB1, &mK, &mZ, &mPed, &mPedSigma, &mZfew, &mC}; if (&set == &mKc) return 2; for (int k = 0; k < Lane::NSETS; k++) if (all[k] == &set) return k; return 0; }
     void run_msm_g1(Lane& ln, const Chunk& ck, const MsmSet<G1Aff>& set, const fe* scalars, int mont, G1Xyzz* sum, bool timed = false, bool side = false, bool digits_ready = false);
     void run_msm_g2(Lane& ln, const Chunk& ck, const MsmSet<G2Aff>& set, const fe* scalars, int mont, G2Xyzz* sum, bool side = false);
     template <class AffT> void flush_horner(MsmHornerJobs& pending, size_t B, hipStream_t s) { launch_msm_horner<AffT>(pending, B, s); pending.n = 0; }
diff --git a/gnark-symmetric-crypto_amd/csrc/engine_prove.hip b/gnark-symmetric-crypto_amd/csrc/engine_prove.hip
--- a/gnark-symmetric-crypto_amd/csrc/engine_prove.hip
+++ b/gnark-symmetric-crypto_amd/csrc/engine_prove.hip
@@ -308,8 +308,8 @@
         flush_horner<G2Aff>(ln.pending2, B, ln.side);
     }
     HIP_CHECK(hipEventRecord(ln.ev_fs, ln.side));
-    run_msm_g1(ln, ck, mK, ln.d_W.p, 1, ln.d_sumK.p);
-    if (rt.eval) {
+    run_msm_g1(ln, ck, rt.c_fold ? mKc : mK, ln.d_W.p, 1, ln.d_sumK.p);
+    if (rt.eval && !rt.c_fold) {
         HIP_CHECK(hipMemsetAsync(ln.d_C.p + domain_n * B, 0, B * sizeof(fe), ln.stream));
         run_msm_g1(ln, ck, mC, ln.d_C.p, 1, ln.d_sumC.p);
     }
@@ -327,7 +327,7 @@
     const size_t B = ck.B; const ChunkRoute& rt = ck.rt;
     HIP_CHECK(hipStreamWaitEvent(ln.stream, ln.ev_fs, 0));
     if (rt.early_b2) HIP_CHECK(hipStreamWaitEvent(ln.stream, ln.ev_s2, 0));
-    launch_fin_combine(ln.d_sumB2.p, ln.d_sumK.p, ln.d_sumZ.p, rt.eval ? ln.d_sumC.p : nullptr, ln.d_tmp.p, B, ln.d_out.p, ln.d_flags.p, ln.stream);
+    launch_fin_combine(ln.d_sumB2.p, ln.d_sumK.p, ln.d_sumZ.p, rt.eval && !rt.c_fold ? ln.d_sumC.p : nullptr, ln.d_tmp.p, B, ln.d_out.p, ln.d_flags.p, ln.stream);
     HIP_CHECK(hipGetLastError());
     HIP_CHECK(hipEventRecord(ln.ev[4], ln.stream));
     if (ck.corrupt) {
diff --git a/gnark-symmetric-crypto_amd/csrc/engine_tables.hip b/gnark-symmetric-crypto_amd/csrc/engine_tables.hip
--- a/gnark-symmetric-crypto_amd/csrc/engine_tables.hip
+++ b/gnark-symmetric-crypto_amd/csrc/engine_tables.hip
@@ -185,7 +185,7 @@
 
 template <class AffT, class XyzzT, class Decomp>
 void AlgorithmImpl::build_set(MsmSet<AffT>& set, const KeyPoints& raw, size_t point_bytes, const std::vector<uint32_t>& rows, int c, const char* what, Decomp decomp, bool uniform, int expand_cv,
-                              const std::vector<uint8_t>* classes, uint32_t zero_row, bool latency_layout) {
+                              const std::vector<uint8_t>* classes, uint32_t zero_row, bool latency_layout, bool batch_rows) {
     const std::vector<uint8_t>& cls = classes ? *classes : row_class;
     const size_t n = raw.x.size() / point_bytes;
     if (rows.size() != n) throw std::runtime_error(std::string("pk: row map size mismatch for ") + what);
@@ -195,7 +195,7 @@
     for (size_t i = 0; i < n; i++) if (st[i] == 1) throw std::runtime_error(std::string("pk: invalid point in ") + what);
     const uint32_t ROW_ZERO = zero_row != 0xFFFFFFFFu ? zero_row : (uint32_t)(n_wires + 3);
     const MsmFlatPlan plan = msm_plan_flat(msm_sort_bases(st, rows, cls, uniform, cfg.bit_groups, cfg.row_margin_bits, NARROW_MAX_BITS), rows, ROW_ZERO, uniform, expand_cv, EXPAND_MAX, EXPAND_C, msm_windows);
-    msm_build_tables<AffT, XyzzT>(set, bases.p, plan, rows, c, stream, &table_bytes);
+    msm_build_tables<AffT, XyzzT>(set, bases.p, plan, rows, c, stream, &table_bytes, batch_rows);
     if (set.nwide && !uniform && cfg.few_path && cfg.few_wide && latency_layout) {
         const std::vector<uint32_t>& wide = plan.wide;
         KeyPoints raw_w; raw_w.x.resize(set.nwide * point_bytes); if (!raw.y.empty()) raw_w.y.resize(set.nwide * point_bytes);
@@ -232,6 +232,32 @@
     if (std::count(stV2.begin(), stV2.end(), (uint8_t)0) != (ptrdiff_t)(m - 1)) { fold_why = "a folded V base is the point at infinity"; return false; }
     fold_why.clear();
     return true;
+}
+
+std::vector<uint8_t> c_fold_bases(const G1Aff* U, const std::vector<uint8_t>& stU, const G1Aff* K, const std::vector<uint8_t>& stK, const srs::Matrix& O, const srs::CoeffTable& ct,
+                                  const std::vector<uint32_t>& slot_wire, const std::vector<uint32_t>& slot_k, G1Aff* out, hipStream_t s) {
+    const size_t m = stU.size(), nk = stK.size(), n_slots = slot_wire.size(), n_terms = O.n_terms(), n_coeff = ct.meta.size();
+    if (O.col_start.empty() || slot_k.size() != n_slots || O.coeff.size() != n_terms || ct.mag.size() != 8 * n_coeff) throw std::runtime_error("c fold: inconsistent lists");
+    const size_t nw = O.col_start.size() - 1;
+    srs::Segments sg;
+    if (m >= (1u << 28) || nw >= (1u << 28) || n_terms >= (1u << 30) || n_slots >= (1u << 28) || !srs::cut_columns(O.col_start.data(), nw, n_terms, sg)) throw std::runtime_error("c fold: column offsets that are not a partition of the terms");
+    for (size_t i = 0; i < n_terms; i++) if (O.row[i] >= m || O.coeff[i] >= n_coeff) throw std::runtime_error("c fold: a term's row or coefficient id out of range");
+    for (size_t j = 0; j < n_slots; j++) if ((slot_wire[j] != cfold::NONE && slot_wire[j] >= nw) || (slot_k[j] != cfold::NONE && slot_k[j] >= nk)) throw std::runtime_error("c fold: a slot's wire or K point out of range");
+    std::vector<uint8_t> st(n_slots);
+    if (!n_slots) return st;
+    const size_t n_segs = sg.begin.size();
+    auto dev = [&](const std::vector<uint32_t>& v, DevBuf<uint32_t>& b) { b.alloc(v.size() ? v.size() : 1); if (!v.empty()) b.upload(v.data(), v.size(), s); };
+    DevBuf<uint32_t> seg_begin, seg_end, col_seg, term_row, term_coeff, mag, meta, d_wire, d_k;
+    dev(sg.begin, seg_begin); dev(sg.end, seg_end); dev(sg.col_seg, col_seg); dev(O.row, term_row); dev(O.coeff, term_coeff); dev(ct.mag, mag); dev(ct.meta, meta); dev(slot_wire, d_wire); dev(slot_k, d_k);
+    DevBuf<uint8_t> d_stU(m ? m : 1), d_stK(nk ? nk : 1), d_st(n_slots), scratch(c_fold_scratch_bytes((uint32_t)m, (uint32_t)nw, (uint32_t)n_segs));
+    if (m) d_stU.upload(stU.data(), m, s);
+    if (nk) d_stK.upload(stK.data(), nk, s);
+    const CFoldArgs a{seg_begin.p, seg_end.p, col_seg.p, term_row.p, term_coeff.p, mag.p, meta.p, (uint32_t)n_segs, (uint32_t)nw, d_wire.p, d_k.p, (uint32_t)n_slots};
+    launch_c_fold(U, d_stU.p, (uint32_t)m, K, d_stK.p, a, scratch.p, out, d_st.p, s);
+    HIP_CHECK(hipGetLastError());
+    HIP_CHECK(hipMemcpyAsync(st.data(), d_st.p, n_slots, hipMemcpyDeviceToHost, s));
+    HIP_CHECK(hipStreamSynchronize(s));
+    return st;
 }
 
 void AlgorithmImpl::init_key(const R1csFile& cs, const PkFile& key) {
@@ -277,8 +303,18 @@
     rowsA.push_back(ROW_ONE); rowsA.push_back(ROW_R);
     std::vector<uint32_t> rowsB2 = rowsB;
     rowsB.push_back(ROW_ONE); rowsB.push_back(ROW_S); rowsB2.push_back(ROW_ONE); rowsB2.push_back(ROW_S);
+    const std::vector<uint32_t> k_wire = rowsK;
     rowsK.push_back(ROW_NRS);
     quotient_eval = cfg.quotient_eval != 0;
+    const bool want_cfold = quotient_eval && cfg.c_fold;
+    if (quotient_eval && !cfg.c_fold) cfold_why = "GSC_C_FOLD=0";
+    else if (!quotient_eval) cfold_why = "coefficient form";
+    srs::Matrix matO; srs::CoeffTable coeffO; cfold::Slots slotsKc;
+    if (want_cfold) { matO = cfold::o_columns(cs); coeffO = cfold::coeff_table(cs); slotsKc = cfold::plan_slots(matO.col_start, k_wire, ROW_NRS); }
+    int zfew_cv = 0;
+    if (cfg.few_path && cfg.few_z_gb > 0) for (int t : {8, 6, 4}) if ((double)(key.g1_Z.size() / 32) * msm_windows(t) * (double)((size_t)1 << (t - 1)) * sizeof(G1Aff) <= (double)cfg.few_z_gb * 1e9) { zfew_cv = t; break; }
+    const bool k_latency_only = !cfg.few_path || cfg.few_wide;
+    const bool c_without_fold = test_hooks_enabled() || (cfg.few_path && !zfew_cv);
     std::vector<uint32_t> rowsZ(quotient_eval ? domain_n : domain_n - 1); for (size_t i = 0; i < rowsZ.size(); i++) rowsZ[i] = quotient_eval ? quot_digit_index(L, (uint32_t)i) : (uint32_t)i;
     std::vector<uint32_t> rowsZkey(domain_n - 1); for (size_t i = 0; i < rowsZkey.size(); i++) rowsZkey[i] = (uint32_t)i;
     std::vector<uint32_t> rowsC; if (quotient_eval) { rowsC.resize(n_constraints); for (size_t i = 0; i < n_constraints; i++) rowsC[i] = (uint32_t)i; }
@@ -302,7 +338,8 @@
             return k > EXPAND_MAX ? (double)k : 0.0;
         };
         auto wide_of = [&](const std::vector<uint32_t>& rows) { return wide_in(rows, row_class); };
-        const double g1 = wide_of(rowsA) + wide_of(rowsB) + wide_of(rowsK) + 2 * wide_of(cs.commit_private) + wide_in(rowsC, row_class_c), g2 = wide_of(rowsB2);
+        const double g1 = wide_of(rowsA) + wide_of(rowsB) + (want_cfold && k_latency_only ? 0.0 : wide_of(rowsK)) + (want_cfold ? wide_of(slotsKc.row) : 0.0) + 2 * wide_of(cs.commit_private)
+                        + (!want_cfold || c_without_fold ? wide_in(rowsC, row_class_c) : 0.0), g2 = wide_of(rowsB2);
         cfg.window_w = 4;
         for (int c = 16; c >= 4; c--) if ((g1 * 64.0 + g2 * 128.0) * (double)((size_t)1 << (c - 1)) <= cfg.w_table_gb * 1e9) { cfg.window_w = c; break; }
     }
@@ -315,7 +352,32 @@
     };
     timed("G1.A", [&] { build_set<G1Aff, G1Xyzz>(mA, cat({key.g1_A, key.g1_A_y}, {{key.g1_alpha, key.g1_alpha_y}, {key.g1_delta, key.g1_delta_y}}), 32, rowsA, cfg.window_w, "G1.A", dec1, false); });
     timed("G1.B", [&] { build_set<G1Aff, G1Xyzz>(mB1, cat({key.g1_B, key.g1_B_y}, {{key.g1_beta, key.g1_beta_y}, {key.g1_delta, key.g1_delta_y}}), 32, rowsB, cfg.window_w, "G1.B", dec1, false); });
-    timed("G1.K", [&] { build_set<G1Aff, G1Xyzz>(mK, cat({key.g1_K, key.g1_K_y}, {{key.g1_delta, key.g1_delta_y}}), 32, rowsK, cfg.window_w, "G1.K", dec1, false); });
+    const KeyPoints rawK = cat({key.g1_K, key.g1_K_y}, {{key.g1_delta, key.g1_delta_y}});
+    auto from_dev = [this](const DevBuf<G1Aff>& src, const std::vector<uint8_t>& st) {
+        return [this, &src, &st](const KeyPoints& raw, G1Aff* out) {
+            const size_t n = raw.x.size() / 32;
+            HIP_CHECK(hipMemcpyAsync(out, src.p, n * sizeof(G1Aff), hipMemcpyDeviceToDevice, stream));
+            HIP_CHECK(hipStreamSynchronize(stream));
+            return std::vector<uint8_t>(st.begin(), st.begin() + n);
+        };
+    };
+    DevBuf<G1Aff> d_Kc; std::vector<uint8_t> stKc;
+    auto fold_c = [&](const DevBuf<G1Aff>& U, const std::vector<uint8_t>& st) {
+        DevBuf<G1Aff> d_K(rowsK.size()); const std::vector<uint8_t> stK = decompress_g1(rawK, d_K.p);
+        for (uint8_t v : stK) if (v == 1) throw std::runtime_error("pk: invalid point in G1.K");
+        d_Kc.alloc(slotsKc.size());
+        stKc = c_fold_bases(U.p, std::vector<uint8_t>(st.begin(), st.begin() + n_constraints), d_K.p, stK, matO, coeffO, slotsKc.slot_wire, slotsKc.slot_k, d_Kc.p, stream);
+        for (size_t j = 0; j < slotsKc.n_k; j++) if (stKc[j] == 2) { cfold_why = "a folded K base is the point at infinity"; return false; }
+        cfold_residual = 0;
+        for (size_t j = slotsKc.n_k + 1; j < stKc.size(); j++) cfold_residual += stKc[j] != 2;
+        cfold_why.clear();
+        return true;
+    };
+    auto build_K = [&] {
+        timed("G1.K", [&] { build_set<G1Aff, G1Xyzz>(mK, rawK, 32, rowsK, cfg.window_w, "G1.K", dec1, false, 0, nullptr, 0xFFFFFFFFu, true, !(c_fold && k_latency_only)); });
+        if (c_fold) timed("G1.K (c folded in)", [&] { build_set<G1Aff, G1Xyzz>(mKc, std::vector<uint8_t>(slotsKc.size() * 32, 0), 32, slotsKc.row, cfg.window_w, "G1.K (c folded in)", from_dev(d_Kc, stKc), false, 0, nullptr, 0xFFFFFFFFu, false); });
+    };
+    if (!quotient_eval) build_K();
     if (!quotient_eval) timed("G1.Z", [&] { build_set<G1Aff, G1Xyzz>(mZ, KeyPoints(key.g1_Z, key.g1_Z_y), 32, rowsZ, cfg.window_z, "G1.Z", dec1, true); });
     else {
         const size_t nz = key.g1_Z.size() / 32;
@@ -334,14 +396,6 @@
             HIP_CHECK(hipMemcpyAsync(stV.data(), d_stV.p, domain_n, hipMemcpyDeviceToHost, stream));
             HIP_CHECK(hipStreamSynchronize(stream));
         });
-        auto from_dev = [this](const DevBuf<G1Aff>& src, const std::vector<uint8_t>& st) {
-            return [this, &src, &st](const KeyPoints& raw, G1Aff* out) {
-                const size_t n = raw.x.size() / 32;
-                HIP_CHECK(hipMemcpyAsync(out, src.p, n * sizeof(G1Aff), hipMemcpyDeviceToDevice, stream));
-                HIP_CHECK(hipStreamSynchronize(stream));
-                return std::vector<uint8_t>(st.begin(), st.begin() + n);
-            };
-        };
         DevBuf<G1Aff> d_U2, d_V2; std::vector<uint8_t> stU2, stV2;
         size_t live = domain_n;
         if (cfg.quotient_fold) {
@@ -356,12 +410,13 @@
         fuse_z_digits = mZ.nwide == live && cfg.fuse_z_digits != 0;
         if (folded) mZ.digit_bases = domain_n;
         quot_live = folded && cfg.quotient_live_tiles ? live : 0;
-        timed("G1.Z (U)", [&] { build_set<G1Aff, G1Xyzz>(mC, rawU, 32, rowsC, cfg.window_w, "G1.Z (evaluation form, c)", folded ? from_dev(d_U2, stU2) : from_dev(d_U, stU), false, 0, &row_class_c, (uint32_t)domain_n, false); });
+        if (want_cfold) timed("G1.K fold", [&] { c_fold = folded ? fold_c(d_U2, stU2) : fold_c(d_U, stU); });
+        build_K();
+        if (!c_fold || c_without_fold)
+            timed("G1.Z (U)", [&] { build_set<G1Aff, G1Xyzz>(mC, rawU, 32, rowsC, cfg.window_w, "G1.Z (evaluation form, c)", folded ? from_dev(d_U2, stU2) : from_dev(d_U, stU), false, 0, &row_class_c, (uint32_t)domain_n, false); });
     }
     if (cfg.few_path && cfg.few_z_gb > 0) {
-        const size_t nz = key.g1_Z.size() / 32;
-        int cv = 0;
-        for (int t : {8, 6, 4}) if ((double)nz * msm_windows(t) * (double)((size_t)1 << (t - 1)) * sizeof(G1Aff) <= (double)cfg.few_z_gb * 1e9) { cv = t; break; }
+        const int cv = zfew_cv;
         if (cv) timed("G1.Z (latency layout)", [&] { build_set<G1Aff, G1Xyzz>(mZfew, KeyPoints(key.g1_Z, key.g1_Z_y), 32, rowsZkey, cfg.window_z, "G1.Z", dec1, true, cv); });
     }
     timed("G2.B", [&] { build_set<G2Aff, G2Xyzz>(mB2, cat({key.g2_B, key.g2_B_y}, {{key.g2_beta, key.g2_beta_y}, {key.g2_delta, key.g2_delta_y}}), 64, rowsB2, cfg.window_w, "G2.B", dec2, false); });
@@ -416,6 +471,7 @@
         for (int k = 0; k < Lane::NSETS; k++) if (g1sets[k] != &mZfew || b == 64) {
             if (fuse_z_digits && g1sets[k] == &mZ) { const size_t keep = dg; dg = 0; need(mZ, b, p1, p1b, sj1[k]); if (dg > dgz) dgz = dg; dg = keep; }
             else need(*g1sets[k], b, p1, p1b, sj1[k]);
+            if (g1sets[k] == &mK && c_fold) need(mKc, b, p1, p1b, sj1[k]);
         }
         need(mB2, b, p2, p2b, sj2);
         Lane::ScratchNeed nd;
@@ -440,7 +496,7 @@
         ln.d_gok_s2.alloc(mB2.nbit / 8 * MSM_FEW_PROOFS + 1);
         ln.d_digits_s.alloc(dgs); ln.d_gok_s.alloc(gks); ln.d_part1c.alloc(ps); ln.d_part1d.alloc((ps / 64 + MSM_REDUCE_FANIN - 1) / MSM_REDUCE_FANIN * 64 + 64);
     }
-    for (int k = 0; k < Lane::NSETS; k++) { ln.d_sj1[k].alloc(sj1[k] ? sj1[k] : 1); ln.d_flat1[k].alloc(g1sets[k]->nflat && g1sets[k]->nwide ? B : 1); }
+    for (int k = 0; k < Lane::NSETS; k++) { ln.d_sj1[k].alloc(sj1[k] ? sj1[k] : 1); ln.d_flat1[k].alloc((g1sets[k]->nflat && g1sets[k]->nwide) || (g1sets[k] == &mK && mKc.nflat && mKc.nwide) ? B : 1); }
     ln.d_sj2.alloc(sj2 ? sj2 : 1); ln.d_flat2.alloc(B);
     ln.d_sumA.alloc(B); ln.d_sumB1.alloc(B); ln.d_sumK.alloc(B); ln.d_sumZ.alloc(B); ln.d_sumC.alloc(B); ln.d_sumB2.alloc(B); ln.d_tmp.alloc(2 * B);
     if (has_commitment) {
diff --git a/gnark-symmetric-crypto_amd/csrc/k_quot_bases.hip b/gnark-symmetric-crypto_amd/csrc/k_quot_bases.hip
--- a/gnark-symmetric-crypto_amd/csrc/k_quot_bases.hip
+++ b/gnark-symmetric-crypto_amd/csrc/k_quot_bases.hip
@@ -2,6 +2,7 @@
 #include "bn254_fp29.hpp"
 #include "verify_dev.hpp"
 #include "group_idft.hpp"
+#include "srs_columns_kernels.hpp"
 
 namespace gsc {
 using namespace bn254;
@@ -195,6 +196,30 @@
     *st = 0;
 }
 
+
+__global__ __launch_bounds__(64) void k_cf_load(const Aff<Fp>* in, const uint8_t* status, uint32_t n, vfy::VP1* out) {
+    const uint32_t i = blockIdx.x * blockDim.x + threadIdx.x;
+    if (i >= n) return;
+    vfy::VP1 r;
+    if (status[i] == 2) { r.x = Fp29f::zero(); r.y = Fp29f::zero(); r.inf = 1; }
+    else { r.x = qb_to_fp29(in[i].x); r.y = qb_to_fp29(in[i].y); r.inf = 0; }
+    out[i] = r;
+}
+
+__global__ __launch_bounds__(64) void k_cf_finish(const vfy::VP1* uhat, const Aff<Fp>* K, const uint8_t* stK, const uint32_t* slot_wire, const uint32_t* slot_k, uint32_t n,
+                                                  Aff<Fp>* out, uint8_t* status) {
+    const uint32_t j = blockIdx.x * blockDim.x + threadIdx.x;
+    if (j >= n) return;
+    const uint32_t w = slot_wire[j], k = slot_k[j];
+    Xyzz9<Fp29f> q = G1x::infinity();
+    if (k != 0xFFFFFFFFu && stK[k] != 2) q = G1x::from_aff(Aff9<Fp29f>{qb_to_fp29(K[k].x), qb_to_fp29(K[k].y)});
+    if (w != 0xFFFFFFFFu && !uhat[w].inf) q = G1x::add(q, G1x::from_aff(Aff9<Fp29f>{uhat[w].x, uhat[w].y}));
+    if (q.inf) { status[j] = 2; out[j] = Aff<Fp>{Fp::zero(), Fp::zero()}; return; }
+    const Aff9<Fp29f> a = G1x::to_aff(q);
+    out[j] = Aff<Fp>{qb_from_fp29(a.x), qb_from_fp29(a.y)};
+    status[j] = 0;
+}
+
 __global__ __launch_bounds__(64) void k_qfd_from_be(const uint8_t* be, const uint8_t* flags, uint32_t n, Aff<Fp>* out, uint8_t* status) {
     const uint32_t i = blockIdx.x * blockDim.x + threadIdx.x;
     if (i >= n) return;
@@ -244,6 +269,21 @@
     hipLaunchKernelGGL(k_qfd_finish, dim3((ncols + 63) / 64), dim3(64), 0, s, Ax, Gy, perm, n, m, node, weight, reinterpret_cast<const Aff<Fp>*>(U), stU,
                        reinterpret_cast<const Aff<Fp>*>(V), stV, reinterpret_cast<Aff<Fp>*>(U2), stU2, reinterpret_cast<Aff<Fp>*>(V2), stV2);
 }
+static size_t cf_round16(size_t b) { return (b + 15) / 16 * 16; }
+size_t c_fold_scratch_bytes(uint32_t m, uint32_t n_wires, uint32_t n_segs) {
+    return cf_round16(sizeof(vfy::VP1) * (size_t)m) + cf_round16(sizeof(vfy::VP1) * (size_t)n_wires) + column_part_bytes(n_segs, false);
+}
+void launch_c_fold(const G1Aff* U, const uint8_t* stU, uint32_t m, const G1Aff* K, const uint8_t* stK, const CFoldArgs& a, void* scratch, G1Aff* out, uint8_t* status, hipStream_t s) {
+    uint8_t* const base = static_cast<uint8_t*>(scratch);
+    vfy::VP1* const rows = reinterpret_cast<vfy::VP1*>(base);
+    vfy::VP1* const uhat = reinterpret_cast<vfy::VP1*>(base + cf_round16(sizeof(vfy::VP1) * (size_t)m));
+    void* const part = base + cf_round16(sizeof(vfy::VP1) * (size_t)m) + cf_round16(sizeof(vfy::VP1) * (size_t)a.n_wires);
+    if (m) hipLaunchKernelGGL(k_cf_load, dim3((m + 63) / 64), dim3(64), 0, s, reinterpret_cast<const Aff<Fp>*>(U), stU, m, rows);
+    launch_column_sums(rows, ColumnArgs{a.seg_begin, a.seg_end, a.col_seg, a.term_row, a.term_coeff, a.mag, a.meta, a.n_segs, a.n_wires}, part, uhat, s);
+    if (a.n_slots) hipLaunchKernelGGL(k_cf_finish, dim3((a.n_slots + 63) / 64), dim3(64), 0, s, (const vfy::VP1*)uhat, reinterpret_cast<const Aff<Fp>*>(K), stK, a.slot_wire, a.slot_k, a.n_slots,
+                                      reinterpret_cast<Aff<Fp>*>(out), status);
+}
+
 void launch_g1_aff_from_be(const uint8_t* be, const uint8_t* flags, size_t n, G1Aff* out, uint8_t* status, hipStream_t s) {
     if (n) hipLaunchKernelGGL(k_qfd_from_be, dim3((unsigned)((n + 63) / 64)), dim3(64), 0, s, be, flags, (uint32_t)n, reinterpret_cast<Aff<Fp>*>(out), status);
 }
diff --git a/gnark-symmetric-crypto_amd/csrc/kernels.hpp b/gnark-symmetric-crypto_amd/csrc/kernels.hpp
--- a/gnark-symmetric-crypto_amd/csrc/kernels.hpp
+++ b/gnark-symmetric-crypto_amd/csrc/kernels.hpp
@@ -123,6 +123,12 @@
 size_t quot_fold_dft_scratch_bytes(int L, uint32_t m);
 void launch_quot_fold_dft(int L, uint32_t m, const uint32_t* perm, const G1Aff* U, const uint8_t* stU, const G1Aff* V, const uint8_t* stV,
                           G1Aff* U2, uint8_t* stU2, G1Aff* V2, uint8_t* stV2, void* scratch, hipStream_t s, hipEvent_t weights_done = nullptr);
+struct CFoldArgs {
+    const uint32_t *seg_begin, *seg_end, *col_seg, *term_row, *term_coeff, *mag, *meta; uint32_t n_segs, n_wires;
+    const uint32_t *slot_wire, *slot_k; uint32_t n_slots;
+};
+size_t c_fold_scratch_bytes(uint32_t m, uint32_t n_wires, uint32_t n_segs);
+void launch_c_fold(const G1Aff* U, const uint8_t* stU, uint32_t m, const G1Aff* K, const uint8_t* stK, const CFoldArgs& a, void* scratch, G1Aff* out, uint8_t* status, hipStream_t s);
 void launch_g1_aff_from_be(const uint8_t* be, const uint8_t* flags, size_t n, G1Aff* out, uint8_t* status, hipStream_t s);
 void launch_g1_aff_to_be(const G1Aff* in, const uint8_t* status, size_t n, uint8_t* be, uint8_t* flags, hipStream_t s);
 void launch_g1_sum_be(const G1Xyzz* a, const G1Xyzz* b, size_t n, uint8_t* out, uint8_t* flags, hipStream_t s);
diff --git a/gnark-symmetric-crypto_amd/csrc/msm_set.hip b/gnark-symmetric-crypto_amd/csrc/msm_set.hip
--- a/gnark-symmetric-crypto_amd/csrc/msm_set.hip
+++ b/gnark-symmetric-crypto_amd/csrc/msm_set.hip
@@ -42,7 +42,7 @@
 }
 
 template <class AffT, class XyzzT>
-void msm_build_tables(MsmSet<AffT>& set, const AffT* bases, const MsmFlatPlan& plan, const std::vector<uint32_t>& rows, int c, hipStream_t stream, size_t* table_bytes) {
+void msm_build_tables(MsmSet<AffT>& set, const AffT* bases, const MsmFlatPlan& plan, const std::vector<uint32_t>& rows, int c, hipStream_t stream, size_t* table_bytes, bool windowed_rows) {
     const std::vector<uint32_t>&src = plan.src, &shift = plan.shift, &frows = plan.frows, &len = plan.len, &wide = plan.wide; const std::vector<int32_t>& octwin = plan.octwin;
     const size_t D = (size_t)1 << (c - 1);
     set.c = c; set.nwin = msm_windows(c);
@@ -68,7 +68,12 @@
         HIP_CHECK(hipStreamSynchronize(stream));
     }
     set.nwide = wide.size();
-    if (set.nwide) {
+    if (set.nwide && !windowed_rows) {
+        std::vector<uint32_t> wrows(set.nwide);
+        for (size_t i = 0; i < set.nwide; i++) wrows[i] = rows[wide[i]];
+        set.wrows.alloc(set.nwide); set.wrows.upload(wrows.data(), set.nwide, stream);
+        HIP_CHECK(hipStreamSynchronize(stream));
+    } else if (set.nwide) {
         DevBuf<AffT> wb(set.nwide); DevBuf<uint32_t> d_src(set.nwide), d_shift(set.nwide);
         std::vector<uint32_t> zero(set.nwide, 0u), wrows(set.nwide);
         for (size_t i = 0; i < set.nwide; i++) wrows[i] = rows[wide[i]];
@@ -117,6 +122,7 @@
         reduce_slices(r, g.flat_slices, B, set.nwide ? r.flat : r.sum, flat_levels);
     }
     if (set.nwide) {
+        if (!set.wtable.p) throw std::runtime_error("internal: MSM over a set whose windowed rows were not built");
         uint4* const digits = r.win_digits ? r.win_digits : ctx.digits;
         MsmRecodeArgs ra{r.scalars, set.wrows.p, r.wires ? 1 : 0, set.nwide, B, set.c, set.nwin, digits};
         if (!r.digits_ready) launch_msm_recode(ra, ctx.stream);
@@ -133,8 +139,8 @@
     if (!set.nflat && !set.nwide) HIP_CHECK(hipMemsetAsync(r.sum, 0, B * sizeof(XyzzT), ctx.stream));
 }
 
-template void msm_build_tables<G1Aff, G1Xyzz>(MsmSet<G1Aff>&, const G1Aff*, const MsmFlatPlan&, const std::vector<uint32_t>&, int, hipStream_t, size_t*);
-template void msm_build_tables<G2Aff, G2Xyzz>(MsmSet<G2Aff>&, const G2Aff*, const MsmFlatPlan&, const std::vector<uint32_t>&, int, hipStream_t, size_t*);
+template void msm_build_tables<G1Aff, G1Xyzz>(MsmSet<G1Aff>&, const G1Aff*, const MsmFlatPlan&, const std::vector<uint32_t>&, int, hipStream_t, size_t*, bool);
+template void msm_build_tables<G2Aff, G2Xyzz>(MsmSet<G2Aff>&, const G2Aff*, const MsmFlatPlan&, const std::vector<uint32_t>&, int, hipStream_t, size_t*, bool);
 template void msm_run<G1Aff, G1Xyzz>(const MsmSet<G1Aff>&, const MsmRun<G1Xyzz>&, MsmHornerJobs&);
 template void msm_run<G2Aff, G2Xyzz>(const MsmSet<G2Aff>&, const MsmRun<G2Xyzz>&, MsmHornerJobs&);
 
diff --git a/gnark-symmetric-crypto_amd/csrc/msm_set.hpp b/gnark-symmetric-crypto_amd/csrc/msm_set.hpp
--- a/gnark-symmetric-crypto_amd/csrc/msm_set.hpp
+++ b/gnark-symmetric-crypto_amd/csrc/msm_set.hpp
@@ -20,7 +20,7 @@
 };
 
 template <class AffT, class XyzzT>
-void msm_build_tables(MsmSet<AffT>& set, const AffT* bases, const MsmFlatPlan& plan, const std::vector<uint32_t>& rows, int c, hipStream_t stream, size_t* table_bytes);
+void msm_build_tables(MsmSet<AffT>& set, const AffT* bases, const MsmFlatPlan& plan, const std::vector<uint32_t>& rows, int c, hipStream_t stream, size_t* table_bytes, bool windowed_rows = true);
 
 struct MsmLevels { std::vector<std::pair<size_t, bool>> flat, win; };
 
diff --git a/gnark-symmetric-crypto_amd/csrc/wipe_plan.hpp b/gnark-symmetric-crypto_amd/csrc/wipe_plan.hpp
--- a/gnark-symmetric-crypto_amd/csrc/wipe_plan.hpp
+++ b/gnark-symmetric-crypto_amd/csrc/wipe_plan.hpp
@@ -40,7 +40,7 @@
     case WR_W: case WR_W8: return f.has_commitment ? WS_POK_SUM : WS_WIRE_SUMS;
     case WR_A: return rt.z_digits_ready ? WS_QUOTIENT : WS_Z_SUM;
     case WR_B: case WR_A8: case WR_B8: return WS_QUOTIENT;
-    case WR_C: case WR_C8: return rt.eval ? WS_WIRE_SUMS : WS_QUOTIENT;
+    case WR_C: case WR_C8: return rt.eval && !rt.c_fold ? WS_WIRE_SUMS : WS_QUOTIENT;
     case WR_DIGITS_W: return f.has_commitment ? WS_POK_SUM : WS_WIRE_SUMS;
     case WR_DIGITS: case WR_PART1A: case WR_PART1B: case WR_GOK: return f.has_commitment ? WS_POK_SUM : WS_Z_SUM;
     case WR_PART2A: case WR_PART2B: case WR_SJ2: case WR_FLAT2: return WS_ASSEMBLY;
@@ -101,9 +101,10 @@
     if (!(rt.latency && rt.use_zfew && alloc_of(table, WR_DIGITS_W))) prefix(p.b, table, WR_DIGITS, z.digits);
     prefix(p.b, table, WR_GOK, z.gok);
     prefix(p.b, table, WR_PART1A, z.part1a); prefix(p.b, table, WR_PART1B, z.part1b); prefix(p.b, table, WR_PART2A, z.part2a); prefix(p.b, table, WR_PART2B, z.part2b);
-    for (int k = 0; k < 8; k++) { prefix(p.b, table, WR_SJ1 + k, z.sj1[k]); prefix(p.b, table, WR_FLAT1 + k, B * x1); }
+    for (int k = 0; k < (rt.c_fold ? 7 : 8); k++) { prefix(p.b, table, WR_SJ1 + k, z.sj1[k]); prefix(p.b, table, WR_FLAT1 + k, B * x1); }
     prefix(p.b, table, WR_SJ2, z.sj2); prefix(p.b, table, WR_FLAT2, B * x2);
-    for (int r : {WR_SUM_A, WR_SUM_B1, WR_SUM_K, WR_SUM_Z, WR_SUM_C}) prefix(p.b, table, r, B * x1);
+    for (int r : {WR_SUM_A, WR_SUM_B1, WR_SUM_K, WR_SUM_Z}) prefix(p.b, table, r, B * x1);
+    if (!rt.c_fold) prefix(p.b, table, WR_SUM_C, B * x1);
     prefix(p.b, table, WR_SUM_B2, B * x2); prefix(p.b, table, WR_TMP, 2 * B * x1);
     prefix(p.b, table, WR_INPUTS, 176 * B); prefix(p.b, table, WR_RS, 64 * B);
     if (f.has_commitment) {
diff --git a/include/libprove.h b/include/libprove.h
--- a/include/libprove.h
+++ b/include/libprove.h
@@ -52,6 +52,9 @@
                           const uint64_t *win, size_t nwin, uint64_t *counts, float *ms);
 extern int gsc_debug_quot_fold_dft(int L, uint32_t m, const uint32_t *perm, const uint8_t *u_be, const uint8_t *u_inf, const uint8_t *v_be, const uint8_t *v_inf,
                                    uint8_t *u2_be, uint8_t *u2_inf, uint8_t *v2_be, uint8_t *v2_inf);
+extern int gsc_debug_c_fold(uint32_t m, const uint8_t *u_be, const uint8_t *u_inf, uint32_t n_wires, const uint32_t *col_start, const uint32_t *term_row, const uint32_t *term_coeff,
+                            uint32_t n_coeff, const uint8_t *coeff_be, uint32_t n_k, const uint8_t *k_be, const uint8_t *k_inf, const uint32_t *k_wire,
+                            uint8_t *uhat_be, uint8_t *uhat_inf, uint8_t *k2_be, uint8_t *k2_inf);
 extern int gsc_debug_glv_split(const uint8_t *k, uint8_t *out);
 
 extern size_t gsc_describe(GoUint8 algorithmID, char *out, size_t cap);
```

Measured after the change: 29460 proofs/s (median of 6 runs). Within noise of the previous version (+0.6%).
